# zihuixue/DynMM

Measured on AMD Instinct MI355X. Metric: images/sec fwd+bwd, 480x640 RGB-D, batch 32/GPU, higher is better.
Workload: dtype f32; 1 GPU; configs[2]: zero-grad + fwd + weighted 4-scale CE + FLOP loss + bwd + fused SGD-Nesterov update, --dynamic --global-gate soft DiffSoftmax gates tau=1; per_gpu_batch=32, global_batch=32, height=480, width=640, parallelism=dp1, launch=eager, streams=4, optimizer_in_step=fused SGD-Nesterov

## Files before the change

dynmm_amd/csrc/conv_igemm.hip:

```cpp
#include <stdlib.h>

#include "common.h"
#include "conv_igemm.h"
#include "conv_small.h"
#include "vec.h"

namespace dynmm {


__device__ __forceinline__ float ldg_f32(const float* sbase, unsigned voff_bytes) {
    return *reinterpret_cast<const float*>(reinterpret_cast<const char*>(sbase) + voff_bytes);
}
__device__ __forceinline__ float4 ldg_f32x4(const float* sbase, unsigned voff_bytes) {
    return *reinterpret_cast<const float4*>(reinterpret_cast<const char*>(sbase) + voff_bytes);
}


template <int TCO, int TPIX, int WCO, int WPIX, bool DGRAD, int MODE>
__global__ void __launch_bounds__(256, (TCO * TPIX > 8192 ? 2 : (TPIX > 128 ? 4 : 6))) conv_igemm_kernel(const IgemmArgs a) {
    constexpr bool GENERIC = MODE == 2;
    constexpr bool padded = MODE == 1;
    constexpr int BK = 16;
    constexpr int MCO = WCO / 32, MPIX = WPIX / 32;
    constexpr int WAVES_PIX = TPIX / WPIX;
    static_assert((TCO / WCO) * WAVES_PIX == 4, "4 waves per workgroup");
    constexpr int AQ = TCO / 4, A_ROWSTEP = 256 / AQ;
    constexpr int A_PER = (BK * AQ + 255) / 256;
    constexpr int B_PER = BK * TPIX / 256, B_ROWSTEP = 256 / TPIX;

    __shared__ __attribute__((aligned(16))) float As[2][BK][TCO];
    __shared__ __attribute__((aligned(16))) float Bs[2][BK][TPIX];

    const int t = threadIdx.x;
    const int lane = t & 63, wave = t >> 6;
    const int wave_co = wave / WAVES_PIX, wave_pix = wave % WAVES_PIX;
    DYNMM_TRACE_MARK(0);
#ifdef DYNMM_TRACE
    if (g_trace && threadIdx.x == 0) g_trace[(size_t)blockIdx.x * 6 + 4] = clock64();
#endif

    const int nblk = a.n_co_tiles * a.n_pix_tiles;
    const int lin = xcd_remap(blockIdx.x, nblk);
    const int co0 = (lin % a.n_co_tiles) * TCO;
    const int pix0 = (lin / a.n_co_tiles) * TPIX;

    const int HW = a.H * a.W;
    const int HoWo = a.Ho * a.Wo;

    const int a_q = t % AQ, a_row0 = t / AQ;
    const bool a_active = a_row0 < BK;
    int q_glob = co0 / 4 + a_q;
    if (q_glob > a.CoP / 4 - 1) q_glob = a.CoP / 4 - 1;
    const unsigned a_voff = (unsigned)((a_active ? a_row0 : 0) * a.CoP + q_glob * 4) * 4u;

    auto pix_decode = [&](int m, int& n, int& oh, int& ow, int& cls) {
        n = m / HoWo;
        const int q = m - n * HoWo;
        if (DGRAD && a.subpix) {
            const int Wc = a.Wo / a.SW;
            const int csz = HoWo / (a.SH * a.SW);
            cls = q / csz;
            const int q2 = q - cls * csz;
            const int ohc = q2 / Wc;
            const int ph = cls / a.SW;
            oh = ohc * a.SH + ph;
            ow = (q2 - ohc * Wc) * a.SW + (cls - ph * a.SW);
        } else {
            cls = 0;
            oh = q / a.Wo;
            ow = q - oh * a.Wo;
        }
    };
    const int b_col = t % TPIX, b_row0 = t / TPIX;
    const int m_b = pix0 + b_col;
    const bool m_ok = m_b < a.M;
    int n_b = 0, oh_b = 0, ow_b = 0, cls_b = 0;
    if (m_ok) pix_decode(m_b, n_b, oh_b, ow_b, cls_b);
    (void)cls_b;
    const int c2 = a.Ci - a.c_in_split;

    auto in_coord = [&](int r, int s, int& ih, int& iw) -> bool {
        if (!DGRAD) {
            ih = oh_b * a.SH - a.PH + r;
            iw = ow_b * a.SW - a.PW + s;
            return m_ok && ih >= 0 && ih < a.H && iw >= 0 && iw < a.W;
        } else {
            const int th = oh_b + a.PH - r, tw = ow_b + a.PW - s;
            if (!m_ok || th < 0 || tw < 0) return false;
            ih = th / a.SH;
            iw = tw / a.SW;
            return (ih * a.SH == th) && (iw * a.SW == tw) && ih < a.H && iw < a.W;
        }
    };

    float4 ra[A_PER];
    float rb[B_PER];
    f32x16 acc[MCO][MPIX];
#pragma unroll
    for (int mi = 0; mi < MCO; ++mi)
#pragma unroll
        for (int ni = 0; ni < MPIX; ++ni)
#pragma unroll
            for (int j = 0; j < 16; ++j) acc[mi][ni][j] = 0.f;

    const int khalf = lane >> 5, l31 = lane & 31;

    auto mfma_tile = [&](int buf) {
        float af[BK / 2][MCO], bf[BK / 2][MPIX];
#pragma unroll
        for (int kk = 0; kk < BK / 2; ++kk) {
#pragma unroll
            for (int mi = 0; mi < MCO; ++mi)
                af[kk][mi] = As[buf][2 * kk + khalf][wave_co * WCO + mi * 32 + l31];
#pragma unroll
            for (int ni = 0; ni < MPIX; ++ni)
                bf[kk][ni] = Bs[buf][2 * kk + khalf][wave_pix * WPIX + ni * 32 + l31];
        }
#pragma unroll
        for (int kk = 0; kk < BK / 2; ++kk)
#pragma unroll
            for (int mi = 0; mi < MCO; ++mi)
#pragma unroll
                for (int ni = 0; ni < MPIX; ++ni)
                    acc[mi][ni] = __builtin_amdgcn_mfma_f32_32x32x2f32(af[kk][mi], bf[kk][ni], acc[mi][ni], 0, 0, 0);
    };

    if constexpr (!GENERIC) {
        const int cpt = a.CiR / BK;
        int live_ph = -1, live_pw = -1;
        if (DGRAD && a.subpix) {
            int n0, oh0, ow0, c0, n1, oh1, ow1, c1;
            pix_decode(pix0, n0, oh0, ow0, c0);
            pix_decode(min(pix0 + TPIX, a.M) - 1, n1, oh1, ow1, c1);
            if (n0 == n1 && c0 == c1) { live_ph = c0 / a.SW; live_pw = c0 - live_ph * a.SW; }
        }
        auto tap_live = [&](int r, int s_) -> bool {
            if (!(DGRAD && a.subpix) || live_ph < 0) return true;
            return ((live_ph + a.PH - r) % a.SH == 0) && ((live_pw + a.PW - s_) % a.SW == 0);
        };
        int n_live = 0;
        for (int r = 0; r < a.KH; ++r)
            for (int s_ = 0; s_ < a.KW; ++s_) n_live += tap_live(r, s_) ? 1 : 0;
        const int nk = n_live * cpt;
        int ci0 = 0, tr = 0, ts = 0, kbase = 0;
        bool tap_ok;
        unsigned voff1, voff2;
        auto set_tap = [&]() {
            int ih = 0, iw = 0;
            tap_ok = in_coord(tr, ts, ih, iw);
            const unsigned pix = tap_ok ? (unsigned)(ih * a.W + iw) : 0u;
            voff1 = ((unsigned)(n_b * a.c_in_split + b_row0) * (unsigned)HW + pix) * 4u;
            voff2 = ((unsigned)(n_b * c2 + b_row0) * (unsigned)HW + pix) * 4u;
        };
        auto next_tap = [&]() {
            do {
                if (++ts == a.KW) { ts = 0; ++tr; }
                if (tr >= a.KH) return;
// ... 1143 lines not shown

extern "C" int dynmm_conv2d_stem_fwd_stats(const float* x, const float* wp_fwd, const float* bias, float* y, double* stats,
                                           const dynmm_conv_geom* g, void* stream) {
    (void)hipGetLastError();
    if (!x || !wp_fwd || !y || !stats || !geom_ok(g)) return DYNMM_EINVAL;
    if (!dynmm_conv2d_stem_fwd_stats_supported(g)) return DYNMM_EUNSUPPORTED;
    SmallConvArgs s{x, nullptr, wp_fwd, nullptr, bias, y, g->N, g->Ci, g->H, g->W, g->Co, g->Ho, g->Wo, g->KH, g->KW,
                    g->SH, g->SW, g->PH, g->PW, g->c_split, round_k(g->Ci), (g->Co + 3) & ~3, DYNMM_ACT_NONE};
    s.stats = stats;
    return launch_stem_conv_fwd(s, (hipStream_t)stream);
}

extern "C" int dynmm_conv2d_dgrad(const float* dy, const float* wp_dgrad, const float* mask,
                                  const float* accum, float* dx, float* dx2,
                                  const dynmm_conv_geom* g, void* stream) {
    (void)hipGetLastError();
    if (!dy || !wp_dgrad || !dx || !geom_ok(g)) return DYNMM_EINVAL;
    if ((g->c_split < g->Ci) != (dx2 != nullptr)) return DYNMM_EINVAL;
    if ((mask || accum) && dx2) return DYNMM_EUNSUPPORTED;
    IgemmArgs a{};
    a.x = dy; a.x2 = nullptr; a.wp = wp_dgrad; a.mask = mask; a.residual = accum; a.y = dx; a.y2 = dx2;
    a.N = g->N; a.Ci = g->Co; a.H = g->Ho; a.W = g->Wo;
    a.Co = g->Ci; a.Ho = g->H; a.Wo = g->W;
    a.KH = g->KH; a.KW = g->KW; a.SH = g->SH; a.SW = g->SW; a.PH = g->PH; a.PW = g->PW;
    a.c_in_split = g->Co; a.c_out_split = g->c_split; a.act = DYNMM_ACT_NONE;
    return launch_igemm<true>(a, (hipStream_t)stream);
}

static bool wgrad_fast_rows_ok(const dynmm_conv_geom* g) {
    return (g->Ci % 64 == 0) || (g->KH == 1 && g->KW == 1);
}

static void launch_wgrad_generic(const WgradArgs& a, const WgradGroup& grp, const WgradPlan& p, dim3 grid, bool dual,
                                 bool fast, hipStream_t st) {
#define DYNMM_WGRAD_LAUNCH(TCO, TK, WCO, WK)                                                          \
    do {                                                                                              \
        if (dual)                                                                                     \
            hipLaunchKernelGGL((conv_wgrad_kernel<TCO, TK, WCO, WK, true, false>), grid, dim3(256), 0, st, a, grp);  \
        else if (fast)                                                                                \
            hipLaunchKernelGGL((conv_wgrad_kernel<TCO, TK, WCO, WK, false, true>), grid, dim3(256), 0, st, a, grp);  \
        else                                                                                          \
            hipLaunchKernelGGL((conv_wgrad_kernel<TCO, TK, WCO, WK, false, false>), grid, dim3(256), 0, st, a, grp); \
    } while (0)
    if (p.tco == 128)
        DYNMM_WGRAD_LAUNCH(128, 128, 64, 64);
    else if (p.tco == 64 && p.tk == 192)
        DYNMM_WGRAD_LAUNCH(64, 192, 32, 96);
    else if (p.tco == 64 && p.tk == 64)
        DYNMM_WGRAD_LAUNCH(64, 64, 32, 32);
    else if (p.tco == 64)
        DYNMM_WGRAD_LAUNCH(64, 128, 64, 32);
    else
        DYNMM_WGRAD_LAUNCH(32, 128, 32, 32);
#undef DYNMM_WGRAD_LAUNCH
}

static size_t generic_wgrad_workspace_bytes(const dynmm_conv_geom* g);

extern "C" size_t dynmm_conv2d_wgrad_workspace_bytes(const dynmm_conv_geom* g) {
    if (!geom_ok(g)) return 0;
    const size_t stem = stem_conv_wgrad_eligible(g->Ci, g->Co, g->KH, g->KW, g->SH, g->SW, g->PH, g->PW, g->c_split < g->Ci, false)
                            ? stem_conv_wgrad_workspace_bytes(g->N, g->Ci, g->Ho, g->Wo) : 0;
    const size_t gen = generic_wgrad_workspace_bytes(g);
    const size_t co8 = co8_wgrad_eligible(g->Ci, g->Co, g->H, g->W, g->Ho, g->Wo, g->KH, g->KW, g->SH, g->SW, g->PH, g->PW, g->c_split)
                           ? co8_wgrad_workspace_bytes(g->N, g->Ci, g->Co) : 0;
    const size_t m = stem > gen ? stem : gen;
    return co8 > m ? co8 : m;
}

static size_t plan_workspace_bytes(const dynmm_conv_geom* g, const WgradPlan& p) {
    if (p.splits <= 1) return 0;
    const size_t wslab = ((size_t)p.splits * g->Co * g->Ci * g->KH * g->KW + 3) & ~(size_t)3;
    return (wslab + (size_t)p.splits * g->Co) * sizeof(float);
}

static size_t generic_wgrad_workspace_bytes(const dynmm_conv_geom* g) {
    const size_t a = plan_workspace_bytes(g, plan_wgrad(g)), b = plan_workspace_bytes(g, plan_wgrad(g, false));
    return a > b ? a : b;
}

extern "C" int dynmm_conv2d_wgrad(const float* x, const float* x2, const float* dy, float* dw, float* dbias,
                                  void* workspace, size_t workspace_bytes,
                                  const dynmm_conv_geom* g, void* stream) {
    (void)hipGetLastError();
    if (!x || !dy || !dw || !geom_ok(g)) return DYNMM_EINVAL;
    if ((g->c_split < g->Ci) != (x2 != nullptr)) return DYNMM_EINVAL;
    if (stem_conv_wgrad_eligible(g->Ci, g->Co, g->KH, g->KW, g->SH, g->SW, g->PH, g->PW, x2 != nullptr, dbias != nullptr) &&
        ((reinterpret_cast<uintptr_t>(dy) & 15u) == 0)) {
        const size_t need_s = stem_conv_wgrad_workspace_bytes(g->N, g->Ci, g->Ho, g->Wo);
        if (!workspace || workspace_bytes < need_s) return DYNMM_EWORKSPACE;
        return launch_stem_conv_wgrad(x, dy, dw, (float*)workspace, g->N, g->Ci, g->H, g->W, g->Ho, g->Wo, (hipStream_t)stream);
    }
    const bool aligned16 = ((reinterpret_cast<uintptr_t>(x) | reinterpret_cast<uintptr_t>(dy)) & 15u) == 0;
    if (co8_wgrad_eligible(g->Ci, g->Co, g->H, g->W, g->Ho, g->Wo, g->KH, g->KW, g->SH, g->SW, g->PH, g->PW, g->c_split) &&
        ((reinterpret_cast<uintptr_t>(x) | reinterpret_cast<uintptr_t>(x2)) & 15u) == 0) {
        const size_t need_c = co8_wgrad_workspace_bytes(g->N, g->Ci, g->Co);
        if (!workspace || workspace_bytes < need_c || (reinterpret_cast<uintptr_t>(workspace) & 15u)) return DYNMM_EWORKSPACE;
        return launch_co8_wgrad(x, x2, dy, dw, dbias, (float*)workspace, g->N, g->Ci, g->H, g->W, g->Co, g->Ho, g->Wo,
                                g->c_split, (hipStream_t)stream);
    }
    const WgradPlan p = plan_wgrad(g, aligned16 && !x2);
    const size_t need = generic_wgrad_workspace_bytes(g);
    if (need > 0 && (!workspace || workspace_bytes < need)) return DYNMM_EWORKSPACE;
    WgradArgs a{};
    a.x = x; a.x2 = x2; a.dy = dy;
    a.out = p.splits > 1 ? (float*)workspace : dw;
    const size_t wslab = ((size_t)p.splits * g->Co * g->Ci * g->KH * g->KW + 3) & ~(size_t)3;
    float* bias_slabs = p.splits > 1 ? (float*)workspace + wslab : dbias;
    a.out_bias = dbias ? bias_slabs : nullptr;
    a.N = g->N; a.Ci = g->Ci; a.H = g->H; a.W = g->W; a.Co = g->Co; a.Ho = g->Ho; a.Wo = g->Wo;
    a.KH = g->KH; a.KW = g->KW; a.SH = g->SH; a.SW = g->SW; a.PH = g->PH; a.PW = g->PW;
    a.c_split = g->c_split;
    a.M = g->N * g->Ho * g->Wo;
    a.K = g->KH * g->KW * g->Ci;
    a.n_co_tiles = p.n_co_tiles; a.n_k_tiles = p.n_k_tiles; a.steps_per_split = p.steps_per_split;
    hipStream_t st = (hipStream_t)stream;
    dim3 grid((unsigned)(p.n_co_tiles * p.n_k_tiles * p.splits));
    const bool dual = x2 != nullptr;
    const bool fast = !dual && wgrad_fast_rows_ok(g) && g->H >= g->KH && g->W >= g->KW;
    a.magic_wo = (g->Wo >= 2 && (unsigned long long)g->Ho * g->Wo * g->Wo < (1ull << 32)) ? (unsigned)((1ull << 32) / (unsigned)g->Wo) + 1u : 0u;
    const bool v4 = !p.v6 && !dual && p.tco == 128 && p.tk == 128 && (g->Ci % 64 == 0) && g->SW == 1 &&
                    (g->KW == 1 || g->KW == 3) && g->PW == g->KW / 2 && g->W == g->Wo && (g->W % 4 == 0) &&
                    ((g->Ho * g->Wo) % 4 == 0) && g->H >= g->KH &&
                    ((reinterpret_cast<uintptr_t>(x) & 15u) == 0) && ((reinterpret_cast<uintptr_t>(dy) & 15u) == 0);
    const bool bias_ok4 = !dbias || ((g->Co % 4 == 0) && ((reinterpret_cast<uintptr_t>(bias_slabs) & 15u) == 0) &&
                                     ((reinterpret_cast<uintptr_t>(dbias) & 15u) == 0));
    const bool perm = (v4 || p.v6) && p.splits > 1 && ((reinterpret_cast<uintptr_t>(workspace) & 15u) == 0) && bias_ok4;
    a.k_major_out = perm ? 1 : 0;
    if (p.v6 || v4) {
        if (p.v6)
            launch_wgrad_v6(a, WgradGroup{}, grid, wgrad_v6_occupancy(g), st);
        else
            hipLaunchKernelGGL((conv_wgrad_v4_kernel<128, 128, 1>), grid, dim3(512), 0, st, a, WgradGroup{});
        DYNMM_LAUNCH_CHECK();
        if (perm) {
            const int n = g->Co * a.K, nb1 = ceil_div(n / 4, 64), nb2 = dbias ? ceil_div(g->Co / 4, 64) : 0;
            hipLaunchKernelGGL(reduce_slabs_perm_kernel, dim3(nb1 + nb2), dim3(256), 0, st, (const float*)workspace, dw,
                               n, p.splits, g->Ci, g->KH * g->KW, a.K, dbias ? bias_slabs : nullptr, dbias,
                               dbias ? g->Co : 0, nb1, ReduceGroup{});
            DYNMM_LAUNCH_CHECK();
            return DYNMM_OK;
        }
    } else
        launch_wgrad_generic(a, WgradGroup{}, p, grid, dual, fast, st);
    DYNMM_LAUNCH_CHECK();
    if (p.splits > 1) {
        launch_reduce_slabs((const float*)workspace, dw, g->Co * a.K, p.splits, st, dbias ? bias_slabs : nullptr,
                            dbias, dbias ? g->Co : 0);
        DYNMM_LAUNCH_CHECK();
    }
    return DYNMM_OK;
}

static bool wgrad_v4_shape_ok(const dynmm_conv_geom* g, const WgradPlan& p) {
    if (p.v6) return (g->Co % 4 == 0);
    return g->c_split == g->Ci && p.tco == 128 && p.tk == 128 && (g->Ci % 64 == 0) && g->SW == 1 &&
           (g->KW == 1 || g->KW == 3) && g->PW == g->KW / 2 && g->W == g->Wo && (g->W % 4 == 0) &&
           ((g->Ho * g->Wo) % 4 == 0) && g->H >= g->KH && (g->Co % 4 == 0);
}

static WgradPlan plan_wgrad_group(const dynmm_conv_geom* g, int n) {
    WgradPlan p = plan_wgrad(g);
    if (!p.v6) p.target = 512;
    plan_splits(p, g, n);
    return p;
}

static size_t group_problem_floats(const dynmm_conv_geom* g, const WgradPlan& p) {
    const size_t wslab = ((size_t)p.splits * g->Co * g->Ci * g->KH * g->KW + 3) & ~(size_t)3;
    return (wslab + (size_t)p.splits * g->Co + 3) & ~(size_t)3;
}

extern "C" int dynmm_conv2d_wgrad_groupable(const dynmm_conv_geom* g) {
    if (!geom_ok(g) || g->c_split != g->Ci) return 0;
    if (stem_conv_wgrad_eligible(g->Ci, g->Co, g->KH, g->KW, g->SH, g->SW, g->PH, g->PW, false, false)) return 0;
    if (co8_wgrad_eligible(g->Ci, g->Co, g->H, g->W, g->Ho, g->Wo, g->KH, g->KW, g->SH, g->SW, g->PH, g->PW, g->c_split)) return 0;
    const WgradPlan p = plan_wgrad(g);
    if (p.splits <= 1) return 0;
    return wgrad_v4_shape_ok(g, p) ? 2 : 1;
}

extern "C" int dynmm_conv2d_wgrad_variant(const dynmm_conv_geom* g) {
    if (!geom_ok(g)) return 0;
    if (stem_conv_wgrad_eligible(g->Ci, g->Co, g->KH, g->KW, g->SH, g->SW, g->PH, g->PW, g->c_split < g->Ci, false)) return 0;
    if (co8_wgrad_eligible(g->Ci, g->Co, g->H, g->W, g->Ho, g->Wo, g->KH, g->KW, g->SH, g->SW, g->PH, g->PW, g->c_split)) return 8;
    const WgradPlan p = plan_wgrad(g);
    if (p.v6) return 6;
    return wgrad_v4_shape_ok(g, p) ? 4 : 0;
}

extern "C" size_t dynmm_conv2d_wgrad_group_workspace_bytes(const dynmm_conv_geom* g, int n) {
    if (!geom_ok(g) || n < 1 || n > kWgradGroupMax) return 0;
    if (n == 1 || !dynmm_conv2d_wgrad_groupable(g)) return dynmm_conv2d_wgrad_workspace_bytes(g);
    const WgradPlan p = plan_wgrad_group(g, n);
    return sizeof(float) * group_problem_floats(g, p) * (size_t)n;
}

extern "C" int dynmm_conv2d_wgrad_group(int n, const float* const* xs, const float* const* dys, float* const* dws,
                                        float* const* dbiases, void* workspace, size_t workspace_bytes,
                                        const dynmm_conv_geom* g, void* stream) {
    (void)hipGetLastError();
    if (n < 1 || n > kWgradGroupMax || !xs || !dys || !dws || !geom_ok(g)) return DYNMM_EINVAL;
    bool aligned = (reinterpret_cast<uintptr_t>(workspace) & 15u) == 0;
    for (int i = 0; i < n; ++i) {
        if (!xs[i] || !dys[i] || !dws[i]) return DYNMM_EINVAL;
        aligned = aligned && ((reinterpret_cast<uintptr_t>(xs[i]) | reinterpret_cast<uintptr_t>(dys[i])) & 15u) == 0 &&
                  (!dbiases || !dbiases[i] || (reinterpret_cast<uintptr_t>(dbiases[i]) & 15u) == 0);
        if (dbiases && ((dbiases[i] != nullptr) != (dbiases[0] != nullptr))) return DYNMM_EINVAL;
    }
    const int kind = dynmm_conv2d_wgrad_groupable(g);
    if (n == 1 || kind == 0 || (kind == 2 && !aligned)) {
        for (int i = 0; i < n; ++i) {
            const int rc = dynmm_conv2d_wgrad(xs[i], nullptr, dys[i], dws[i], dbiases ? dbiases[i] : nullptr, workspace,
                                              workspace_bytes, g, stream);
            if (rc != DYNMM_OK) return rc;
        }
        return DYNMM_OK;
    }
    const WgradPlan p = plan_wgrad_group(g, n);
    const size_t per_floats = group_problem_floats(g, p);
    if (!workspace || workspace_bytes < sizeof(float) * per_floats * (size_t)n) return DYNMM_EWORKSPACE;
    const bool has_bias = dbiases && dbiases[0];
    const size_t wslab = ((size_t)p.splits * g->Co * g->Ci * g->KH * g->KW + 3) & ~(size_t)3;
    WgradArgs a{};
    WgradGroup grp{};
    grp.nprob = n;
    grp.per = p.n_co_tiles * p.n_k_tiles * p.splits;
    for (int i = 0; i < n; ++i) {
        float* base = (float*)workspace + per_floats * (size_t)i;
        grp.x[i] = xs[i];
        grp.dy[i] = dys[i];
        grp.out[i] = base;
        grp.out_bias[i] = has_bias ? base + wslab : nullptr;
    }
    a.x = xs[0]; a.x2 = nullptr; a.dy = dys[0]; a.out = grp.out[0]; a.out_bias = grp.out_bias[0];
    a.N = g->N; a.Ci = g->Ci; a.H = g->H; a.W = g->W; a.Co = g->Co; a.Ho = g->Ho; a.Wo = g->Wo;
    a.KH = g->KH; a.KW = g->KW; a.SH = g->SH; a.SW = g->SW; a.PH = g->PH; a.PW = g->PW;
    a.c_split = g->c_split;
    a.M = g->N * g->Ho * g->Wo;
    a.K = g->KH * g->KW * g->Ci;
    a.n_co_tiles = p.n_co_tiles; a.n_k_tiles = p.n_k_tiles; a.steps_per_split = p.steps_per_split;
    a.magic_wo = (g->Wo >= 2 && (unsigned long long)g->Ho * g->Wo * g->Wo < (1ull << 32)) ? (unsigned)((1ull << 32) / (unsigned)g->Wo) + 1u : 0u;
    hipStream_t st = (hipStream_t)stream;
    dim3 grid((unsigned)(grp.per * n));
    if (kind == 1) {
        a.k_major_out = 0;
        const bool fast = wgrad_fast_rows_ok(g) && g->H >= g->KH && g->W >= g->KW;
        launch_wgrad_generic(a, grp, p, grid, false, fast, st);
        DYNMM_LAUNCH_CHECK();
        ReduceGroup rgp{};
        rgp.nprob = n;
        for (int i = 0; i < n; ++i) {
            rgp.slabs[i] = grp.out[i];
            rgp.out[i] = dws[i];
            rgp.slabs2[i] = has_bias ? grp.out_bias[i] : nullptr;
            rgp.out2[i] = has_bias ? dbiases[i] : nullptr;
        }
        launch_reduce_slabs_group(rgp, g->Co * a.K, p.splits, has_bias ? g->Co : 0, st);
        DYNMM_LAUNCH_CHECK();
        return DYNMM_OK;
    }
    a.k_major_out = 1;
    if (p.v6)
        launch_wgrad_v6(a, grp, grid, wgrad_v6_occupancy(g), st);
    else
        hipLaunchKernelGGL((conv_wgrad_v4_kernel<128, 128, 1>), grid, dim3(512), 0, st, a, grp);
    DYNMM_LAUNCH_CHECK();
    const int nel = g->Co * a.K, nb1 = ceil_div(nel / 4, 64), nb2 = has_bias ? ceil_div(g->Co / 4, 64) : 0;
    ReduceGroup rg{};
    rg.nprob = n;
    for (int i = 0; i < n; ++i) {
        rg.slabs[i] = grp.out[i];
        rg.out[i] = dws[i];
        rg.slabs2[i] = has_bias ? grp.out_bias[i] : nullptr;
        rg.out2[i] = has_bias ? dbiases[i] : nullptr;
    }
    hipLaunchKernelGGL(reduce_slabs_perm_kernel, dim3(nb1 + nb2, n), dim3(256), 0, st, (const float*)nullptr, (float*)nullptr,
                       nel, p.splits, g->Ci, g->KH * g->KW, a.K, (const float*)nullptr, (float*)nullptr,
                       has_bias ? g->Co : 0, nb1, rg);
    DYNMM_LAUNCH_CHECK();
    return DYNMM_OK;
}

extern "C" int dynmm_reduce_slabs(const float* slabs, float* out, int n, int nslabs, void* stream) {
    (void)hipGetLastError();
    if (!slabs || !out || n <= 0 || nslabs <= 0) return DYNMM_EINVAL;
    launch_reduce_slabs(slabs, out, n, nslabs, (hipStream_t)stream);
    DYNMM_LAUNCH_CHECK();
    return DYNMM_OK;
}

#ifdef DYNMM_TRACE
#include "conv_igemm_v5.hip"
#endif
```

dynmm_amd/csrc/conv_small.h:

```cpp
#pragma once
#include <hip/hip_runtime.h>

namespace dynmm {

struct SmallConvArgs {
    const float* x;
    const float* x2;
    const float* wp;
    const float* scale;
    const float* shift;
    float* y;
    int N, Ci, H, W, Co, Ho, Wo, KH, KW, SH, SW, PH, PW, c_split, CiR, CoP, act;
    double* stats = nullptr;
};

struct StemWgradArgs {
    const float* x;
    const float* dy;
    float* slabs;
    int N, H, W, Ho, Wo;
};

bool stem_conv_wgrad_eligible(int Ci, int Co, int KH, int KW, int SH, int SW, int PH, int PW, bool has_x2, bool has_bias);
size_t stem_conv_wgrad_workspace_bytes(int N, int Ci, int Ho, int Wo);
int launch_stem_conv_wgrad(const float* x, const float* dy, float* dw, float* workspace, int N, int Ci, int H, int W,
                           int Ho, int Wo, hipStream_t st);

bool co8_wgrad_eligible(int Ci, int Co, int H, int W, int Ho, int Wo, int KH, int KW, int SH, int SW, int PH, int PW, int c_split);
size_t co8_wgrad_workspace_bytes(int N, int Ci, int Co);
int launch_co8_wgrad(const float* x, const float* x2, const float* dy, float* dw, float* dbias, float* workspace, int N, int Ci,
                     int H, int W, int Co, int Ho, int Wo, int c_split, hipStream_t st);

bool small_conv_fwd_eligible(const SmallConvArgs& a, const float* residual);
int launch_small_conv_fwd(const SmallConvArgs& a, hipStream_t st);
bool stem_conv_fwd_eligible(const SmallConvArgs& a, const float* residual);
int launch_stem_conv_fwd(const SmallConvArgs& a, hipStream_t st);

}
```

dynmm_amd/csrc/conv_small.hip:

```cpp
#include "common.h"
#include "conv_small.h"
#include "conv_igemm.h"

namespace dynmm {

constexpr int kSP = 5;
constexpr int kSRows = 4;
constexpr int kSColGroups = 16;
constexpr int kSCols = kSColGroups * kSP;

__device__ __forceinline__ float small_act(float v, int act) {
    if (act == DYNMM_ACT_RELU) return v > 0.f ? v : 0.f;
    if (act == DYNMM_ACT_TANH) return tanhf(v);
    if (act == DYNMM_ACT_SWISH) return swish_fwd(v);
    if (act == DYNMM_ACT_HSWISH) return hswish_fwd(v);
    return v;
}

template <int KS, int S>
__global__ void __launch_bounds__(256) conv_co8_fwd_kernel(const SmallConvArgs a) {
    constexpr int IR = (kSRows - 1) * S + KS;
    constexpr int IC = (kSCols - 1) * S + KS;
    constexpr int TILE = IR * IC;
    constexpr int NLD = (TILE + 63) / 64;
    constexpr int XW = (kSP - 1) * S + KS;
    constexpr int RED = 4 * 8 * kSRows * kSCols;
    constexpr int LDSF = (4 * 2 * TILE > RED) ? 4 * 2 * TILE : RED;
    __shared__ float lds[LDSF];

    const int lane = threadIdx.x & 63;
    const int wave = __builtin_amdgcn_readfirstlane(threadIdx.x >> 6);
    const int tw = (a.Wo + kSCols - 1) / kSCols, th = (a.Ho + kSRows - 1) / kSRows;
    int b = blockIdx.x;
    const int n = b / (th * tw);
    b -= n * th * tw;
    const int oh0 = (b / tw) * kSRows, ow0 = (b - (b / tw) * tw) * kSCols;
    const int ih0 = oh0 * S, iw0 = ow0 * S;
    const int r = lane >> 4, cg = lane & 15;

    int goff[NLD];
    unsigned okmask = 0u;
#pragma unroll
    for (int k = 0; k < NLD; ++k) {
        const int e = k * 64 + lane;
        const int rr = e / IC, cc = e - rr * IC;
        const bool ok = e < TILE && ih0 + rr < a.H && iw0 + cc < a.W;
        goff[k] = ok ? (ih0 + rr) * a.W + iw0 + cc : 0;
        okmask |= ok ? (1u << k) : 0u;
    }
    const int cpw = a.Ci / 4;
    const int c_begin = wave * cpw;
    const int HW = a.H * a.W;
    float* const tile0 = lds + wave * 2 * TILE;

    auto plane = [&](int ci) -> const float* {
        return ci < a.c_split ? a.x + ((size_t)n * a.c_split + ci) * HW
                              : a.x2 + ((size_t)n * (a.Ci - a.c_split) + (ci - a.c_split)) * HW;
    };
    float st[NLD];
    auto stage_load = [&](int ci) {
        const float* p = plane(ci);
#pragma unroll
        for (int k = 0; k < NLD; ++k) st[k] = p[goff[k]];
    };
    auto stage_store = [&](float* t) {
#pragma unroll
        for (int k = 0; k < NLD; ++k)
            if (k * 64 + lane < TILE) t[k * 64 + lane] = ((okmask >> k) & 1u) ? st[k] : 0.f;
    };

    float acc[8][kSP];
#pragma unroll
    for (int co = 0; co < 8; ++co)
#pragma unroll
        for (int p = 0; p < kSP; ++p) acc[co][p] = 0.f;

    auto wave_sync = [] {
        __builtin_amdgcn_fence(__ATOMIC_ACQ_REL, "wavefront");
        __builtin_amdgcn_wave_barrier();
    };
    stage_load(c_begin);
    stage_store(tile0);
    wave_sync();
    for (int i = 0; i < cpw; ++i) {
        const int ci = c_begin + i;
        const float* t = tile0 + (i & 1) * TILE;
        if (i + 1 < cpw) stage_load(ci + 1);
        const float* wci = a.wp + (size_t)ci * 8;
#pragma unroll
        for (int kh = 0; kh < KS; ++kh) {
            const float* row = t + (S * r + kh) * IC + S * kSP * cg;
            float xv[XW];
#pragma unroll
            for (int j = 0; j < XW; ++j) xv[j] = row[j];
#pragma unroll
            for (int kw = 0; kw < KS; ++kw) {
                const float* wt = wci + (size_t)(kh * KS + kw) * a.CiR * 8;
#pragma unroll
                for (int co = 0; co < 8; ++co) {
                    const float wv = wt[co];
#pragma unroll
                    for (int p = 0; p < kSP; ++p) acc[co][p] = fmaf(wv, xv[S * p + kw], acc[co][p]);
                }
            }
        }
        if (i + 1 < cpw) stage_store(tile0 + ((i + 1) & 1) * TILE);
        wave_sync();
    }
    __syncthreads();
#pragma unroll
    for (int co = 0; co < 8; ++co)
#pragma unroll
        for (int p = 0; p < kSP; ++p)
            lds[((wave * 8 + co) * kSRows + r) * kSCols + cg * kSP + p] = acc[co][p];
    __syncthreads();
    constexpr int PER = 8 * kSRows * kSCols;
    for (int e = threadIdx.x; e < PER; e += 256) {
        const int co = e / (kSRows * kSCols), rem = e - co * (kSRows * kSCols);
        const int rr = rem / kSCols, cc = rem - rr * kSCols;
        const int oh = oh0 + rr, ow = ow0 + cc;
        if (co < a.Co && oh < a.Ho && ow < a.Wo) {
            float v = ((lds[e] + lds[PER + e]) + lds[2 * PER + e]) + lds[3 * PER + e];
            v = v * (a.scale ? a.scale[co] : 1.f) + (a.shift ? a.shift[co] : 0.f);
            a.y[(((size_t)n * a.Co + co) * a.Ho + oh) * a.Wo + ow] = small_act(v, a.act);
        }
    }
}

struct Co8WgradArgs {
    const float* x;
    const float* x2;
    const float* dy;
    float* slabs;
    float* bias_slabs;
    int N, Ci, H, W, Co, Ho, Wo, c_split, NI, G;
};

__device__ __forceinline__ float row16_sum(float v) {
    v += __int_as_float(__builtin_amdgcn_mov_dpp(__float_as_int(v), 0xB1, 0xF, 0xF, true));
    v += __int_as_float(__builtin_amdgcn_mov_dpp(__float_as_int(v), 0x4E, 0xF, 0xF, true));
    v += __int_as_float(__builtin_amdgcn_mov_dpp(__float_as_int(v), 0x141, 0xF, 0xF, true));
    v += __int_as_float(__builtin_amdgcn_mov_dpp(__float_as_int(v), 0x140, 0xF, 0xF, true));
    return v;
}

template <int KS, int S>
__global__ void __launch_bounds__(256, 1) conv_co8_wgrad_kernel(const Co8WgradArgs a) {
    constexpr int PR = 16;
    constexpr int IR = (PR - 1) * S + KS;
    constexpr int XW = (kSP - 1) * S + KS;
    constexpr int NACC = KS * KS * 8;
    extern __shared__ __attribute__((aligned(16))) float dyn_lds[];
    const int tile_floats = IR * a.W + 16;
    float* const tiles = dyn_lds;
    float* const red = dyn_lds + 2 * tile_floats;
// ... 184 lines not shown
    const int tw = (a.Wo + TCW - 1) / TCW, th = (a.Ho + TRW - 1) / TRW;
    const int HW = a.H * a.W;
    const int tiles = a.N * th * tw;

    float areg[NSTEP];
#pragma unroll
    for (int st = 0; st < NSTEP; ++st) {
        const int ci = st / (KS * KW8 / 2), rem = st - ci * (KS * KW8 / 2);
        const int kh = rem / (KW8 / 2), kp = rem - kh * (KW8 / 2);
        const int kw = 2 * kp + khalf;
        areg[st] = kw < KS ? a.wp[((size_t)(kh * KS + kw) * a.CiR + ci) * a.CoP + mi * 32 + l31] : 0.f;
    }
    const int pb_off = (S * 2 * rp) * ICP + S * l31 + khalf;
    const bool vec_out = (a.Wo & 3) == 0;

    auto fetch_patch = [&](int tile, float* dst) __attribute__((always_inline)) {
        int b = tile;
        const int n = b / (th * tw);
        b -= n * th * tw;
        const int ih0 = (b / tw) * TRW * S - PAD, iw0 = (b - (b / tw) * tw) * TCW * S - PAD;
        const float* xn = a.x + (size_t)n * CI * HW;
#pragma unroll 1
        for (int it = 0; it < NIT; ++it) {
            const int e = it * 256 + threadIdx.x;
            const int ci = min(e / (IR * ICP), CI - 1), rem = e - ci * (IR * ICP);
            const int rr = rem / ICP, cc = rem - rr * ICP;
            const int ih = ih0 + rr, iw = iw0 + cc;
            const bool inside = e < NPATCH;
            const bool ok = inside && ih >= 0 && ih < a.H && iw >= 0 && iw < a.W;
            float* slot = dst + it * 256 + (threadIdx.x & ~63);
            if (ok)
                __builtin_amdgcn_global_load_lds((const __attribute__((address_space(1))) void*)(xn + (size_t)ci * HW + (size_t)ih * a.W + iw),
                                                 (__attribute__((address_space(3))) void*)slot, 4, 0, 0);
            else if (inside)
                dst[e] = 0.f;
        }
    };

    float st1[2][4], st2[2][4];
#pragma unroll
    for (int q = 0; q < 2; ++q)
#pragma unroll
        for (int ps = 0; ps < 4; ++ps) st1[q][ps] = st2[q][ps] = 0.f;

    int buf = 0;
    if ((int)blockIdx.x < tiles) fetch_patch(blockIdx.x, patch2[0]);
    __builtin_amdgcn_s_waitcnt(0);
    __syncthreads();
    for (int tile = blockIdx.x; tile < tiles; tile += gridDim.x, buf ^= 1) {
        int b = tile;
        const int n = b / (th * tw);
        b -= n * th * tw;
        const int oh0 = (b / tw) * TRW, ow0 = (b - (b / tw) * tw) * TCW;
        const float* patch = patch2[buf];
        const float* pb = patch + pb_off;
        float* const ostage = patch2[buf] + wave * OCH;
        const int next = tile + (int)gridDim.x;
        if (next < tiles) fetch_patch(next, patch2[buf ^ 1]);

        f32x16 acc[2][2];
#pragma unroll
        for (int i = 0; i < 2; ++i)
#pragma unroll
            for (int j = 0; j < 2; ++j)
#pragma unroll
                for (int e = 0; e < 16; ++e) acc[i][j][e] = 0.f;
#pragma unroll
        for (int ci = 0; ci < CI; ++ci)
#pragma unroll
            for (int kh = 0; kh < KS; ++kh)
#pragma unroll
                for (int kp = 0; kp < KW8 / 2; ++kp) {
                    const int boff = (ci * IR + kh) * ICP + 2 * kp;
                    const float av = areg[(ci * KS + kh) * (KW8 / 2) + kp];
                    const float b00 = pb[boff], b01 = pb[boff + S * 32];
                    const float b10 = pb[boff + S * ICP], b11 = pb[boff + S * ICP + S * 32];
                    acc[0][0] = __builtin_amdgcn_mfma_f32_32x32x2f32(av, b00, acc[0][0], 0, 0, 0);
                    acc[0][1] = __builtin_amdgcn_mfma_f32_32x32x2f32(av, b01, acc[0][1], 0, 0, 0);
                    acc[1][0] = __builtin_amdgcn_mfma_f32_32x32x2f32(av, b10, acc[1][0], 0, 0, 0);
                    acc[1][1] = __builtin_amdgcn_mfma_f32_32x32x2f32(av, b11, acc[1][1], 0, 0, 0);
                }
        __syncthreads();

#pragma unroll
        for (int rr = 0; rr < 2; ++rr)
#pragma unroll
            for (int q = 0; q < 2; ++q) {
#pragma unroll
                for (int jj = 0; jj < 8; ++jj) {
                    const int j = 8 * q + jj;
                    const int cl = (jj & 3) + 8 * (jj >> 2) + 4 * khalf;
                    const int c = mi * 32 + 16 * q + cl;
                    const float sc = a.scale ? a.scale[c] : 1.f, sh = a.shift ? a.shift[c] : 0.f;
                    const int act = STATS ? DYNMM_ACT_NONE : a.act;
                    ostage[cl * OP + l31] = small_act(fmaf(acc[rr][0][j], sc, sh), act);
                    ostage[cl * OP + 32 + l31] = small_act(fmaf(acc[rr][1][j], sc, sh), act);
                }
                __builtin_amdgcn_fence(__ATOMIC_ACQ_REL, "wavefront");
                __builtin_amdgcn_wave_barrier();
                const int oh = oh0 + 2 * rp + rr;
                if (oh < a.Ho) {
#pragma unroll
                    for (int ps = 0; ps < 4; ++ps) {
                        const int cl = ps * 4 + (lane >> 4), col = (lane & 15) * 4;
                        const int c = mi * 32 + 16 * q + cl;
                        const float4 v = *reinterpret_cast<const float4*>(ostage + cl * OP + col);
                        float* yr = a.y + (((size_t)n * a.Co + c) * a.Ho + oh) * a.Wo + ow0 + col;
                        if (vec_out && ow0 + col + 3 < a.Wo) {
                            *reinterpret_cast<float4*>(yr) = v;
                            if constexpr (STATS) {
                                st1[q][ps] += (v.x + v.y) + (v.z + v.w);
                                st2[q][ps] += fmaf(v.x, v.x, v.y * v.y) + fmaf(v.z, v.z, v.w * v.w);
                            }
                        } else {
                            const float e[4] = {v.x, v.y, v.z, v.w};
#pragma unroll
                            for (int k = 0; k < 4; ++k)
                                if (ow0 + col + k < a.Wo) {
                                    yr[k] = e[k];
                                    if constexpr (STATS) {
                                        st1[q][ps] += e[k];
                                        st2[q][ps] = fmaf(e[k], e[k], st2[q][ps]);
                                    }
                                }
                        }
                    }
                }
                __builtin_amdgcn_fence(__ATOMIC_ACQ_REL, "wavefront");
                __builtin_amdgcn_wave_barrier();
            }
        __builtin_amdgcn_s_waitcnt(0);
        __syncthreads();
    }
    if constexpr (STATS) {
#pragma unroll
        for (int q = 0; q < 2; ++q)
#pragma unroll
            for (int ps = 0; ps < 4; ++ps) {
                float s1 = st1[q][ps], s2 = st2[q][ps];
#pragma unroll
                for (int o = 1; o < 16; o <<= 1) {
                    s1 += __shfl_xor(s1, o, 64);
                    s2 += __shfl_xor(s2, o, 64);
                }
                if ((lane & 15) == 0) {
                    const int c = mi * 32 + 16 * q + 4 * ps + (lane >> 4);
                    atomicAdd(a.stats + c, (double)s1);
                    atomicAdd(a.stats + a.Co + c, (double)s2);
                }
            }
    }
}

template <int CI>
__global__ void __launch_bounds__(256, CI == 1 ? 4 : 2) conv_stem_wgrad_kernel(const StemWgradArgs a) {
    constexpr int KS = 7, S = 2, PAD = 3, KW8 = 8;
    constexpr int TRW = 2, TCW = 64, NPX = TRW * TCW;
    constexpr int IR = (TRW - 1) * S + KS;
    constexpr int ICP = (TCW - 1) * S + KW8 + 1;
    constexpr int KT = CI * KS * KW8;
    constexpr int NKT = (KT + 31) / 32;
    constexpr int KPW = NKT / 2;
    constexpr int PP = NPX + 1;
    __shared__ float patch[CI * IR * ICP];
    __shared__ float dyt[64 * PP];

    const int lane = threadIdx.x & 63, l31 = lane & 31, khalf = lane >> 5;
    const int wave = threadIdx.x >> 6;
    const int cot = wave & 1, kt0 = (wave >> 1) * KPW;
    const int tw = (a.Wo + TCW - 1) / TCW, th = (a.Ho + TRW - 1) / TRW;
    const int HW = a.H * a.W, HoWo = a.Ho * a.Wo;
    const int tiles = a.N * th * tw;

    int boff[KPW];
#pragma unroll
    for (int j = 0; j < KPW; ++j) {
        int k = (kt0 + j) * 32 + l31;
        if (k >= KT) k = 0;
        const int ci = k / (KS * KW8), rem = k - ci * (KS * KW8);
        boff[j] = (ci * IR + (rem >> 3)) * ICP + (rem & 7) + S * khalf;
    }
    const float* ab = dyt + (cot * 32 + l31) * PP + khalf;
    f32x16 acc[KPW];
#pragma unroll
    for (int j = 0; j < KPW; ++j)
#pragma unroll
        for (int e = 0; e < 16; ++e) acc[j][e] = 0.f;

    for (int tile = blockIdx.x; tile < tiles; tile += gridDim.x) {
        int b = tile;
        const int n = b / (th * tw);
        b -= n * th * tw;
        const int oh0 = (b / tw) * TRW, ow0 = (b - (b / tw) * tw) * TCW;
        const int ih0 = oh0 * S - PAD, iw0 = ow0 * S - PAD;
        __syncthreads();
        {
            constexpr int NIT = (CI * IR * ICP + 255) / 256;
            float sv[NIT];
            const float* xn = a.x + (size_t)n * CI * HW;
#pragma unroll
            for (int it = 0; it < NIT; ++it) {
                const int e = it * 256 + threadIdx.x;
                const int ci = min(e / (IR * ICP), CI - 1), rem = e - ci * (IR * ICP);
                const int rr = rem / ICP, cc = rem - rr * ICP;
                const int ih = ih0 + rr, iw = iw0 + cc;
                const bool ok = ih >= 0 && ih < a.H && iw >= 0 && iw < a.W;
                const float v = xn[(size_t)ci * HW + (size_t)min(max(ih, 0), a.H - 1) * a.W + min(max(iw, 0), a.W - 1)];
                sv[it] = ok ? v : 0.f;
            }
            float4 dv[8];
            const float* dn = a.dy + (size_t)n * 64 * HoWo;
            const bool vec = (a.Wo & 3) == 0;
#pragma unroll
            for (int it = 0; it < 8; ++it) {
                const int i4 = it * 256 + threadIdx.x;
                const int co = i4 >> 5, q = i4 & 31, r = q >> 4, c4 = (q & 15) * 4;
                const int oh = oh0 + r, ow = ow0 + c4;
                const float* src = dn + (size_t)co * HoWo + (size_t)min(oh, a.Ho - 1) * a.Wo;
                float4 v = make_float4(0.f, 0.f, 0.f, 0.f);
                if (oh < a.Ho) {
                    if (vec && ow + 3 < a.Wo) v = *reinterpret_cast<const float4*>(src + ow);
                    else {
                        if (ow < a.Wo) v.x = src[ow];
                        if (ow + 1 < a.Wo) v.y = src[ow + 1];
                        if (ow + 2 < a.Wo) v.z = src[ow + 2];
                        if (ow + 3 < a.Wo) v.w = src[ow + 3];
                    }
                }
                dv[it] = v;
            }
#pragma unroll
            for (int it = 0; it < NIT; ++it) {
                const int e = it * 256 + threadIdx.x;
                if (e < CI * IR * ICP) patch[e] = sv[it];
            }
#pragma unroll
            for (int it = 0; it < 8; ++it) {
                const int i4 = it * 256 + threadIdx.x;
                const int co = i4 >> 5, q = i4 & 31;
                float* dst = dyt + co * PP + q * 4;
                dst[0] = dv[it].x; dst[1] = dv[it].y; dst[2] = dv[it].z; dst[3] = dv[it].w;
            }
        }
        __syncthreads();
#pragma unroll
        for (int ps = 0; ps < NPX / 2; ++ps) {
            const int row = (2 * ps) / TCW, col = (2 * ps) % TCW;
            const int poff = S * row * ICP + S * col;
            const float av = ab[2 * ps];
#pragma unroll
            for (int j = 0; j < KPW; ++j) {
                const float bv = patch[boff[j] + poff];
                acc[j] = __builtin_amdgcn_mfma_f32_32x32x2f32(av, bv, acc[j], 0, 0, 0);
            }
        }
    }
    float* slab = a.slabs + (size_t)blockIdx.x * 64 * (NKT * 32);
#pragma unroll
    for (int j = 0; j < KPW; ++j)
#pragma unroll
        for (int e = 0; e < 16; ++e) {
            const int co = cot * 32 + (e & 3) + 8 * (e >> 2) + 4 * khalf;
            slab[(size_t)co * (NKT * 32) + (kt0 + j) * 32 + l31] = acc[j][e];
        }
}

__global__ void __launch_bounds__(256) stem_wgrad_finish_kernel(const float* __restrict__ slabs, int nslabs, int kpad,
                                                                int CI, float* __restrict__ dw) {
    const int i = blockIdx.x * 256 + threadIdx.x;
    const int per_co = CI * 49;
    if (i >= 64 * per_co) return;
    const int co = i / per_co, rem = i - co * per_co;
    const int ci = rem / 49, t = rem - ci * 49;
    const int k = (ci * 7 + t / 7) * 8 + t % 7;
    float s0 = 0.f, s1 = 0.f, s2 = 0.f, s3 = 0.f;
    const size_t stride = (size_t)64 * kpad;
    const float* p = slabs + (size_t)co * kpad + k;
    int sl = 0;
    for (; sl + 3 < nslabs; sl += 4) {
        s0 += p[(size_t)sl * stride];
        s1 += p[(size_t)(sl + 1) * stride];
        s2 += p[(size_t)(sl + 2) * stride];
        s3 += p[(size_t)(sl + 3) * stride];
    }
    for (; sl < nslabs; ++sl) s0 += p[(size_t)sl * stride];
    dw[i] = (s0 + s1) + (s2 + s3);
}

static int stem_wgrad_grid(long tiles, int Ci) {
    static int cus = 0;
    if (!cus) {
        int dev = 0;
        hipDeviceProp_t prop;
        if (hipGetDevice(&dev) == hipSuccess && hipGetDeviceProperties(&prop, dev) == hipSuccess) cus = prop.multiProcessorCount;
        if (cus <= 0) cus = 256;
    }
    const long cap = (long)cus * (Ci == 1 ? 4 : 2);
    return (int)(tiles < cap ? tiles : cap);
}

bool stem_conv_wgrad_eligible(int Ci, int Co, int KH, int KW, int SH, int SW, int PH, int PW, bool has_x2, bool has_bias) {
    if (has_x2 || has_bias) return false;
    if (KH != 7 || KW != 7 || SH != 2 || SW != 2 || PH != 3 || PW != 3) return false;
    return (Ci == 1 || Ci == 3) && Co == 64;
}

size_t stem_conv_wgrad_workspace_bytes(int N, int Ci, int Ho, int Wo) {
    const long tiles = (long)N * ceil_div(Ho, 2) * ceil_div(Wo, 64);
    const int kpad = ((Ci * 56 + 31) / 32) * 32;
    return sizeof(float) * (size_t)stem_wgrad_grid(tiles, Ci) * 64 * kpad;
}

int launch_stem_conv_wgrad(const float* x, const float* dy, float* dw, float* workspace, int N, int Ci, int H, int W,
                           int Ho, int Wo, hipStream_t st) {
    const long tiles = (long)N * ceil_div(Ho, 2) * ceil_div(Wo, 64);
    if (tiles > 0x7fffffffL) return DYNMM_EUNSUPPORTED;
    const int grid = stem_wgrad_grid(tiles, Ci);
    const int kpad = ((Ci * 56 + 31) / 32) * 32;
    StemWgradArgs a{x, dy, workspace, N, H, W, Ho, Wo};
    if (Ci == 3)
        hipLaunchKernelGGL((conv_stem_wgrad_kernel<3>), dim3(grid), dim3(256), 0, st, a);
    else
        hipLaunchKernelGGL((conv_stem_wgrad_kernel<1>), dim3(grid), dim3(256), 0, st, a);
    DYNMM_LAUNCH_CHECK();
    hipLaunchKernelGGL(stem_wgrad_finish_kernel, dim3(ceil_div(64 * Ci * 49, 256)), dim3(256), 0, st, workspace, grid, kpad,
                       Ci, dw);
    DYNMM_LAUNCH_CHECK();
    return DYNMM_OK;
}

bool stem_conv_fwd_eligible(const SmallConvArgs& a, const float* residual) {
    if (residual || a.x2) return false;
    if (a.KH != 7 || a.KW != 7 || a.SH != 2 || a.SW != 2 || a.PH != 3 || a.PW != 3) return false;
    return (a.Ci == 1 || a.Ci == 3) && a.Co == 64;
}

int launch_stem_conv_fwd(const SmallConvArgs& a_in, hipStream_t st) {
    const long tiles = (long)a_in.N * ceil_div(a_in.Ho, 4) * ceil_div(a_in.Wo, 64);
    if (tiles > 0x7fffffffL) return DYNMM_EUNSUPPORTED;
    const SmallConvArgs& a = a_in;
    static int cus = 0;
    if (!cus) {
        int dev = 0;
        hipDeviceProp_t prop;
        if (hipGetDevice(&dev) == hipSuccess && hipGetDeviceProperties(&prop, dev) == hipSuccess) cus = prop.multiProcessorCount;
        if (cus <= 0) cus = 256;
    }
    const int resident = a.Ci == 1 ? 3 : 2;
    const long cap = (long)cus * resident;
    const unsigned grid = (unsigned)(tiles < cap ? tiles : cap);
    if (a.stats) {
        if (a.act != DYNMM_ACT_NONE) return DYNMM_EUNSUPPORTED;
        if (a.Ci == 3)
            hipLaunchKernelGGL((conv_stem_fwd_kernel<3, true>), dim3(grid), dim3(256), 0, st, a);
        else
            hipLaunchKernelGGL((conv_stem_fwd_kernel<1, true>), dim3(grid), dim3(256), 0, st, a);
    } else if (a.Ci == 3)
        hipLaunchKernelGGL((conv_stem_fwd_kernel<3>), dim3(grid), dim3(256), 0, st, a);
    else
        hipLaunchKernelGGL((conv_stem_fwd_kernel<1>), dim3(grid), dim3(256), 0, st, a);
    DYNMM_LAUNCH_CHECK();
    return DYNMM_OK;
}

bool small_conv_fwd_eligible(const SmallConvArgs& a, const float* residual) {
    if (residual) return false;
    if (a.Co < 5 || a.Co > 8) return false;
    if (a.KH != 5 || a.KW != 5 || a.SH != 2 || a.SW != 2 || a.PH != 0 || a.PW != 0) return false;
    if (a.Ci % 4 != 0 || a.Ci < 16) return false;
    if (a.c_split < a.Ci && a.c_split % (a.Ci / 4) != 0) return false;
    return true;
}

int launch_small_conv_fwd(const SmallConvArgs& a, hipStream_t st) {
    const long tiles = (long)a.N * ceil_div(a.Ho, kSRows) * ceil_div(a.Wo, kSCols);
    if (tiles > 0x7fffffffL) return DYNMM_EUNSUPPORTED;
    hipLaunchKernelGGL((conv_co8_fwd_kernel<5, 2>), dim3((unsigned)tiles), dim3(256), 0, st, a);
    DYNMM_LAUNCH_CHECK();
    return DYNMM_OK;
}

}
```

dynmm_amd/csrc/pointwise.hip:

```cpp
#include "common.h"
#include <initializer_list>
#include "vec.h"
#include "pool.h"

namespace dynmm {

__device__ __forceinline__ float keep_if(float v, bool keep) { return __int_as_float(__float_as_int(v) & -(int)keep); }



__global__ void __launch_bounds__(256) maxpool_fwd_kernel(const float* __restrict__ x,
                                                          float* __restrict__ y,
                                                          signed char* __restrict__ idx, int H,
                                                          int W, int Ho, int Wo) {
    const size_t plane = blockIdx.x;
    const float* xp = x + plane * H * W;
    const int HoWo = Ho * Wo;
    const int beg = blockIdx.y * kChunk, end = min(HoWo, beg + kChunk);
    for (int i = beg + threadIdx.x; i < end; i += 256) {
        const int oh = i / Wo, ow = i - oh * Wo;
        float best = -INFINITY;
        int bi = -1;
#pragma unroll
        for (int r = 0; r < 3; ++r) {
// ... 872 lines not shown
    return DYNMM_OK;
}

extern "C" int dynmm_nearest_into_bwd(const float* g_out, float* dy, int N, int C, int h, int w,
                                      int Ctot, int c_off, int H, int W, void* stream) {
    (void)hipGetLastError();
    if (!g_out || !dy || N <= 0 || C <= 0 || h <= 0 || w <= 0 || H <= 0 || W <= 0) return DYNMM_EINVAL;
    if (c_off < 0 || c_off + C > Ctot) return DYNMM_EINVAL;
    const int area = ceil_div(H, h) * ceil_div(W, w);
    const int nout = N * C * h * w;
#define DYNMM_NIB(L) hipLaunchKernelGGL(nearest_into_bwd_kernel<L>, dim3(ceil_div_sz((size_t)nout * L, 256)), dim3(256), 0, ST, \
                                        g_out, dy, N, C, h, w, Ctot, c_off, H, W)
    if ((h == H && w == W) || area < 8) DYNMM_NIB(1);
    else if (area < 32) DYNMM_NIB(4);
    else if (area < 128) DYNMM_NIB(16);
    else DYNMM_NIB(64);
#undef DYNMM_NIB
    DYNMM_LAUNCH_CHECK();
    return DYNMM_OK;
}

extern "C" int dynmm_upsample2x_dw3x3_fwd(const float* x, const float* w, const float* b,
                                          const float* skip, float* y, int N, int C, int H, int W,
                                          void* stream) {
    (void)hipGetLastError();
    if (!x || !w || !y || N <= 0 || C <= 0 || H <= 0 || W <= 0) return DYNMM_EINVAL;
    if (!aligned16(y) || (skip && !aligned16(skip))) return DYNMM_EUNSUPPORTED;
    dim3 grid(N * C, plane_chunks(H * ((W + 1) / 2), kChunk / 8));
    hipLaunchKernelGGL(upsample_fwd_kernel, grid, dim3(256), 0, ST, x, w, b, skip, y, C, H, W);
    DYNMM_LAUNCH_CHECK();
    return DYNMM_OK;
}

static int upsample_w_splits(int N, int C) {
    int S = 2048 / C;
    if (S < 1) S = 1;
    if (S > N) S = N;
    return S;
}

extern "C" size_t dynmm_upsample2x_dw3x3_bwd_workspace_bytes(int N, int C) {
    if (N <= 0 || C <= 0) return 0;
    const int S = upsample_w_splits(N, C);
    return S > 1 ? sizeof(float) * (size_t)S * C * 10 : 0;
}

extern "C" int dynmm_upsample2x_dw3x3_bwd(const float* g, const float* x, const float* w, float* dx,
                                          float* dw, float* db, float* workspace, int N, int C, int H, int W,
                                          void* stream) {
    (void)hipGetLastError();
    if (!g || !w || N <= 0 || C <= 0 || H <= 0 || W <= 0) return DYNMM_EINVAL;
    if (dx) {
        dim3 grid(N * C, plane_chunks(H * W, kChunk));
        const int pairs = (W % 2 == 0) && aligned16(g) && ((reinterpret_cast<uintptr_t>(dx) & 7u) == 0);
        hipLaunchKernelGGL(upsample_bwd_dx_kernel, grid, dim3(256), 0, ST, g, w, dx, C, H, W, pairs);
        DYNMM_LAUNCH_CHECK();
    }
    if (dw) {
        if (!x) return DYNMM_EINVAL;
        const int S = upsample_w_splits(N, C);
        if (S == 1) {
            hipLaunchKernelGGL(upsample_bwd_w_kernel, dim3(C, 1), dim3(256), 0, ST, g, x, dw, db, N, C, H, W);
            DYNMM_LAUNCH_CHECK();
        } else {
            if (!workspace) return DYNMM_EWORKSPACE;
            float* pw = workspace, *pb = workspace + (size_t)S * C * 9;
            hipLaunchKernelGGL(upsample_bwd_w_kernel, dim3(C, S), dim3(256), 0, ST, g, x, pw, db ? pb : nullptr, N, C, H, W);
            DYNMM_LAUNCH_CHECK();
            launch_reduce_slabs(pw, dw, C * 9, S, ST, db ? pb : nullptr, db, db ? C : 0);
            DYNMM_LAUNCH_CHECK();
        }
    }
    return DYNMM_OK;
}

static int gap2_launch(const float* xr, const float* xd, float* sr, float* sd, int NC, int HW, const float* tr, int C,
                       void* stream);

extern "C" int dynmm_gap2_fwd(const float* xr, const float* xd, float* sr, float* sd, int NC, int HW,
                              void* stream) {
    return gap2_launch(xr, xd, sr, sd, NC, HW, nullptr, 1, stream);
}

extern "C" int dynmm_gap2_bnrelu_fwd(const float* xr, const float* xd, const float* bn_tr, int C, float* sr, float* sd,
                                     int NC, int HW, void* stream) {
    if (!bn_tr || C <= 0 || NC % C != 0) return DYNMM_EINVAL;
    return gap2_launch(xr, xd, sr, sd, NC, HW, bn_tr, C, stream);
}

static int gap2_launch(const float* xr, const float* xd, float* sr, float* sd, int NC, int HW, const float* tr, int C,
                       void* stream) {
    (void)hipGetLastError();
    if (!xr || !sr || NC <= 0 || HW <= 0) return DYNMM_EINVAL;
    if (xd && !sd) return DYNMM_EINVAL;
#define DYNMM_GAP2(V, DUAL, TR) hipLaunchKernelGGL((gap2_kernel<V, DUAL, TR>), dim3(NC), dim3(256), 0, ST, xr, xd, sr, sd, HW, tr, C)
#define DYNMM_GAP2_V(V)                                    \
    do {                                                   \
        if (xd && tr) DYNMM_GAP2(V, true, true);           \
        else if (xd) DYNMM_GAP2(V, true, false);           \
        else if (tr) DYNMM_GAP2(V, false, true);           \
        else DYNMM_GAP2(V, false, false);                  \
    } while (0)
    if (can_vec4(HW, {xr, xd}))
        DYNMM_GAP2_V(4);
    else
        DYNMM_GAP2_V(1);
#undef DYNMM_GAP2_V
#undef DYNMM_GAP2
    DYNMM_LAUNCH_CHECK();
    return DYNMM_OK;
}

extern "C" int dynmm_axpby_fwd(const float* xr, const float* xd, const float* a, const float* b,
                               float* out, int NC, int HW, void* stream) {
    (void)hipGetLastError();
    if (!xr || !xd || !a || !b || !out || NC <= 0 || HW <= 0) return DYNMM_EINVAL;
    dim3 grid(NC, plane_chunks(HW, kChunk));
    if (can_vec4(HW, {xr, xd, out}))
        hipLaunchKernelGGL(axpby_fwd_kernel<4>, grid, dim3(256), 0, ST, xr, xd, a, b, out, HW);
    else
        hipLaunchKernelGGL(axpby_fwd_kernel<1>, grid, dim3(256), 0, ST, xr, xd, a, b, out, HW);
    DYNMM_LAUNCH_CHECK();
    return DYNMM_OK;
}

extern "C" int dynmm_axpby_bwd_reduce(const float* g, const float* xr, const float* xd, float* da,
                                      float* db, int NC, int HW, void* stream) {
    (void)hipGetLastError();
    if (!g || !xr || !xd || !da || !db || NC <= 0 || HW <= 0) return DYNMM_EINVAL;
    if (can_vec4(HW, {g, xr, xd}))
        hipLaunchKernelGGL(axpby_bwd_reduce_kernel<4>, dim3(NC), dim3(256), 0, ST, g, xr, xd, da, db, HW);
    else
        hipLaunchKernelGGL(axpby_bwd_reduce_kernel<1>, dim3(NC), dim3(256), 0, ST, g, xr, xd, da, db, HW);
    DYNMM_LAUNCH_CHECK();
    return DYNMM_OK;
}

extern "C" int dynmm_axpby_bwd_apply(const float* g, const float* a, const float* b, const float* ca,
                                     const float* cb, float cscale, float* dxr, float* dxd, int NC,
                                     int HW, void* stream) {
    (void)hipGetLastError();
    if (!g || !a || !b || !dxr || !dxd || NC <= 0 || HW <= 0) return DYNMM_EINVAL;
    dim3 grid(NC, plane_chunks(HW, kChunk));
    if (can_vec4(HW, {g, dxr, dxd}))
        hipLaunchKernelGGL(axpby_bwd_apply_kernel<4>, grid, dim3(256), 0, ST, g, a, b, ca, cb, cscale, dxr, dxd, HW);
    else
        hipLaunchKernelGGL(axpby_bwd_apply_kernel<1>, grid, dim3(256), 0, ST, g, a, b, ca, cb, cscale, dxr, dxd, HW);
    DYNMM_LAUNCH_CHECK();
    return DYNMM_OK;
}

namespace dynmm {

struct StemBnArgs {
    const float* go; const signed char* io;
    const float* gd; const signed char* id;
    const float* coef; const float* off; float cscale;
    const float* x; const float* mean; const float* invstd; const float* gamma; const float* beta;
    int N, C, H, W, Ho, Wo;
};

__device__ __forceinline__ void stem_gy_block(const StemBnArgs& a, size_t plane, int ar, int t, float fc, float fo,
                                              float (&top)[8], float (&bot)[8]) {
    const size_t po = plane * (size_t)a.Ho * a.Wo;
    pool_bwd_block(a.go + po, a.io + po, ar, t, a.Ho, a.Wo, top, bot);
#pragma unroll
    for (int k = 0; k < 8; ++k) { top[k] = fmaf(fc, top[k], fo); bot[k] = fmaf(fc, bot[k], fo); }
    if (a.gd) {
        float dt[8], db[8];
        pool_bwd_block(a.gd + po, a.id + po, ar, t, a.Ho, a.Wo, dt, db);
#pragma unroll
        for (int k = 0; k < 8; ++k) { top[k] += dt[k]; bot[k] += db[k]; }
    }
}

__global__ void __launch_bounds__(256) stem_bn_bwd_reduce_kernel(const StemBnArgs a, double* __restrict__ sums) {
    __shared__ float red[4];
    const int c = blockIdx.x, S = gridDim.y;
    const float mu = a.mean[c], is = a.invstd[c];
    const float sc = a.gamma[c] * is;
    const float sh = fmaf(-mu, sc, a.beta[c]);
    const int Wq = a.Wo / 4, nq = a.Ho * Wq;
    float s1 = 0.f, s2 = 0.f;
    for (int n = blockIdx.y; n < a.N; n += S) {
        const size_t plane = (size_t)n * a.C + c;
        const float fc = a.coef[plane], fo = a.off ? a.off[plane] * a.cscale : 0.f;
        const float* xp = a.x + plane * (size_t)a.H * a.W;
        float a1 = 0.f, a2 = 0.f;
        for (int q = threadIdx.x; q < nq; q += 256) {
            const int ar = q / Wq, t = q - ar * Wq;
            float top[8], bot[8];
            stem_gy_block(a, plane, ar, t, fc, fo, top, bot);
            const size_t o = (size_t)(2 * ar) * a.W + 8 * t;
#pragma unroll
            for (int h = 0; h < 2; ++h) {
                const float4 x0 = *reinterpret_cast<const float4*>(xp + o + 4 * h);
                const float4 x1 = *reinterpret_cast<const float4*>(xp + o + a.W + 4 * h);
                const float xv[8] = {x0.x, x0.y, x0.z, x0.w, x1.x, x1.y, x1.z, x1.w};
#pragma unroll
                for (int k = 0; k < 8; ++k) {
                    const float gy = k < 4 ? top[4 * h + k] : bot[4 * h + k - 4];
                    const float ge = fmaf(xv[k], sc, sh) > 0.f ? gy : 0.f;
                    a1 += ge;
                    a2 += ge * (xv[k] - mu) * is;
                }
            }
        }
        s1 += a1; s2 += a2;
    }
    const float t1 = block_reduce_sum_256<float>(s1, red);
    const float t2 = block_reduce_sum_256<float>(s2, red);
    if (threadIdx.x == 0) {
        atomicAdd(&sums[c], (double)t1);
        atomicAdd(&sums[a.C + c], (double)t2);
    }
}

__global__ void __launch_bounds__(256) stem_bn_bwd_apply_kernel(const StemBnArgs a, const double* __restrict__ sums,
                                                                float* __restrict__ dx, float* __restrict__ dgamma,
                                                                float* __restrict__ dbeta) {
    const size_t plane = blockIdx.x;
    const int c = (int)(plane % a.C);
    const float mu = a.mean[c], is = a.invstd[c];
    const float sc = a.gamma[c] * is;
    const float sh = fmaf(-mu, sc, a.beta[c]);
    const float sg = (float)sums[c], sgx = (float)sums[a.C + c];
    if (plane < (size_t)a.C && blockIdx.y == 0 && threadIdx.x == 0) {
        if (dgamma) dgamma[c] = sgx;
        if (dbeta) dbeta[c] = sg;
    }
    const float invM = 1.f / ((float)a.N * (float)(a.H * a.W));
    const float k0 = sc, m1 = sg * invM, m2 = sgx * invM;
    const float fc = a.coef[plane], fo = a.off ? a.off[plane] * a.cscale : 0.f;
    const float* xp = a.x + plane * (size_t)a.H * a.W;
    float* dp = dx + plane * (size_t)a.H * a.W;
    const int Wq = a.Wo / 4, nq = a.Ho * Wq;
    const int beg = blockIdx.y * (kChunk / 4), end = min(nq, beg + kChunk / 4);
    for (int q = beg + threadIdx.x; q < end; q += 256) {
        const int ar = q / Wq, t = q - ar * Wq;
        float top[8], bot[8];
        stem_gy_block(a, plane, ar, t, fc, fo, top, bot);
        const size_t o = (size_t)(2 * ar) * a.W + 8 * t;
#pragma unroll
        for (int h = 0; h < 2; ++h) {
            const float4 x0 = *reinterpret_cast<const float4*>(xp + o + 4 * h);
            const float4 x1 = *reinterpret_cast<const float4*>(xp + o + a.W + 4 * h);
            const float xv[8] = {x0.x, x0.y, x0.z, x0.w, x1.x, x1.y, x1.z, x1.w};
            float ov[8];
#pragma unroll
            for (int k = 0; k < 8; ++k) {
                const float gy = k < 4 ? top[4 * h + k] : bot[4 * h + k - 4];
                const float ge = fmaf(xv[k], sc, sh) > 0.f ? gy : 0.f;
                ov[k] = k0 * (ge - m1 - (xv[k] - mu) * is * m2);
            }
            *reinterpret_cast<float4*>(dp + o + 4 * h) = make_float4(ov[0], ov[1], ov[2], ov[3]);
            *reinterpret_cast<float4*>(dp + o + a.W + 4 * h) = make_float4(ov[4], ov[5], ov[6], ov[7]);
        }
    }
}

}

extern "C" int dynmm_axpby_pool_supported(int H, int W) { return (H > 0 && W > 0 && H % 2 == 0 && W % 8 == 0) ? 1 : 0; }

extern "C" int dynmm_axpby_pool_fwd(const float* xr, const float* xd, const float* a, const float* b, float* y_out,
                                    signed char* idx_out, float* y_depth, signed char* idx_depth, const float* bn_tr,
                                    int C, int NC, int H, int W, void* stream) {
    (void)hipGetLastError();
    if (!xr || !xd || !a || !b || !y_out || !idx_out || !y_depth || !idx_depth || NC <= 0) return DYNMM_EINVAL;
    if (bn_tr && (C <= 0 || NC % C != 0)) return DYNMM_EINVAL;
    const int Ho = H / 2, Wo = W / 2;
    if (!pool_fusable(H, W, Ho, Wo, {xr, xd, y_out, y_depth}, {idx_out, idx_depth})) return DYNMM_EUNSUPPORTED;
    hipLaunchKernelGGL(axpby_pool_fwd_kernel, dim3(NC, plane_chunks(Ho * Wo, kChunk)), dim3(256), 0, ST, xr, xd, a, b,
                       y_out, idx_out, y_depth, idx_depth, H, W, Ho, Wo, bn_tr, C);
    DYNMM_LAUNCH_CHECK();
    return DYNMM_OK;
}

extern "C" int dynmm_axpby_pool_bwd_reduce(const float* g_out, const signed char* idx_out, const float* xr,
                                           const float* xd, float* da, float* db, const float* bn_tr, int C, int NC,
                                           int H, int W, void* stream) {
    (void)hipGetLastError();
    if (!g_out || !idx_out || !xr || !xd || !da || !db || NC <= 0) return DYNMM_EINVAL;
    if (bn_tr && (C <= 0 || NC % C != 0)) return DYNMM_EINVAL;
    const int Ho = H / 2, Wo = W / 2;
    if (!pool_fusable(H, W, Ho, Wo, {g_out, xr, xd}, {idx_out})) return DYNMM_EUNSUPPORTED;
    hipLaunchKernelGGL(axpby_pool_bwd_reduce_kernel, dim3(NC), dim3(256), 0, ST, g_out, idx_out, xr, xd, da, db, H, W,
                       Ho, Wo, bn_tr, C);
    DYNMM_LAUNCH_CHECK();
    return DYNMM_OK;
}

extern "C" int dynmm_axpby_pool_bwd_apply(const float* g_out, const signed char* idx_out, const float* g_depth,
                                          const signed char* idx_depth, const float* a, const float* b, const float* ca,
                                          const float* cb, float cscale, float* dxr, float* dxd, int NC, int H, int W,
                                          void* stream) {
    (void)hipGetLastError();
    if (!g_out || !idx_out || !g_depth || !idx_depth || !a || !b || !dxr || !dxd || NC <= 0) return DYNMM_EINVAL;
    const int Ho = H / 2, Wo = W / 2;
    if (!pool_fusable(H, W, Ho, Wo, {g_out, g_depth, dxr, dxd}, {idx_out, idx_depth})) return DYNMM_EUNSUPPORTED;
    hipLaunchKernelGGL(axpby_pool_bwd_apply_kernel, dim3(NC, plane_chunks(Ho * Wo, kChunk)), dim3(256), 0, ST, g_out,
                       idx_out, g_depth, idx_depth, a, b, ca, cb, cscale, dxr, dxd, H, W, Ho, Wo);
    DYNMM_LAUNCH_CHECK();
    return DYNMM_OK;
}

static int stem_bn_args(StemBnArgs& a, const float* g_out, const signed char* idx_out, const float* g_depth,
                        const signed char* idx_depth, const float* coef, const float* off, float cscale, const float* x,
                        const float* mean, const float* invstd, const float* gamma, const float* beta, int N, int C, int H,
                        int W) {
    if (!g_out || !idx_out || !coef || !x || !mean || !invstd || !gamma || !beta || N <= 0 || C <= 0) return DYNMM_EINVAL;
    if ((g_depth != nullptr) != (idx_depth != nullptr)) return DYNMM_EINVAL;
    const int Ho = H / 2, Wo = W / 2;
    if (!pool_fusable(H, W, Ho, Wo, {g_out, g_depth, x}, {idx_out, idx_depth})) return DYNMM_EUNSUPPORTED;
    a = StemBnArgs{g_out, idx_out, g_depth, idx_depth, coef, off, cscale, x, mean, invstd, gamma, beta, N, C, H, W, Ho, Wo};
    return DYNMM_OK;
}

extern "C" int dynmm_stem_bn_bwd_reduce(const float* g_out, const signed char* idx_out, const float* g_depth,
                                        const signed char* idx_depth, const float* coef, const float* off, float cscale,
                                        const float* x, const float* mean, const float* invstd, const float* gamma,
                                        const float* beta, double* sums, int N, int C, int H, int W, int sums_are_zero,
                                        void* stream) {
    (void)hipGetLastError();
    StemBnArgs a;
    const int rc = stem_bn_args(a, g_out, idx_out, g_depth, idx_depth, coef, off, cscale, x, mean, invstd, gamma, beta, N, C,
                                H, W);
    if (rc != DYNMM_OK || !sums) return rc != DYNMM_OK ? rc : DYNMM_EINVAL;
    if (!sums_are_zero) DYNMM_HIP_TRY(hipMemsetAsync(sums, 0, sizeof(double) * 2 * C, ST));
    int S = 2048 / C;
    S = S < 1 ? 1 : (S > N ? N : S);
    hipLaunchKernelGGL(stem_bn_bwd_reduce_kernel, dim3(C, S), dim3(256), 0, ST, a, sums);
    DYNMM_LAUNCH_CHECK();
    return DYNMM_OK;
}

extern "C" int dynmm_stem_bn_bwd_apply(const float* g_out, const signed char* idx_out, const float* g_depth,
                                       const signed char* idx_depth, const float* coef, const float* off, float cscale,
                                       const float* x, const float* mean, const float* invstd, const float* gamma,
                                       const float* beta, const double* sums, float* dx, float* dgamma, float* dbeta,
                                       int N, int C, int H, int W, void* stream) {
    (void)hipGetLastError();
    StemBnArgs a;
    const int rc = stem_bn_args(a, g_out, idx_out, g_depth, idx_depth, coef, off, cscale, x, mean, invstd, gamma, beta, N, C,
                                H, W);
    if (rc != DYNMM_OK || !sums || !dx) return rc != DYNMM_OK ? rc : DYNMM_EINVAL;
    if (reinterpret_cast<uintptr_t>(dx) & 15u) return DYNMM_EUNSUPPORTED;
    hipLaunchKernelGGL(stem_bn_bwd_apply_kernel, dim3(N * C, plane_chunks(a.Ho * a.Wo, kChunk)), dim3(256), 0, ST, a, sums,
                       dx, dgamma, dbeta);
    DYNMM_LAUNCH_CHECK();
    return DYNMM_OK;
}
```

dynmm_amd/csrc/pool.h:

```cpp
#pragma once
#include <initializer_list>
#include "common.h"

namespace dynmm {

static inline int plane_chunks(int HW, int chunk) { return (HW + chunk - 1) / chunk; }
constexpr int kChunk = 8192;

__device__ __forceinline__ void pool_update(float& best, int& bi, float val, int code) {
    if (bi < 0 || val > best || val != val) { best = val; bi = code; }
}

__device__ __forceinline__ void pool_bwd_block(const float* __restrict__ gp, const signed char* __restrict__ ip, int a,
                                               int t, int Ho, int Wo, float (&top)[8], float (&bot)[8]) {
    float gv[2][5];
    int cd[2][5];
#pragma unroll
    for (int rr = 0; rr < 2; ++rr) {
        const bool rok = a + rr < Ho;
        const size_t o = (size_t)(rok ? a + rr : a) * Wo + 4 * t;
        const float4 g4 = *reinterpret_cast<const float4*>(gp + o);
        const unsigned c4 = *reinterpret_cast<const unsigned*>(ip + o);
        const bool cok = 4 * t + 4 < Wo;
        const float g5 = cok ? gp[o + 4] : 0.f;
        const int c5 = cok ? (int)ip[o + 4] : -1;
        gv[rr][0] = g4.x; gv[rr][1] = g4.y; gv[rr][2] = g4.z; gv[rr][3] = g4.w; gv[rr][4] = g5;
#pragma unroll
        for (int j = 0; j < 4; ++j) cd[rr][j] = rok ? (int)(signed char)((c4 >> (8 * j)) & 0xffu) : -1;
        cd[rr][4] = rok ? c5 : -1;
    }
#pragma unroll
    for (int m = 0; m < 4; ++m) {
        const float g00 = gv[0][m], g01 = gv[0][m + 1], g10 = gv[1][m], g11 = gv[1][m + 1];
        const int c00 = cd[0][m], c01 = cd[0][m + 1], c10 = cd[1][m], c11 = cd[1][m + 1];
        top[2 * m] = c00 == 4 ? g00 : 0.f;
        top[2 * m + 1] = (c00 == 5 ? g00 : 0.f) + (c01 == 3 ? g01 : 0.f);
        bot[2 * m] = (c00 == 7 ? g00 : 0.f) + (c10 == 1 ? g10 : 0.f);
        bot[2 * m + 1] = ((c00 == 8 ? g00 : 0.f) + (c01 == 6 ? g01 : 0.f)) + ((c10 == 2 ? g10 : 0.f) + (c11 == 0 ? g11 : 0.f));
    }
}

static inline bool pool_fusable(int H, int W, int Ho, int Wo, std::initializer_list<const void*> p16,
                                std::initializer_list<const void*> p4) {
    if (H % 2 != 0 || W % 8 != 0 || Ho != H / 2 || Wo != W / 2) return false;
    for (const void* p : p16) if (reinterpret_cast<uintptr_t>(p) & 15u) return false;
    for (const void* p : p4) if (reinterpret_cast<uintptr_t>(p) & 3u) return false;
    return true;
}

}
```

dynmm_amd/lib.py:

```python
import ctypes as C
import os
import subprocess

_HERE = os.path.dirname(os.path.abspath(__file__))
LIB_PATH = os.path.join(_HERE, 'libdynmm_hip.so')
CSRC = os.path.join(_HERE, 'csrc')

ACT_NONE, ACT_RELU, ACT_TANH, ACT_SWISH, ACT_HSWISH = 0, 1, 2, 3, 4
SMOOTH_ACTS = (ACT_SWISH, ACT_HSWISH)
DYNMM_OK, DYNMM_EINVAL, DYNMM_EUNSUPPORTED, DYNMM_EWORKSPACE = 0, -1, -2, -3
ACT = {None: 0, 'none': 0, 'relu': 1, 'tanh': 2, 'swish': 3, 'silu': 3, 'hswish': 4}
LOSS_BCE_LOGITS, LOSS_L1 = 0, 1

c_f = C.c_void_p
c_i = C.c_int
c_fl = C.c_float
c_sz = C.c_size_t
c_ll = C.c_longlong


class ConvGeom(C.Structure):
    _fields_ = [(n, C.c_int) for n in ('N', 'Ci', 'H', 'W', 'Co', 'Ho', 'Wo',
                                       'KH', 'KW', 'SH', 'SW', 'PH', 'PW', 'c_split')]


class Dropout(C.Structure):
    _fields_ = [('mask', C.c_void_p), ('step', C.c_void_p), ('seed', C.c_ulonglong), ('offset', C.c_ulonglong),
                ('p', C.c_float)]


_GP = C.POINTER(ConvGeom)
_DP = C.POINTER(Dropout)
_PP = C.POINTER(C.c_void_p)
_IP = C.POINTER(C.c_int)

SIGNATURES = {
    'dynmm_abi_version': (c_i, []),
    'dynmm_build_info': (C.c_char_p, []),
    'dynmm_debug_set_igemm_v5': (c_i, [c_i]),
    'dynmm_conv2d_uses_operand_ring': (c_i, [_GP, c_i]),
    'dynmm_packed_weight_floats': (c_sz, [c_i, c_i, c_i, c_i, c_i]),
    'dynmm_pack_weight': (c_i, [c_f, c_f, c_f, c_i, c_i, c_i, c_i, c_f]),
    'dynmm_pack_weight_multi': (c_i, [c_f, c_f, c_f, c_i, c_i, c_f]),
    'dynmm_pack_weight_multi_blocks': (c_i, [c_i] * 5),
    'dynmm_conv2d_fwd': (c_i, [c_f, c_f, c_f, c_f, c_f, c_f, c_f, _GP, c_i, c_f]),
    'dynmm_conv2d_stem_fwd_stats_supported': (c_i, [_GP]),
    'dynmm_conv2d_stem_fwd_stats': (c_i, [c_f, c_f, c_f, c_f, c_f, _GP, c_f]),
    'dynmm_conv2d_dgrad': (c_i, [c_f, c_f, c_f, c_f, c_f, c_f, _GP, c_f]),
    'dynmm_conv2d_wino_supported': (c_i, [_GP, c_i]),
    'dynmm_wino_packed_floats': (c_sz, [c_i, c_i, c_i, c_i]),
    'dynmm_wino_pack': (c_i, [c_f, c_f, c_f, c_i, c_i, c_i, c_i, c_i, c_f]),
    'dynmm_wino_pack_multi_blocks': (c_i, [c_i] * 4),
    'dynmm_wino_pack_multi': (c_i, [c_f, c_f, c_f, c_i, c_i, c_f]),
    'dynmm_conv2d_wino_fwd': (c_i, [c_f, c_f, c_f, c_f, c_f, _GP, c_i, c_f]),
    'dynmm_conv2d_wino_dgrad_bnred_supported': (c_i, [_GP]),
    'dynmm_conv2d_wino_dgrad_bnred_slots': (c_i, [_GP]),
    'dynmm_conv2d_wino_dgrad_bnred': (c_i, [c_f] * 9 + [_GP, c_f]),
    'dynmm_conv2d_wino_dgrad_bnred2': (c_i, [c_f] * 9 + [_GP, c_f]),
    'dynmm_conv2d_wino_fwd_stats_supported': (c_i, [_GP]),
    'dynmm_conv2d_wino_fwd_stats_slots': (c_i, [_GP]),
    'dynmm_conv2d_wino_fwd_stats': (c_i, [c_f, c_f, c_f, c_f, c_f, c_i, _GP, c_f]),
    'dynmm_conv2d_wino_dgrad': (c_i, [c_f, c_f, c_f, c_f, c_f, _GP, c_f]),
    'dynmm_conv2d_wino2d_supported': (c_i, [_GP, c_i]),
    'dynmm_wino2d_packed_floats': (c_sz, [c_i, c_i]),
    'dynmm_wino2d_pack': (c_i, [c_f, c_f, c_f, c_i, c_i, c_i, c_f]),
    'dynmm_wino2d_pack_multi_blocks': (c_i, [c_i, c_i, c_i]),
    'dynmm_wino2d_pack_multi': (c_i, [c_f, c_f, c_f, c_i, c_i, c_f]),
    'dynmm_conv2d_wino2d_stats_slots': (c_i, [_GP]),
    'dynmm_conv2d_wino2d_fwd': (c_i, [c_f, c_f, c_f, c_f, c_f, c_f, c_i, _GP, c_i, c_f]),
    'dynmm_conv2d_wino2d_dgrad': (c_i, [c_f, c_f, c_f, c_f, c_f, _GP, c_f]),
    'dynmm_conv2d_wino43_supported': (c_i, [_GP]),
    'dynmm_wino43_packed_floats': (c_sz, [c_i, c_i, c_i, c_i]),
    'dynmm_wino43_pack': (c_i, [c_f, c_f, c_i, c_i, c_i, c_i, c_f]),
    'dynmm_wino43_pack_multi_blocks': (c_i, [c_i] * 4),
    'dynmm_wino43_pack_multi': (c_i, [c_f, c_f, c_f, c_i, c_i, c_f]),
    'dynmm_conv2d_wino43_dgrad': (c_i, [c_f, c_f, c_f, c_f, c_f, _GP, c_f]),
    'dynmm_conv2d_wgrad_workspace_bytes': (c_sz, [_GP]),
    'dynmm_conv2d_wgrad': (c_i, [c_f, c_f, c_f, c_f, c_f, c_f, c_sz, _GP, c_f]),
    'dynmm_conv2d_wgrad_groupable': (c_i, [_GP]),
    'dynmm_conv2d_wgrad_variant': (c_i, [_GP]),
    'dynmm_conv2d_wgrad_group_workspace_bytes': (c_sz, [_GP, c_i]),
    'dynmm_conv2d_wgrad_group': (c_i, [c_i, c_f, c_f, c_f, c_f, c_f, c_sz, _GP, c_f]),
    'dynmm_act_bwd_bias_workspace_bytes': (c_sz, [c_i, c_i]),
    'dynmm_act_bwd_bias': (c_i, [c_f, c_f, c_f, c_f, c_f, c_i, c_i, c_i, c_i, c_f]),
    'dynmm_act_pre_fwd': (c_i, [c_f, c_f, c_i, c_i, c_i, c_i, c_f]),
    'dynmm_act_pre_bwd': (c_i, [c_f, c_f, c_f, c_f, c_f, c_i, c_i, c_i, c_i, c_f]),
    'dynmm_bn_stats': (c_i, [c_f, c_f, c_i, c_i, c_i, c_i, c_f]),
    'dynmm_bn_stats_f64': (c_i, [c_f, c_f, c_i, c_i, c_i, c_i, c_f]),
    'dynmm_bn_relu_bits_words': (c_sz, [c_i, c_i, c_i]),
    'dynmm_bn_apply': (c_i, [c_f] * 11 + [c_i, c_i, c_i, c_fl, c_fl, c_i, c_i, c_f, c_f]),
    'dynmm_bn_bwd_reduce': (c_i, [c_f] * 8 + [c_i, c_i, c_i, c_i, c_i, c_f, c_f]),
    'dynmm_bn_bwd_apply': (c_i, [c_f] * 12 + [c_i, c_i, c_i, c_i, c_i, c_f, c_f]),
    'dynmm_bn_bwd_reduce_pre': (c_i, [c_f] * 8 + [c_i, c_i, c_i, c_i, c_i, c_f]),
    'dynmm_bn_bwd_apply_pre': (c_i, [c_f] * 12 + [c_i, c_i, c_i, c_i, c_i, c_f]),
    'dynmm_bn_fold': (c_i, [c_f] * 7 + [c_i, c_fl, c_f]),
    'dynmm_maxpool3x3s2_fwd': (c_i, [c_f, c_f, c_f] + [c_i] * 6 + [c_f]),
    'dynmm_maxpool3x3s2_bwd': (c_i, [c_f, c_f, c_f] + [c_i] * 6 + [c_f]),
    'dynmm_adaptive_avgpool_fwd': (c_i, [c_f, c_f] + [c_i] * 5 + [c_f]),
    'dynmm_adaptive_avgpool_bwd': (c_i, [c_f, c_f] + [c_i] * 5 + [c_f]),
    'dynmm_nearest_into_fwd': (c_i, [c_f, c_f] + [c_i] * 8 + [c_f]),
    'dynmm_nearest_into_bwd': (c_i, [c_f, c_f] + [c_i] * 8 + [c_f]),
    'dynmm_upsample2x_dw3x3_fwd': (c_i, [c_f] * 5 + [c_i] * 4 + [c_f]),
    'dynmm_upsample2x_dw3x3_bwd_workspace_bytes': (c_sz, [c_i, c_i]),
    'dynmm_upsample2x_dw3x3_bwd': (c_i, [c_f] * 7 + [c_i] * 4 + [c_f]),
    'dynmm_upsample2x_fwd': (c_i, [c_f] * 3 + [c_i] * 5 + [c_f]),
    'dynmm_upsample2x_bwd': (c_i, [c_f] * 2 + [c_i] * 5 + [c_f]),
    'dynmm_upsample2x_dw3x3_rep_fwd': (c_i, [c_f] * 5 + [c_i] * 4 + [c_f]),
    'dynmm_upsample2x_dw3x3_rep_bwd': (c_i, [c_f] * 7 + [c_i] * 4 + [c_f]),
    'dynmm_bilinear_into_fwd': (c_i, [c_f, c_f] + [c_i] * 8 + [c_f]),
    'dynmm_bilinear_into_bwd': (c_i, [c_f, c_f] + [c_i] * 8 + [c_f]),
    'dynmm_gap2_fwd': (c_i, [c_f] * 4 + [c_i, c_i, c_f]),
    'dynmm_se_coeff_fwd_act': (c_i, [c_f, c_f, _PP, c_f, c_i] + [c_f] * 6 + [c_i, c_i, c_i, c_i, c_f]),
    'dynmm_se_coeff_bwd_act': (c_i, [c_f] * 4 + [_PP, c_f, c_i] + [c_f] * 4 + [_PP, c_f, c_f, c_f, c_i, c_f, c_i, c_i, c_i, c_i, c_f]),
    'dynmm_se_coeff_bwd_workspace_bytes': (c_sz, [c_i, c_i]),
    'dynmm_axpby_fwd': (c_i, [c_f] * 5 + [c_i, c_i, c_f]),
    'dynmm_axpby_bwd_reduce': (c_i, [c_f] * 5 + [c_i, c_i, c_f]),
    'dynmm_axpby_bwd_apply': (c_i, [c_f] * 5 + [c_fl, c_f, c_f, c_i, c_i, c_f]),
    'dynmm_axpby_pool_supported': (c_i, [c_i, c_i]),
    'dynmm_axpby_pool_fwd': (c_i, [c_f] * 9 + [c_i] * 4 + [c_f]),
    'dynmm_axpby_pool_bwd_reduce': (c_i, [c_f] * 7 + [c_i] * 4 + [c_f]),
    'dynmm_stem_bn_bwd_reduce': (c_i, [c_f] * 6 + [c_fl] + [c_f] * 6 + [c_i] * 5 + [c_f]),
    'dynmm_stem_bn_bwd_apply': (c_i, [c_f] * 6 + [c_fl] + [c_f] * 9 + [c_i] * 4 + [c_f]),
    'dynmm_gap2_bnrelu_fwd': (c_i, [c_f] * 3 + [c_i] + [c_f] * 2 + [c_i] * 2 + [c_f]),
    'dynmm_bn_finalize': (c_i, [c_f] * 10 + [c_i] * 3 + [c_fl, c_fl, c_f]),
    'dynmm_axpby_pool_bwd_apply': (c_i, [c_f] * 8 + [C.c_float] + [c_f] * 2 + [c_i] * 3 + [c_f]),
    'dynmm_se1_coeff_fwd': (c_i, [c_f, _PP, c_f, c_f, c_i, c_i, c_i, c_f]),
    'dynmm_se1_coeff_bwd_workspace_bytes': (c_sz, [c_i, c_i]),
    'dynmm_se1_coeff_bwd': (c_i, [c_f, c_f, _PP, c_f, c_f, _PP, c_f, c_f, c_i, c_i, c_i, c_f]),
    'dynmm_se1_scale_fwd': (c_i, [c_f] * 3 + [c_i, c_i, c_f]),
    'dynmm_se1_scale_bwd_reduce': (c_i, [c_f] * 3 + [c_i, c_i, c_f]),
    'dynmm_se1_scale_bwd_apply': (c_i, [c_f] * 3 + [c_fl, c_f, c_i, c_i, c_f]),
    'dynmm_se1_scale_pool_supported': (c_i, [c_i, c_i]),
    'dynmm_se1_scale_pool_fwd': (c_i, [c_f] * 4 + [c_i] * 3 + [c_f]),
    'dynmm_se1_scale_pool_bwd_reduce': (c_i, [c_f] * 4 + [c_i] * 3 + [c_f]),
    'dynmm_se1_scale_pool_bwd_apply': (c_i, [c_f] * 4 + [c_fl, c_f] + [c_i] * 3 + [c_f]),
    'dynmm_reweigh_fwd_act': (c_i, [c_f, c_f, _PP, c_f, c_i, c_f, c_i, c_f, C.c_ulonglong, C.c_ulonglong, c_fl, c_i]
                              + [c_f] * 6 + [c_i, c_i, c_i, c_f]),
    'dynmm_reweigh_bwd_act': (c_i, [c_f] * 5 + [_PP, c_f, c_i, c_f, c_f, c_f, _PP, c_f, c_f, c_f, c_f, c_f, c_fl, c_i, c_i, c_i,
                                    c_f]),
    'dynmm_reweigh_bwd_workspace_bytes': (c_sz, [c_i, c_i]),
    'dynmm_gate_head_fwd': (c_i, [c_f] * 8 + [c_i, c_i, c_fl, c_i, c_i, c_f]),
    'dynmm_gate_decide': (c_i, [c_f] * 5 + [c_i, c_f]),
    'dynmm_gate_head_bwd': (c_i, [c_f] * 9 + [c_i, c_i, c_fl, c_f]),
    'dynmm_ce2d_fwd': (c_i, [c_f] * 4 + [c_i, c_i, c_i, c_i, c_f]),
    'dynmm_up2ce_fwd': (c_i, [c_f] * 7 + [c_i] * 5 + [c_f]),
    'dynmm_up2ce_bwd_workspace_bytes': (c_sz, [c_i] * 4),
    'dynmm_up2ce_bwd': (c_i, [c_f] * 11 + [c_i] * 4 + [c_f]),
    'dynmm_loss_head': (c_i, [c_f, c_i, c_f, c_fl, c_fl, c_f, c_f, c_f, c_f, c_f]),
    'dynmm_ce2d_valid': (c_i, [c_f] * 4 + [c_i, c_i, c_i, c_f]),
    'dynmm_ce2d_bwd': (c_i, [c_f] * 5 + [c_i, c_i, c_i, c_f]),
    'dynmm_eval_confusion': (c_i, [c_f, c_f, c_f] + [c_i] * 6 + [c_f]),
    'dynmm_batch_gather': (c_i, [c_f, c_f, c_f, c_i, c_sz, c_f]),
    'dynmm_batch_merge': (c_i, [c_f, c_f, c_f, c_f, c_i, c_sz, c_f]),
    'dynmm_add_n': (c_i, [_PP, c_i, c_f, c_sz, c_f]),
    'dynmm_reduce_slabs': (c_i, [c_f, c_f, c_i, c_i, c_f]),
    'dynmm_opt_tick': (c_i, [c_f, c_f]),
    'dynmm_sgd_nesterov': (c_i, [c_f, c_f, c_f, c_sz, c_sz, c_f, c_fl, c_fl, c_f, c_f, c_f, c_f]),
    'dynmm_adam': (c_i, [c_f, c_f, c_f, c_f, c_sz, c_sz, c_f, c_f, c_fl, c_fl, c_f, c_f, c_i, c_f, c_f]),
    'dynmm_layernorm_fwd': (c_i, [c_f] * 7 + [c_i, c_i, c_i, c_fl, c_f]),
    'dynmm_layernorm_bwd': (c_i, [c_f] * 9 + [c_i, c_i, c_i, c_f]),
    'dynmm_moe_blend_bwd': (c_i, [c_f, c_f, c_f, _PP, c_i, c_f, c_fl, _PP, c_f, c_i, c_f]),
    'dynmm_mha_fwd': (c_i, [c_f, c_f, c_f, c_i, c_i, c_i, c_i, c_f]),
    'dynmm_mha_bwd': (c_i, [c_f, c_f, c_f, c_f, c_i, c_i, c_i, c_i, c_f]),
    'dynmm_dropout_apply': (c_i, [c_f, c_f, c_sz, _DP, c_f]),
    'dynmm_layernorm_drop_fwd': (c_i, [c_f] * 7 + [c_i, c_i, c_i, c_fl, _DP, c_f]),
    'dynmm_layernorm_drop_bwd': (c_i, [c_f] * 10 + [c_i, c_i, c_i, _DP, c_f]),
    'dynmm_layernorm_bwd_workspace_bytes': (c_sz, [c_i, c_i, c_i]),
    'dynmm_layernorm_drop_bwd_ws': (c_i, [c_f] * 10 + [c_i, c_i, c_i, _DP, c_f, c_sz, c_f]),
    'dynmm_layernorm_parts_fwd': (c_i, [c_f, c_i] + [c_f] * 8 + [c_i, c_i, c_i, c_fl, _DP, c_f]),
    'dynmm_ffn_supported': (c_i, [c_i] * 4),
    'dynmm_ffn_nsplit': (c_i, [c_i] * 4),
    'dynmm_ffn_fwd': (c_i, [c_f] * 6 + [c_i] * 5 + [_DP, c_f]),
    'dynmm_ffn_bwd_data': (c_i, [c_f] * 6 + [c_i] * 5 + [c_fl, c_f]),
    'dynmm_mha_drop_fwd': (c_i, [c_f, c_f, c_f, c_i, c_i, c_i, c_i, _DP, c_f]),
    'dynmm_mha_drop_bwd': (c_i, [c_f, c_f, c_f, c_f, c_i, c_i, c_i, c_i, _DP, c_f]),
    'dynmm_moe_head': (c_i, [c_f, _PP, c_i, c_f, c_fl, c_i, c_fl, c_f, c_f, c_f, _PP, c_f, c_i, c_f]),
    'dynmm_clip_grad_norm_workspace_bytes': (c_sz, []),
    'dynmm_clip_grad_norm': (c_i, [c_f, c_sz, c_fl, c_f, c_f, c_f]),
    'dynmm_maxout_bn_fwd': (c_i, [c_f] * 9 + [c_i, c_i, c_i, c_fl, c_fl, c_i, _DP, c_f]),
    'dynmm_maxout_bn_bwd': (c_i, [c_f] * 8 + [c_i, c_i, c_i, c_i, _DP, c_f]),
    'dynmm_ml_head': (c_i, [c_f, _PP, c_i, c_i, c_f, c_fl, c_i, c_fl, c_f, c_f, c_f, _PP, c_f, c_i, c_f]),
    'dynmm_ml_blend_bwd': (c_i, [c_f, c_f, c_f, _PP, c_i, c_i, c_f, c_fl, _PP, c_f, c_i, c_f]),
    'dynmm_ml_counts': (c_i, [c_f, c_f, c_i, c_i, c_f, c_f, c_f]),
    'dynmm_ml_partition': (c_i, [c_f, c_i, c_i, c_f, c_f, c_f, c_f]),
    'dynmm_posneg_counts': (c_i, [c_f, c_i, c_f, c_i, c_f, C.c_double, c_i, c_f, c_f, c_f]),
    'dynmm_head_loss': (c_i, [c_f, c_f, c_i, c_i, c_i, c_f, c_f, c_f, c_f]),
    'dynmm_gru_packed_floats': (c_sz, [c_i]),
    'dynmm_gru_pack': (c_i, [c_f, c_f, c_i, c_f]),
    'dynmm_gru_arm': (c_i, [c_i, c_i, c_i]),
    'dynmm_gru_bwd_workspace_bytes': (c_sz, [c_i, c_i]),
    'dynmm_gru_seq_fwd': (c_i, [c_f] * 7 + [c_i] * 4 + [c_f]),
    'dynmm_gru_seq_bwd': (c_i, [c_f] * 9 + [c_sz] + [c_i] * 4 + [c_f]),
    'dynmm_lrtf_fwd_workspace_bytes': (c_sz, [c_i, c_i, c_i]),
    'dynmm_lrtf_fwd': (c_i, [_PP, _PP, _IP, c_i, c_f, c_f, c_f, c_f, c_sz, c_i, c_i, c_i, c_f]),
    'dynmm_lrtf_bwd_workspace_bytes': (c_sz, [c_i, _IP, c_i, c_i, c_i]),
    'dynmm_lrtf_bwd': (c_i, [c_f, _PP, _PP, _IP, c_i, c_f, _PP, _PP, c_f, c_f, c_f, c_sz, c_i, c_i, c_i, c_f]),
    'dynmm_mim_fwd_workspace_bytes': (c_sz, [c_i] * 4),
    'dynmm_mim_fwd': (c_i, [c_f] * 8 + [c_sz] + [c_i] * 4 + [c_f]),
    'dynmm_mim_bwd_workspace_bytes': (c_sz, [c_i] * 4),
    'dynmm_mim_bwd': (c_i, [c_f] * 13 + [c_sz] + [c_i] * 4 + [c_f]),
    'dynmm_attn_supported': (c_i, [c_i, c_i, c_i]),
    'dynmm_attn_fwd': (c_i, [c_f, c_f, c_f, c_i, c_i, c_i, c_i, _DP, c_f]),
    'dynmm_attn_bwd': (c_i, [c_f, c_f, c_f, c_f, c_i, c_i, c_i, c_i, _DP, c_f]),
    'dynmm_xattn_supported': (c_i, [c_i] * 4),
    'dynmm_xattn_fwd': (c_i, [c_f] * 3 + [c_ll] * 3 + [c_f, c_f] + [c_i] * 6 + [_DP, c_f]),
    'dynmm_xattn_bwd': (c_i, [c_f] * 4 + [c_ll] * 3 + [c_f] * 4 + [c_ll] * 3 + [c_i] * 6 + [_DP, c_f]),
    'dynmm_posembed_fwd': (c_i, [c_f] * 4 + [c_i] * 3 + [c_fl, _DP, _DP, c_f]),
    'dynmm_posembed_bwd': (c_i, [c_f] * 3 + [c_i] * 3 + [c_fl, _DP, _DP, c_f]),
    'dynmm_prenorm_fwd': (c_i, [c_f] * 8 + [c_i] * 3 + [c_fl, _DP, c_f]),
    'dynmm_prenorm_bwd_workspace_bytes': (c_sz, [c_i, c_i, c_i]),
    'dynmm_prenorm_bwd': (c_i, [c_f] * 10 + [c_i] * 3 + [_DP, c_i, c_f, c_sz, c_f]),
    'dynmm_rgbd_aug': (c_i, [c_f, c_f, c_f] + [c_i] * 3 + [c_f, c_f] + [c_i] * 3 + [c_fl, c_fl, c_i] + [c_f] * 7),
}

ABI_VERSION = 5
_lib = None


class DynmmHipError(RuntimeError):
    pass


def build(force=False):
    if force and os.path.exists(LIB_PATH):
        os.remove(LIB_PATH)
    subprocess.run(['make', '-C', CSRC, '-j8'], check=True)
    if not os.path.exists(LIB_PATH):
        raise DynmmHipError(f'build did not produce {LIB_PATH}')
    return LIB_PATH


def load():
    global _lib
    if _lib is not None:
        return _lib
    if not os.path.exists(LIB_PATH):
        raise DynmmHipError(
            f'{LIB_PATH} not found: the HIP extension is required (no CPU/PyTorch fallback). '
            'Build it with `python -c "import __graft_entry__ as g; g.build()"` or `make -C dynmm_amd/csrc`.')
    import torch
    lib = C.CDLL(LIB_PATH)
    runtimes = _mapped_hip_runtimes()
    if len(runtimes) > 1:
        raise DynmmHipError(f'two HIP runtimes are mapped in this process: {sorted(runtimes)}; '
                            'import torch before anything that links libamdhip64')
    for name, (res, args) in SIGNATURES.items():
        fn = getattr(lib, name)
        fn.restype = res
        fn.argtypes = args
    if lib.dynmm_abi_version() != ABI_VERSION:
        raise DynmmHipError('libdynmm_hip.so ABI version mismatch')
    _lib = lib
    return lib


def _mapped_hip_runtimes():
    try:
        with open('/proc/self/maps') as f:
            return {ln.split()[-1] for ln in f if 'libamdhip64' in ln}
    except OSError:
        return set()


def check(status, what):
    if status != 0:
        if status <= -1000:
            raise DynmmHipError(f'{what}: HIP error {-(status + 1000)}')
        raise DynmmHipError(f'{what}: status {status} '
                            f'({ {-1: "EINVAL", -2: "EUNSUPPORTED", -3: "EWORKSPACE"}.get(status, "?") })')
```

dynmm_amd/ops.py:

```python
import collections
import contextlib
import ctypes as C

import torch
from torch.autograd import Function

from . import lib as L

ACT = L.ACT


def _lib():
    return L.load()


def _stream():
    if not torch.cuda.is_available():
        raise L.DynmmHipError('no HIP device is available: the DynMM hot path runs only on its HIP kernels '
                              '(there is no CPU / eager-PyTorch fallback)')
    h = torch.cuda.current_stream().cuda_stream
    _CENSUS.add(h)
    return h


def _p(t):
    return None if t is None else t.data_ptr()


def _chk(t, name='tensor'):
    if t is None:
        return None
    if not t.is_cuda:
        raise L.DynmmHipError(f'{name} is on {t.device}: the DynMM HIP path needs a HIP (cuda) device; '
                              'there is no CPU fallback')
    if t.dtype != torch.float32:
        raise L.DynmmHipError(f'{name} must be float32, got {t.dtype}')
    return t if t.is_contiguous() else t.contiguous()


def _operand(op, t, name, shape=None):
    if not torch.is_tensor(t):
        raise L.DynmmHipError(f'{op}: {name} must be a tensor, got {type(t).__name__}')
    _chk(t, name)
    if not t.is_contiguous():
        raise L.DynmmHipError(f'{op}: {name} must be contiguous, got strides {tuple(t.stride())} for {tuple(t.shape)}')
    if shape is not None and tuple(t.shape) != tuple(shape):
        raise L.DynmmHipError(f'{op}: {name} must be {tuple(shape)}, got {tuple(t.shape)}')
    return t


WINO = 'all'
WINO_DGRAD = '43h'
CONV_BN_STATS = True
_WINO_OK = {}
_WINO43_OK = {}


def _wino43(g):
    if WINO_DGRAD == '23' or g.KW != 3:
        return False
    key = (g.N, g.Ci, g.H, g.W, g.Co, g.KH, g.KW, g.SH, g.SW, g.PH, g.PW, g.c_split)
    ok = _WINO43_OK.get(key)
    if ok is None:
        ok = _WINO43_OK[key] = bool(_lib().dynmm_conv2d_wino43_supported(C.byref(g)))
    return ok


_WINO2D_OK = {}


def _wino2d(g, dgrad, x2=None, infer=False):
    if WINO == '0' or x2 is not None or g.KH != 3 or g.KW != 3:
        return False
    if not infer and ((WINO == 'dgrad' and not dgrad) or (WINO == 'fwd' and dgrad)):
        return False
    key = (g.N, g.Ci, g.H, g.W, g.Co, g.SH, g.SW, g.PH, g.PW, g.c_split, bool(dgrad))
    ok = _WINO2D_OK.get(key)
    if ok is None:
        ok = _WINO2D_OK[key] = bool(_lib().dynmm_conv2d_wino2d_supported(C.byref(g), int(bool(dgrad))))
    return ok


def _wino(g, dgrad, x2=None, infer=False):
    if WINO == '0' or x2 is not None:
        return False
    if not infer and ((WINO == 'dgrad' and not dgrad) or (WINO == 'fwd' and dgrad)):
        return False
    key = (g.N, g.Ci, g.H, g.W, g.Co, g.KH, g.KW, g.SH, g.SW, g.PH, g.PW, g.c_split, bool(dgrad))
    ok = _WINO_OK.get(key)
    if ok is None:
        ok = _WINO_OK[key] = int(_lib().dynmm_conv2d_wino_supported(C.byref(g), int(bool(dgrad))))
    return ok


_FWD_KIND = {'direct': 'fwd', 'wino': 'wino_fwd', 'wino2d': 'wino2d_fwd'}
_DGRAD_KIND = {'direct': 'dgrad', 'wino': 'wino_dgrad', 'wino_s2': 'wino_dgrad_s2', 'wino43': 'wino43_dgrad',
               'wino2d': 'wino2d_dgrad'}
_WINO_F23 = ('wino', 'wino_s2')


def _fwd_route(g, x2, aligned, infer=False):
    if not aligned:
        return 'direct'
    if _wino2d(g, False, x2, infer):
        return 'wino2d'
    return 'wino' if _wino(g, False, x2, infer) else 'direct'


def _dgrad_route(g, x2):
    if _wino2d(g, True, x2):
        return 'wino2d'
    w = _wino(g, True, x2)
    if not w:
        return 'direct'
    if _wino43(g):
        return 'wino43'
    return 'wino_s2' if w == 2 else 'wino'


_WINO_PACK_ARG = {'wino_fwd': 0, 'wino_dgrad': 1, 'wino_dgrad_s2': 2}
_WINO2D_PACK_ARG = {'wino2d_fwd': 0, 'wino2d_dgrad': 1}


def _pack_operands(weight, g, kinds, scale=None):
    lib, st, dims = _lib(), _stream(), (g.Co, g.Ci, g.KH, g.KW)
    out = {}

    def new(kind, n):
        out[kind] = torch.empty(n, device=weight.device, dtype=torch.float32)
        return out[kind].data_ptr()
    if 'fwd' in kinds or 'dgrad' in kinds:
        wp = new('fwd', lib.dynmm_packed_weight_floats(*dims, 0)) if 'fwd' in kinds else None
        wpd = new('dgrad', lib.dynmm_packed_weight_floats(*dims, 1)) if 'dgrad' in kinds else None
        L.check(lib.dynmm_pack_weight(_p(weight), wp, wpd, *dims, st), 'pack_weight')
    for kind in kinds:
        if kind in _WINO_PACK_ARG:
            L.check(lib.dynmm_wino_pack(_p(weight), new(kind, lib.dynmm_wino_packed_floats(*dims)), _p(scale), *dims,
                                        _WINO_PACK_ARG[kind], st), 'wino_pack')
        elif kind == 'wino43_dgrad':
            L.check(lib.dynmm_wino43_pack(_p(weight), new(kind, lib.dynmm_wino43_packed_floats(*dims)), *dims, st), 'wino43_pack')
        elif kind in _WINO2D_PACK_ARG:
            L.check(lib.dynmm_wino2d_pack(_p(weight), new(kind, lib.dynmm_wino2d_packed_floats(g.Co, g.Ci)), _p(scale), g.Co, g.Ci,
                                          _WINO2D_PACK_ARG[kind], st), 'wino2d_pack')
    return out


WGRAD_STREAMS = 2
_WGRAD_RR = [0]


MAX_BUSY_STREAMS = 4
VERIFY_STREAM_PLAN = True
_PLANS = {}
_HIP_RT = []
_CENSUS = set()


def _hip_runtime():
    if not _HIP_RT:
        mapped = sorted(L._mapped_hip_runtimes())
        hip = C.CDLL(mapped[0]) if len(mapped) == 1 else None
        if hip is not None:
            hip.hipDeviceGetStreamPriorityRange.argtypes = [C.POINTER(C.c_int), C.POINTER(C.c_int)]
            hip.hipDeviceGetStreamPriorityRange.restype = C.c_int
            hip.hipStreamCreateWithPriority.argtypes = [C.POINTER(C.c_void_p), C.c_uint, C.c_int]
            hip.hipStreamCreateWithPriority.restype = C.c_int
            hip.hipStreamGetPriority.argtypes = [C.c_void_p, C.POINTER(C.c_int)]
            hip.hipStreamGetPriority.restype = C.c_int
        _HIP_RT.append(hip)
    return _HIP_RT[0]


def _runtime_stream(device, least_priority):
    hip = _hip_runtime()
    with torch.cuda.device(device):
        torch.cuda.current_stream()
        if hip is None:
            return torch.cuda.Stream(device=device), None
        prio = 0
        if least_priority:
            least, greatest = C.c_int(0), C.c_int(0)
            if hip.hipDeviceGetStreamPriorityRange(C.byref(least), C.byref(greatest)) != 0 or least.value <= 0:
                return torch.cuda.Stream(device=device), None
            prio = least.value
        h = C.c_void_p()
        if hip.hipStreamCreateWithPriority(C.byref(h), 1, prio) != 0 or not h.value:
            return torch.cuda.Stream(device=device), None
        return torch.cuda.ExternalStream(h.value, device=device), h


class _StreamPlan:
    def __init__(self, device):
        if torch.cuda.is_current_stream_capturing():
            raise L.DynmmHipError('the stream plan must exist before a stream capture starts (hipStreamCreate is not '
                                  'capturable): build engine.TrainStep / call ops.stream_plan() first')
        self.device = device
        self.handles = []
        self.side = self._make(False)
        self.wgrad = [self._make(True) for _ in range(max(1, WGRAD_STREAMS))]
        self.report = {'checked': False}
        if VERIFY_STREAM_PLAN:
            self.verify()

    def _make(self, least_priority):
        s, h = _runtime_stream(self.device, least_priority)
        if h is not None:
# ... 463 lines not shown
                rows.append([src, dstf, dstd, Co | (Ci << 32), (KH * KW) | (blk << 32)])
                span['fwd'] = (dstf, nf)
                if nd:
                    span['dgrad'] = (dstd, ndg)
                blk += lib.dynmm_pack_weight_multi_blocks(Co, Ci, KH, KW, int(nd))
            for kind, dgrad in _WINO_PACK_ARG.items():
                if kind in kinds:
                    nu = lib.dynmm_wino_packed_floats(Co, Ci, KH, KW)
                    wrows.append([src, off, Co | (Ci << 32), KH | (KW << 8) | (dgrad << 16) | (wblk << 32)])
                    span[kind] = (off, nu)
                    off += nu
                    wblk += lib.dynmm_wino_pack_multi_blocks(Co, Ci, KH, KW)
            if 'wino43_dgrad' in kinds:
                nu43 = lib.dynmm_wino43_packed_floats(Co, Ci, KH, KW)
                w43rows.append([src, off, Co | (Ci << 32), KH | (KW << 8) | (w43blk << 32)])
                span['wino43_dgrad'] = (off, nu43)
                off += _up4(nu43)
                w43blk += lib.dynmm_wino43_pack_multi_blocks(Co, Ci, KH, KW)
            for kind, dgrad in _WINO2D_PACK_ARG.items():
                if kind in kinds:
                    nu2 = lib.dynmm_wino2d_packed_floats(Co, Ci)
                    w2rows.append([src, off, Co | (Ci << 32), (dgrad << 16) | (w2blk << 32)])
                    span[kind] = (off, nu2)
                    off += nu2
                    w2blk += lib.dynmm_wino2d_pack_multi_blocks(Co, Ci, dgrad)
        self.arena = torch.empty(off, device=dev, dtype=torch.float32)
        self.base = base
        self.launches = [(name, torch.tensor(r, dtype=torch.int64).to(dev), len(r), b) for name, r, b in
                         (('pack_weight_multi', rows, blk), ('wino_pack_multi', wrows, wblk), ('wino43_pack_multi', w43rows, w43blk),
                          ('wino2d_pack_multi', w2rows, w2blk)) if r]
        self.slots = {k: {kind: self.arena[o:o + n] for kind, (o, n) in span.items()} for k, span in spans.items()}
        self.dirty = False

    def pack(self):
        self.valid = False
        if not self.reg:
            return
        if self.dirty or self.arena is None:
            if torch.cuda.is_current_stream_capturing():
                return
            self._layout()
        for name, desc, n, blocks in self.launches:
            L.check(getattr(_lib(), 'dynmm_' + name)(C.c_void_p(self.base), _p(self.arena), desc.data_ptr(), n, blocks, _stream()), name)
        self.valid = True

    def invalidate(self):
        self.valid = False


def _planes(t):
    if t.dim() >= 2:
        return t.shape[0], t.shape[1], max(t.numel() // max(t.shape[0] * t.shape[1], 1), 1)
    return 1, max(t.numel(), 1), 1


class _Activation(Function):

    @staticmethod
    def forward(ctx, z, act):
        z = _chk(z, 'z')
        a = torch.empty_like(z)
        if z.numel():
            N, Cc, HW = _planes(z)
            L.check(_lib().dynmm_act_pre_fwd(_p(z), _p(a), N, Cc, HW, act, _stream()), 'act_pre_fwd')
        ctx.act = act
        ctx.save_for_backward(z)
        return a

    @staticmethod
    def backward(ctx, g):
        z, = ctx.saved_tensors
        g = _chk(g, 'grad')
        dz = torch.empty_like(z)
        if z.numel():
            N, Cc, HW = _planes(z)
            L.check(_lib().dynmm_act_pre_bwd(_p(g), _p(z), _p(dz), None, None, N, Cc, HW, ctx.act, _stream()), 'act_pre_bwd')
        return dz, None


def is_smooth(act):
    return ACT[act] in L.SMOOTH_ACTS


def activation(x, act):
    code = ACT[act]
    if code == L.ACT_NONE:
        return x
    if not (torch.is_grad_enabled() and x.requires_grad):
        x = _chk(x, 'x')
        a = torch.empty_like(x)
        if x.numel():
            N, Cc, HW = _planes(x)
            L.check(_lib().dynmm_act_pre_fwd(_p(x), _p(a), N, Cc, HW, code, _stream()), 'act_pre_fwd')
        return a
    return _Activation.apply(x, code)


class _Conv2d(Function):
    @staticmethod
    def forward(ctx, x, x2, weight, bias, stride, padding, act, mask_input, defer_mask, link, w_owner=None, stats=None,
                bn_link=None):
        lib = _lib()
        st = _stream()
        x, x2, weight, bias = _chk(x, 'x'), _chk(x2, 'x2'), _chk(weight, 'weight'), _chk(bias, 'bias')
        g = _geom(x, x2, weight, stride, padding)
        need_dx = ctx.needs_input_grad[0] or (x2 is not None and ctx.needs_input_grad[1])
        y = torch.empty((g.N, g.Co, g.Ho, g.Wo), device=x.device, dtype=torch.float32)
        fwd = _fwd_route(g, x2, x.data_ptr() % 16 == 0)
        dgrad = _dgrad_route(g, x2) if need_dx else None
        kinds = (_FWD_KIND[fwd], _DGRAD_KIND[dgrad]) if need_dx else (_FWD_KIND[fwd],)
        wkey = w_owner if w_owner is not None else weight
        prepack = _STEP.prepack if _STEP is not None else None
        packed = prepack.lookup(wkey, kinds) if prepack is not None else None
        if packed is None:
            packed = _pack_operands(weight, g, kinds)
            if prepack is not None:
                prepack.register(wkey, g, kinds)
        wf = packed[kinds[0]]
        if fwd == 'wino2d':
            sums, ns = None, 0
            if stats is not None and act == L.ACT_NONE and g.Co % 64 == 0:
                ns = lib.dynmm_conv2d_wino2d_stats_slots(C.byref(g))
                stats['sums'] = sums = _zeroed_sums(2 * g.Co * ns, x.device)
            L.check(_timed('fwd', g, lambda: lib.dynmm_conv2d_wino2d_fwd(_p(x), _p(wf), _p(bias), None, _p(y), _p(sums), ns,
                                                                         C.byref(g), act, st), route=fwd), 'conv2d_wino2d_fwd')
        elif (fwd == 'wino' and stats is not None and act == L.ACT_NONE and g.KW == 3 and
                lib.dynmm_conv2d_wino_fwd_stats_supported(C.byref(g))):
            ns = lib.dynmm_conv2d_wino_fwd_stats_slots(C.byref(g))
            sums = _zeroed_sums(2 * g.Co * ns, x.device)
            L.check(_timed('fwd', g, lambda: lib.dynmm_conv2d_wino_fwd_stats(_p(x), _p(wf), _p(bias), _p(y), _p(sums), ns,
                                                                             C.byref(g), st), route=fwd), 'conv2d_wino_fwd_stats')
            stats['sums'] = sums
        elif fwd == 'wino':
            L.check(_timed('fwd', g, lambda: lib.dynmm_conv2d_wino_fwd(_p(x), _p(wf), _p(bias), None, _p(y), C.byref(g), act, st),
                           route=fwd), 'conv2d_wino_fwd')
        elif (stats is not None and act == L.ACT_NONE and x2 is None and
                lib.dynmm_conv2d_stem_fwd_stats_supported(C.byref(g))):
            sums = _zeroed_sums(2 * g.Co, x.device)
            L.check(_timed('fwd', g, lambda: lib.dynmm_conv2d_stem_fwd_stats(_p(x), _p(wf), _p(bias), _p(y), _p(sums),
                                                                             C.byref(g), st)), 'conv2d_stem_fwd_stats')
            stats['sums'] = sums
        else:
            L.check(_timed('fwd', g, lambda: lib.dynmm_conv2d_fwd(_p(x), _p(x2), _p(wf), None, _p(bias), None, _p(y),
                                                                  C.byref(g), act, st)), 'conv2d_fwd')
        ctx.geom = g
        ctx.act = act
        ctx.has_bias = bias is not None
        ctx.has_x2 = x2 is not None
        ctx.dgrad_route = dgrad
        ctx.mask_input = mask_input
        ctx.defer_mask = defer_mask
        ctx.link = link
        ctx.bn_link = bn_link
        ctx.save_for_backward(x, x2, packed[kinds[1]] if need_dx else None, y if (act != L.ACT_NONE and not defer_mask) else None)
        ctx.wshape = tuple(weight.shape)
        ctx.w_param, ctx.b_param = (w_owner if w_owner is not None else weight), bias
        return y

    @staticmethod
    def backward(ctx, gy):
        lib = _lib()
        st = _stream()
        x, x2, wpd, y = ctx.saved_tensors
        g = ctx.geom
        gy = _chk(gy, 'grad')
        dbias = None
        act = L.ACT_NONE if ctx.defer_mask else ctx.act
        dbias_ret = None
        bias_in_wgrad = ctx.has_bias and ctx.needs_input_grad[2]
        defer = (ctx.needs_input_grad[2] and x2 is None and
                 _wgrad_grouped(g, ctx.w_param, *([ctx.b_param] if ctx.has_bias else [])))
        if ctx.has_bias and not (defer and bias_in_wgrad):
            dbias, dbias_ret = _grad_dst(ctx.b_param)
        if act != L.ACT_NONE or (ctx.has_bias and not bias_in_wgrad):
            ge = torch.empty_like(gy) if act != L.ACT_NONE else None
            wsb = None
            if not bias_in_wgrad and dbias is not None:
                nb = lib.dynmm_act_bwd_bias_workspace_bytes(g.N, g.Co)
                wsb = torch.empty(max(nb // 4, 1), device=gy.device, dtype=torch.float32)
            L.check(lib.dynmm_act_bwd_bias(_p(gy), _p(y), _p(ge), None if bias_in_wgrad else _p(dbias), _p(wsb),
                                           g.N, g.Co, g.Ho * g.Wo, act, st), 'act_bwd_bias')
            if ge is not None:
                gy = ge
        dx = dx2 = None
        if wpd is not None:
            dx = torch.empty_like(x)
            dx2 = torch.empty_like(x2) if x2 is not None else None
            mask = x if ctx.mask_input else None
            accum = None
            if ctx.link is not None and ctx.link.dres is not None:
                accum, ctx.link.dres = ctx.link.dres, None
            extra = (mask is not None) + (accum is not None)
            route = ctx.dgrad_route
            if route != 'direct':
                gyw = gy if gy.data_ptr() % 16 == 0 else gy.clone()
                mask, accum = (t if (t is None or t.data_ptr() % 16 == 0) else t.clone() for t in (mask, accum))
                bl = ctx.bn_link
                if (bl is not None and bl.x is not None and bl.bits is not None and route in _WINO_F23 and mask is None and
                        (ctx.link is None) == (accum is None) and
                        bl.x.data_ptr() % 8 == 0 and (g.H * g.W) % 4 == 0 and
                        lib.dynmm_conv2d_wino_dgrad_bnred_supported(C.byref(g))):
                    sums = _zeroed_sums(2 * g.Ci * lib.dynmm_conv2d_wino_dgrad_bnred_slots(C.byref(g)), dx.device)
                    L.check(_timed('dgrad', g, lambda: lib.dynmm_conv2d_wino_dgrad_bnred2(
                        _p(gyw), _p(wpd), _p(accum), _p(bl.x), _p(bl.bits), _p(bl.mean), _p(bl.invstd), _p(sums), _p(dx),
                        C.byref(g), st), extra=2, route=route), 'conv2d_wino_dgrad_bnred2')
                    bl.sums, bl.premasked = sums, True
                elif (bl is not None and bl.x is not None and bl.bits is None and route in _WINO_F23 and mask is None and
                        accum is None and
                        bl.x.data_ptr() % 8 == 0 and lib.dynmm_conv2d_wino_dgrad_bnred_supported(C.byref(g))):
                    sums = _zeroed_sums(2 * g.Ci * lib.dynmm_conv2d_wino_dgrad_bnred_slots(C.byref(g)), dx.device)
                    L.check(_timed('dgrad', g, lambda: lib.dynmm_conv2d_wino_dgrad_bnred(
                        _p(gyw), _p(wpd), _p(bl.x), _p(bl.mean), _p(bl.invstd), _p(bl.gamma), _p(bl.beta), _p(sums), _p(dx),
                        C.byref(g), st), extra=1, route=route), 'conv2d_wino_dgrad_bnred')
                    bl.sums = sums
                else:
                    fn = {'wino2d': lib.dynmm_conv2d_wino2d_dgrad, 'wino43': lib.dynmm_conv2d_wino43_dgrad}.get(route, lib.dynmm_conv2d_wino_dgrad)
                    L.check(_timed('dgrad', g, lambda: fn(_p(gyw), _p(wpd), _p(mask), _p(accum), _p(dx), C.byref(g), st),
                                   extra=extra, route=route), 'conv2d_wino_dgrad')
            else:
                L.check(_timed('dgrad', g, lambda: lib.dynmm_conv2d_dgrad(_p(gy), _p(wpd), _p(mask), _p(accum), _p(dx),
                                                                          _p(dx2), C.byref(g), st), extra=extra), 'conv2d_dgrad')
        dw_ret = None
        ws_stream = None
        _age_wgrad_queues()
        if defer:
            _queue_wgrad(g, x, gy, ctx.w_param, ctx.b_param if bias_in_wgrad else None)
        elif ctx.needs_input_grad[2]:
            dw, dw_ret = _grad_dst(ctx.w_param)
            nbytes = lib.dynmm_conv2d_wgrad_workspace_bytes(C.byref(g))
            if dw_ret is None and _STEP.async_wgrad and PROFILE is None:
                ws_stream = _wgrad_stream()
                _CENSUS.add(ws_stream.cuda_stream)
                ws_stream.wait_stream(torch.cuda.current_stream())
                with torch.cuda.stream(ws_stream):
                    ws = torch.empty(max(nbytes // 4, 1), device=gy.device, dtype=torch.float32)
                    L.check(lib.dynmm_conv2d_wgrad(_p(x), _p(x2), _p(gy), _p(dw), _p(dbias) if bias_in_wgrad else None,
                                                   _p(ws), nbytes, C.byref(g), ws_stream.cuda_stream), 'conv2d_wgrad')
                _STEP.inflight.append((x, x2, gy))
            else:
                ws = torch.empty(max(nbytes // 4, 1), device=gy.device, dtype=torch.float32)
                L.check(_timed('wgrad', g, lambda: lib.dynmm_conv2d_wgrad(_p(x), _p(x2), _p(gy), _p(dw),
                                                                          _p(dbias) if bias_in_wgrad else None, _p(ws), nbytes,
                                                                          C.byref(g), st)), 'conv2d_wgrad')
        _grads_enqueued(torch.cuda.current_stream(), ws_stream)
        if dw_ret is not None and tuple(dw_ret.shape) != ctx.wshape:
            dw_ret = dw_ret.reshape(ctx.wshape)
        return dx, dx2, dw_ret, dbias_ret, None, None, None, None, None, None, None, None, None


def conv2d(x, weight, bias=None, stride=1, padding=0, act=None, x2=None, mask_input=False, defer_mask=False,
           link=None, w_owner=None, bn_stats=False, bn_link=None):
    if is_smooth(act) and (torch.is_grad_enabled() or not isinstance(weight, torch.nn.Parameter) or w_owner is not None):
        z = conv2d(x, weight, bias, stride, padding, None, x2, link=link, w_owner=w_owner)
        return activation(z, act)
    if not torch.is_grad_enabled() and isinstance(weight, torch.nn.Parameter) and w_owner is None:
        return conv2d_fused_eval(x, weight, bias, None, act, None, stride, padding, x2)
    holder = {} if (bn_stats and CONV_BN_STATS and x2 is None) else None
    y = _Conv2d.apply(x, x2, weight, bias, _pair(stride), _pair(padding), ACT[act], bool(mask_input),
                      bool(defer_mask), link, w_owner, holder, bn_link if BN_BWD_FUSE else None)
    if holder:
        y._bn_sums = holder['sums']
    if ACT_TRACE is not None and ACT[act] == L.ACT_RELU:
        ACT_TRACE.append(y.detach())
    return y


class _FanOut(Function):

    @staticmethod
    def forward(ctx, x, n):
        return tuple(x.view_as(x) for _ in range(n))

    @staticmethod
    def backward(ctx, *gs):
        gs = [_chk(g, 'grad') for g in gs if g is not None]
        if not gs:
            return None, None
        if len(gs) == 1:
            return gs[0], None
        out = torch.empty_like(gs[0])
        while len(gs) > 1:
            take, gs = gs[:4], gs[4:]
            dst = out if not gs else torch.empty_like(out)
            L.check(_lib().dynmm_add_n(_ptr_array(take), len(take), _p(dst), C.c_size_t(dst.numel()), _stream()), 'add_n')
            gs = [dst] + gs
        return out, None


_NO_FANOUT = False


def fan_out(x, n):
    if n <= 1 or _NO_FANOUT or not (torch.is_grad_enabled() and x.requires_grad):
        return (x,) * n
    return _FanOut.apply(x, n)


_MUTATION_GEN = [0]


def note_mutation():
    _MUTATION_GEN[0] += 1


CAPTURE_EVAL_CACHE = False
_EVAL_CACHE = {'direct': '_dynmm_eval_cache', 'wino': '_dynmm_eval_cache_wino', 'wino2d': '_dynmm_eval_cache_wino2d'}


def conv2d_fused_eval(x, weight, conv_bias, bn, act=None, residual=None, stride=1, padding=0, x2=None):
    lib = _lib()
    st = _stream()
    x, x2, weight = _chk(x, 'x'), _chk(x2, 'x2'), _chk(weight, 'weight')
    residual = _chk(residual, 'residual')
    g = _geom(x, x2, weight, _pair(stride), _pair(padding))
    dev = x.device
    srcs = [weight, conv_bias] + ([bn.weight, bn.bias, bn.running_mean, bn.running_var] if bn is not None else [])
    route = _fwd_route(g, x2, x.data_ptr() % 16 == 0 and (residual is None or residual.data_ptr() % 8 == 0), infer=True)
    slot = _EVAL_CACHE[route]
    stamp = (_MUTATION_GEN[0],) + tuple((t.data_ptr(), t._version) for t in srcs if t is not None) + \
        ((float(bn.eps),) if bn is not None else ())
    hit = getattr(weight, slot, None)
    if hit is not None and hit[0] == stamp and (CAPTURE_EVAL_CACHE or not torch.cuda.is_current_stream_capturing()):
        wp, scale, shift = hit[1]
    else:
        scale = shift = None
        if bn is not None:
            scale = torch.empty(g.Co, device=dev, dtype=torch.float32)
            shift = torch.empty(g.Co, device=dev, dtype=torch.float32)
            L.check(lib.dynmm_bn_fold(_p(bn.weight), _p(bn.bias), _p(bn.running_mean), _p(bn.running_var),
                                      _p(conv_bias), _p(scale), _p(shift), g.Co, bn.eps, st), 'bn_fold')
        else:
            shift = _chk(conv_bias, 'bias')
        kind = _FWD_KIND[route]
        wp = _pack_operands(weight, g, (kind,), scale)[kind]
        if route != 'direct':
            scale = None
        if not torch.cuda.is_current_stream_capturing():
            setattr(weight, slot, (stamp, (wp, scale, shift)))
    y = torch.empty((g.N, g.Co, g.Ho, g.Wo), device=dev, dtype=torch.float32)
    if route == 'wino2d':
        L.check(_timed('fwd', g, lambda: lib.dynmm_conv2d_wino2d_fwd(_p(x), _p(wp), _p(shift), _p(residual), _p(y), None, 0, C.byref(g),
                                                                     ACT[act], st), extra=int(residual is not None), route=route),
                'conv2d_wino2d_fwd')
    elif route == 'wino':
        L.check(_timed('fwd', g, lambda: lib.dynmm_conv2d_wino_fwd(_p(x), _p(wp), _p(shift), _p(residual), _p(y), C.byref(g),
                                                                   ACT[act], st), extra=int(residual is not None), route=route),
                'conv2d_wino_fwd')
    else:
        L.check(_timed('fwd', g, lambda: lib.dynmm_conv2d_fwd(_p(x), _p(x2), _p(wp), _p(scale), _p(shift), _p(residual),
                                                              _p(y), C.byref(g), ACT[act], st),
                       extra=int(residual is not None)), 'conv2d_fwd')
    return y


_ARENA = {'buf': None, 'off': 0, 'elems': 1 << 19}


def begin_step():
    a = _ARENA
    if a['buf'] is not None and a['off'] > 0:
        a['buf'][:a['off']].zero_()
    a['off'] = 0


def _zero_sums(n, device):
    a = _ARENA
    if a['buf'] is None or a['buf'].device != device:
        if torch.cuda.is_current_stream_capturing():
            return torch.empty(n, device=device, dtype=torch.float64), 0
        a['buf'] = torch.zeros(a['elems'], device=device, dtype=torch.float64)
        a['off'] = 0
    if a['off'] + n > a['elems']:
        return torch.empty(n, device=device, dtype=torch.float64), 0
    t = a['buf'][a['off']:a['off'] + n]
    a['off'] += n
    return t, 1


def _zeroed_sums(n, device):
    sums, zeroed = _zero_sums(n, device)
    if not zeroed:
        sums.zero_()
    return sums


class _BatchNormAct(Function):
    @staticmethod
    def forward(ctx, x, gamma, beta, running_mean, running_var, residual, training, momentum, eps, act, link, nbt, pre_sums=None,
                bwd_link=None):
        lib = _lib()
        st = _stream()
        x, residual = _chk(x, 'x'), _chk(residual, 'residual')
        _same_shape(x, residual, 'batch_norm residual')
        N, Cc, H, W = x.shape
        HW = H * W
        dev = x.device
# ... 383 lines not shown
            raise L.DynmmHipError(f'rgb/depth fusion: shape mismatch {tuple(rgb.shape)} vs {tuple(depth.shape)}')
        HW = H * W
        wc_ptr, wc_stride = None, 0
        if wcum is not None:
            wcum = _chk(wcum, 'wcum')
            wc_stride = wcum.shape[1]
            wc_ptr = wcum.data_ptr() + 4 * col
        params, a, b, saved = _se2_excite(
            lib, st, lambda sr, sd: L.check(lib.dynmm_gap2_fwd(_p(rgb), _p(depth), _p(sr), _p(sd), n_act * Cc, HW, st), 'gap2'),
            params, use_se, se_act, n_act, Cc, rgb.device, wc_ptr, wc_stride)
        if inplace and n_act < N:
            out = rgb
            ctx.mark_dirty(rgb)
        else:
            out = torch.empty_like(rgb)
            _copy_rows(rgb, out, n_act, N - n_act)
        L.check(lib.dynmm_axpby_fwd(_p(rgb), _p(depth), _p(a), _p(b), _p(out), n_act * Cc, HW, st), 'axpby_fwd')
        ctx.use_se = use_se
        ctx.se_act = se_act
        ctx.col = col
        ctx.param_objs = params
        ctx.save_for_backward(rgb, depth, wcum, a, b, *saved, *params)
        return out

    @staticmethod
    def backward(ctx, g):
        lib = _lib()
        st = _stream()
        rgb, depth, wcum, a, b = ctx.saved_tensors[:5]
        saved, params = ctx.saved_tensors[5:11], list(ctx.saved_tensors[11:])
        g = _chk(g, 'grad')
        N, Cc, H, W = rgb.shape
        n_act = depth.shape[0]
        HW = H * W
        f32 = dict(device=g.device, dtype=torch.float32)
        da, db = torch.empty((n_act, Cc), **f32), torch.empty((n_act, Cc), **f32)
        L.check(lib.dynmm_axpby_bwd_reduce(_p(g), _p(rgb), _p(depth), _p(da), _p(db), n_act * Cc, HW, st), 'axpby_bwd_reduce')
        dwcum = None
        wc_ptr, wc_stride, dwc_ptr = None, 0, None
        if wcum is not None:
            wc_stride = wcum.shape[1]
            wc_ptr = wcum.data_ptr() + 4 * ctx.col
            if ctx.needs_input_grad[2]:
                dwcum = torch.zeros_like(wcum)
                dwc_ptr = dwcum.data_ptr() + 4 * ctx.col
        dsr, dsd, dparams_ret = _se2_excite_bwd(lib, st, ctx, da, db, saved, params, wc_ptr, wc_stride, dwc_ptr)
        drgb, ddepth = torch.empty_like(rgb), torch.empty_like(depth)
        L.check(lib.dynmm_axpby_bwd_apply(_p(g), _p(a), _p(b), _p(dsr), _p(dsd), 1.0 / HW,
                                          _p(drgb), _p(ddepth), n_act * Cc, HW, st), 'axpby_bwd_apply')
        _copy_rows(g, drgb, n_act, N - n_act)
        _grads_enqueued()
        return (drgb, ddepth, dwcum, None, None, None, None, *dparams_ret)


class _SEFusePool(Function):

    @staticmethod
    def forward(ctx, rgb, depth, use_se, se_act, *params):
        lib = _lib()
        st = _stream()
        rgb, depth = _chk(rgb, 'rgb'), _chk(depth, 'depth')
        _same_shape(rgb, depth, 'stem fusion')
        N, Cc, H, W = rgb.shape
        params, a, b, saved = _se2_excite(
            lib, st, lambda sr, sd: L.check(lib.dynmm_gap2_fwd(_p(rgb), _p(depth), _p(sr), _p(sd), N * Cc, H * W, st), 'gap2'),
            params, use_se, se_act, N, Cc, rgb.device)
        yo, yd, io, idd = _fuse_pool_fwd(lib, st, rgb, depth, a, b, None)
        ctx.use_se = use_se
        ctx.se_act = se_act
        ctx.param_objs = params
        ctx.save_for_backward(rgb, depth, a, b, *saved, io, idd, *params)
        return yo, yd

    @staticmethod
    def backward(ctx, g_o, g_d):
        lib = _lib()
        st = _stream()
        rgb, depth, a, b = ctx.saved_tensors[:4]
        saved, (io, idd), params = ctx.saved_tensors[4:10], ctx.saved_tensors[10:12], list(ctx.saved_tensors[12:])
        N, Cc, H, W = rgb.shape
        HW = H * W
        f32 = dict(device=rgb.device, dtype=torch.float32)
        g_o = torch.zeros_like(io, dtype=torch.float32) if g_o is None else _chk(g_o, 'grad')
        g_d = torch.zeros_like(io, dtype=torch.float32) if g_d is None else _chk(g_d, 'grad')
        da, db = torch.empty((N, Cc), **f32), torch.empty((N, Cc), **f32)
        L.check(lib.dynmm_axpby_pool_bwd_reduce(_p(g_o), io.data_ptr(), _p(rgb), _p(depth), _p(da), _p(db), None, Cc,
                                                N * Cc, H, W, st), 'axpby_pool_bwd_reduce')
        dsr, dsd, dparams_ret = _se2_excite_bwd(lib, st, ctx, da, db, saved, params)
        drgb, ddepth = torch.empty_like(rgb), torch.empty_like(depth)
        L.check(lib.dynmm_axpby_pool_bwd_apply(_p(g_o), io.data_ptr(), _p(g_d), idd.data_ptr(), _p(a), _p(b), _p(dsr), _p(dsd),
                                               1.0 / HW, _p(drgb), _p(ddepth), N * Cc, H, W, st), 'axpby_pool_bwd_apply')
        _grads_enqueued()
        return (drgb, ddepth, None, None, *dparams_ret)


class _StemBNFusePool(Function):

    @staticmethod
    def forward(ctx, xr, xd, gam_r, bet_r, rm_r, rv_r, nbt_r, gam_d, bet_d, rm_d, rv_d, nbt_d, mom_r, eps_r, mom_d,
                eps_d, use_se, pre_r, pre_d, slots, *params):
        lib = _lib()
        st = _stream()
        xr, xd = _chk(xr, 'x_rgb'), _chk(xd, 'x_depth')
        _same_shape(xr, xd, 'stem fusion')
        N, Cc, H, W = xr.shape
        HW = H * W
        dev = xr.device
        f32 = dict(device=dev, dtype=torch.float32)
        if N * HW <= 1:
            raise ValueError(f'Expected more than 1 value per channel when training, got input size {tuple(xr.shape)}')
        note_mutation()
        tr = torch.empty((4, Cc), **f32)
        stats = torch.empty((4, Cc), **f32)
        for k, (x, gam, bet, rm, rv, nbt, mom, eps, pre) in enumerate(((xr, gam_r, bet_r, rm_r, rv_r, nbt_r, mom_r, eps_r, pre_r),
                                                                       (xd, gam_d, bet_d, rm_d, rv_d, nbt_d, mom_d, eps_d, pre_d))):
            if pre is not None:
                sums = pre
            else:
                sums, zeroed = _zero_sums(2 * Cc, dev)
                L.check(lib.dynmm_bn_stats(_p(x), _p(sums), N, Cc, HW, zeroed, st), 'bn_stats')
            L.check(lib.dynmm_bn_finalize(_p(sums), _p(gam), _p(bet), _p(rm), _p(rv), _p(stats[2 * k]), _p(stats[2 * k + 1]),
                                          _p(nbt), _p(tr[2 * k]), _p(tr[2 * k + 1]), N, Cc, HW, eps, mom, st), 'bn_finalize')
        ctx.se_act = ACT['relu']
        params, a, b, saved = _se2_excite(
            lib, st, lambda sr, sd: L.check(lib.dynmm_gap2_bnrelu_fwd(_p(xr), _p(xd), _p(tr), Cc, _p(sr), _p(sd), N * Cc, HW, st),
                                            'gap2_bnrelu'),
            params, use_se, ctx.se_act, N, Cc, dev)
        yo, yd, io, idd = _fuse_pool_fwd(lib, st, xr, xd, a, b, tr)
        ctx.use_se = use_se
        ctx.param_objs = params
        ctx.bn_params = (gam_r, bet_r, gam_d, bet_d)
        ctx.slots = slots
        ctx.save_for_backward(xr, xd, tr, stats, a, b, *saved, io, idd, gam_r, bet_r, gam_d, bet_d, *params)
        return yo, yd

    @staticmethod
    def backward(ctx, g_o, g_d):
        lib = _lib()
        st = _stream()
        xr, xd, tr, stats, a, b = ctx.saved_tensors[:6]
        saved, (io, idd, gam_r, bet_r, gam_d, bet_d) = ctx.saved_tensors[6:12], ctx.saved_tensors[12:18]
        params = list(ctx.saved_tensors[18:])
        N, Cc, H, W = xr.shape
        HW = H * W
        dev = xr.device
        f32 = dict(device=dev, dtype=torch.float32)
        g_o = torch.zeros_like(io, dtype=torch.float32) if g_o is None else _chk(g_o, 'grad')
        g_d = torch.zeros_like(io, dtype=torch.float32) if g_d is None else _chk(g_d, 'grad')
        da, db = torch.empty((N, Cc), **f32), torch.empty((N, Cc), **f32)
        L.check(lib.dynmm_axpby_pool_bwd_reduce(_p(g_o), io.data_ptr(), _p(xr), _p(xd), _p(da), _p(db), _p(tr), Cc,
                                                N * Cc, H, W, st), 'axpby_pool_bwd_reduce')
        dsr, dsd, dparams_ret = _se2_excite_bwd(lib, st, ctx, da, db, saved, params)
        _grads_enqueued()
        def bn_chain(k):
            x, coef, off, gdp, idp, gam, bet, gp, bp = (
                (xr, a, dsr, None, None, gam_r, bet_r, ctx.bn_params[0], ctx.bn_params[1]),
                (xd, b, dsd, g_d, idd, gam_d, bet_d, ctx.bn_params[2], ctx.bn_params[3]))[k]
            stq = _stream()
            mean, invstd = stats[2 * k], stats[2 * k + 1]
            sums, zeroed = _zero_sums(2 * Cc, dev)
            head = (_p(g_o), io.data_ptr(), _p(gdp), None if idp is None else idp.data_ptr(), _p(coef), _p(off), 1.0 / HW,
                    _p(x), _p(mean), _p(invstd), _p(gam), _p(bet))
            L.check(lib.dynmm_stem_bn_bwd_reduce(*head, _p(sums), N, Cc, H, W, zeroed, stq), 'stem_bn_bwd_reduce')
            dgamma, dgamma_ret = _grad_dst(gp)
            dbeta, dbeta_ret = _grad_dst(bp)
            dx = torch.empty_like(x)
            L.check(lib.dynmm_stem_bn_bwd_apply(*head, _p(sums), _p(dx), _p(dgamma), _p(dbeta), N, Cc, H, W, stq),
                    'stem_bn_bwd_apply')
            _grads_enqueued()
            return dx, dgamma_ret, dbeta_ret
        if ctx.slots is not None:
            for k in (0, 1):
                ctx.slots[k]['bwd'] = (lambda k=k: bn_chain(k))
            ph = torch.empty(1, **f32)
            return (ph.expand(xr.shape), ph.expand(xd.shape), *([None] * 18), *dparams_ret)
        (dxr, dgr, dbr), (dxd, dgd, dbd) = bn_chain(0), bn_chain(1)
        return (dxr, dxd, dgr, dbr, None, None, None, dgd, dbd, None, None, None, None, None, None, None, None, None, None, None,
                *dparams_ret)


class _StemBNDeferred(Function):

    @staticmethod
    def forward(ctx, x, gam, bet, slot):
        ctx.slot = slot
        return x.view_as(x)

    @staticmethod
    def backward(ctx, g):
        fn = ctx.slot.pop('bwd', None)
        if fn is None:
            return g, None, None, None
        dx, dgam, dbet = fn()
        return dx, dgam, dbet, None


def stem_bn_defer(x, bn):
    if not (torch.is_grad_enabled() and (x.requires_grad or bn.weight.requires_grad)):
        return x
    slot = {}
    y = _StemBNDeferred.apply(x, bn.weight, bn.bias, slot)
    y._stem_slot = slot
    for attr in ('_bn_sums',):
        if hasattr(x, attr):
            setattr(y, attr, getattr(x, attr))
    return y


def stem_bn_fuse_pool(x_rgb, bn_rgb, x_depth, bn_depth, se_params=None):
    use_se = se_params is not None
    for bn in (bn_rgb, bn_depth):
        nbt = bn.num_batches_tracked
        if nbt.dtype != torch.int64 or not nbt.is_cuda:
            raise L.DynmmHipError('BatchNorm num_batches_tracked must be an int64 tensor on the HIP device')
    pre = []
    for x in (x_rgb, x_depth):
        p = getattr(x, '_bn_sums', None)
        pre.append(p if (p is not None and p.numel() == 2 * x.shape[1]) else None)
    slots = (getattr(x_rgb, '_stem_slot', None), getattr(x_depth, '_stem_slot', None))
    slots = slots if (slots[0] is not None and slots[1] is not None) else None
    return _StemBNFusePool.apply(x_rgb, x_depth, bn_rgb.weight, bn_rgb.bias, bn_rgb.running_mean, bn_rgb.running_var,
                                 bn_rgb.num_batches_tracked, bn_depth.weight, bn_depth.bias, bn_depth.running_mean,
                                 bn_depth.running_var, bn_depth.num_batches_tracked, float(bn_rgb.momentum),
                                 float(bn_rgb.eps), float(bn_depth.momentum), float(bn_depth.eps), use_se, pre[0], pre[1], slots,
                                 *(tuple(se_params) if use_se else ()))


def stem_bn_fuse_supported(h, w, bn_a, bn_b, act='relu'):
    return ACT[act] == L.ACT_RELU and bool(_lib().dynmm_axpby_pool_supported(int(h), int(w))) and \
        bn_a.training and bn_b.training and torch.is_grad_enabled() and bn_a.momentum is not None and \
        bn_b.momentum is not None


def se_fuse_pool_supported(x):
    return x.dim() == 4 and bool(_lib().dynmm_axpby_pool_supported(int(x.shape[2]), int(x.shape[3])))


def se_fuse_pool(rgb, depth, se_params=None, se_act='relu'):
    use_se = se_params is not None
    return _SEFusePool.apply(rgb, depth, use_se, ACT[se_act], *(tuple(se_params) if use_se else ()))


def se_fuse_blend(rgb, depth, se_params=None, wcum=None, col=0, inplace=False, se_act='relu'):
    use_se = se_params is not None
    params = tuple(se_params) if use_se else ()
    return _SEFuseBlend.apply(rgb, depth, wcum, col, use_se, bool(inplace) and not torch.is_grad_enabled(), ACT[se_act], *params)


def _se1_excite(lib, st, x, params, se_act):
    N, Cc, H, W = x.shape
    f32 = dict(device=x.device, dtype=torch.float32)
    s, h, g = torch.empty((N, Cc), **f32), torch.empty((N, Cc // 16), **f32), torch.empty((N, Cc), **f32)
    L.check(lib.dynmm_gap2_fwd(_p(x), None, _p(s), None, N * Cc, H * W, st), 'gap')
    L.check(lib.dynmm_se1_coeff_fwd(_p(s), _ptr_array(params), _p(h), _p(g), N, Cc, se_act, st), 'se1_coeff_fwd')
    return s, h, g


def _se1_excite_bwd(lib, st, ctx, dg, s, h, g, params):
    N, Cc = s.shape
    dparams, dparams_ret = _grad_dsts(ctx.param_objs)
    ds = torch.empty_like(s)
    ws = torch.empty(lib.dynmm_se1_coeff_bwd_workspace_bytes(N, Cc) // 4, device=s.device, dtype=torch.float32)
    L.check(lib.dynmm_se1_coeff_bwd(_p(dg), _p(s), _ptr_array(params), _p(h), _p(g), _ptr_array(dparams), _p(ds), _p(ws),
                                    N, Cc, ctx.se_act, st), 'se1_coeff_bwd')
    return ds, dparams_ret


class _SEScale(Function):

    @staticmethod
    def forward(ctx, x, inplace, se_act, *params):
        lib = _lib()
        st = _stream()
        x = _chk(x, 'x')
        params = [_chk(p, 'se param') for p in params]
        N, Cc, H, W = x.shape
        s, h, g = _se1_excite(lib, st, x, params, se_act)
        if inplace:
            out = x
            ctx.mark_dirty(x)
        else:
            out = torch.empty_like(x)
        L.check(lib.dynmm_se1_scale_fwd(_p(x), _p(g), _p(out), N * Cc, H * W, st), 'se1_scale_fwd')
        ctx.se_act = se_act
        ctx.param_objs = list(params)
        ctx.save_for_backward(x, s, h, g, *params)
        return out

    @staticmethod
    def backward(ctx, gout):
        lib = _lib()
        st = _stream()
        x, s, h, g = ctx.saved_tensors[:4]
        params = list(ctx.saved_tensors[4:])
        gout = _chk(gout, 'grad')
        N, Cc, H, W = x.shape
        HW = H * W
        dg = torch.empty_like(g)
        L.check(lib.dynmm_se1_scale_bwd_reduce(_p(gout), _p(x), _p(dg), N * Cc, HW, st), 'se1_scale_bwd_reduce')
        ds, dparams_ret = _se1_excite_bwd(lib, st, ctx, dg, s, h, g, params)
        dx = torch.empty_like(x)
        L.check(lib.dynmm_se1_scale_bwd_apply(_p(gout), _p(g), _p(ds), 1.0 / HW, _p(dx), N * Cc, HW, st), 'se1_scale_bwd_apply')
        _grads_enqueued()
        return (dx, None, None, *dparams_ret)


class _SEScalePool(Function):

    @staticmethod
    def forward(ctx, x, se_act, *params):
        lib = _lib()
        st = _stream()
        x = _chk(x, 'x')
        params = [_chk(p, 'se param') for p in params]
        N, Cc, H, W = x.shape
        s, h, g = _se1_excite(lib, st, x, params, se_act)
        y = torch.empty((N, Cc, H // 2, W // 2), device=x.device, dtype=torch.float32)
        idx = torch.empty((N, Cc, H // 2, W // 2), device=x.device, dtype=torch.int8)
        L.check(lib.dynmm_se1_scale_pool_fwd(_p(x), _p(g), _p(y), idx.data_ptr(), N * Cc, H, W, st), 'se1_scale_pool_fwd')
        ctx.se_act = se_act
        ctx.param_objs = list(params)
        ctx.save_for_backward(x, s, h, g, idx, *params)
        return y

    @staticmethod
    def backward(ctx, gy):
        lib = _lib()
        st = _stream()
        x, s, h, g, idx = ctx.saved_tensors[:5]
        params = list(ctx.saved_tensors[5:])
        gy = _chk(gy, 'grad')
        if gy.data_ptr() % 16 != 0:
            gy = gy.clone()
        N, Cc, H, W = x.shape
        dg = torch.empty_like(g)
        L.check(lib.dynmm_se1_scale_pool_bwd_reduce(_p(gy), idx.data_ptr(), _p(x), _p(dg), N * Cc, H, W, st),
                'se1_scale_pool_bwd_reduce')
        ds, dparams_ret = _se1_excite_bwd(lib, st, ctx, dg, s, h, g, params)
        dx = torch.empty_like(x)
        L.check(lib.dynmm_se1_scale_pool_bwd_apply(_p(gy), idx.data_ptr(), _p(g), _p(ds), 1.0 / (H * W), _p(dx), N * Cc, H, W, st),
                'se1_scale_pool_bwd_apply')
        _grads_enqueued()
        return (dx, None, *dparams_ret)


def _se1_params(x, se_params):
    params = tuple(se_params)
    if len(params) != 4:
        raise L.DynmmHipError(f'se_scale: se_params must be the 4 tensors (W1, b1, W2, b2), got {len(params)}')
    if x.dim() != 4 or x.shape[1] % 16 != 0:
        raise L.DynmmHipError(f'se_scale: x must be [N, C, H, W] with C a multiple of 16, got {tuple(x.shape)}')
    return params

# ... 415 lines not shown
```

include/dynmm_hip.h:

```cpp
#ifndef DYNMM_HIP_H
#define DYNMM_HIP_H

#include <stddef.h>

#ifdef __cplusplus
extern "C" {
#endif

#define DYNMM_OK 0
#define DYNMM_EINVAL (-1)
#define DYNMM_EUNSUPPORTED (-2)
#define DYNMM_EWORKSPACE (-3)

#define DYNMM_ACT_NONE 0
#define DYNMM_ACT_RELU 1
#define DYNMM_ACT_TANH 2
#define DYNMM_ACT_SWISH 3
#define DYNMM_ACT_HSWISH 4

#define DYNMM_LOSS_BCE_LOGITS 0
#define DYNMM_LOSS_L1 1

int dynmm_abi_version(void);
const char* dynmm_build_info(void);
// ... 37 lines not shown
                          void* stream);
int dynmm_conv2d_wino_fwd(const float* x, const float* ut, const float* bias, const float* residual, float* y,
                          const dynmm_conv_geom* g, int act, void* stream);
int dynmm_conv2d_wino_dgrad_bnred_supported(const dynmm_conv_geom* g);
int dynmm_conv2d_wino_dgrad_bnred_slots(const dynmm_conv_geom* g);
int dynmm_conv2d_wino_dgrad_bnred(const float* dy, const float* ut, const float* bn_x, const float* bn_mean,
                                  const float* bn_invstd, const float* bn_gamma, const float* bn_beta, double* sums, float* dx,
                                  const dynmm_conv_geom* g, void* stream);
int dynmm_conv2d_wino_dgrad_bnred2(const float* dy, const float* ut, const float* accum, const float* bn_x,
                                   const unsigned long long* relu_bits, const float* bn_mean, const float* bn_invstd,
                                   double* sums, float* dx, const dynmm_conv_geom* g, void* stream);
int dynmm_conv2d_wino_fwd_stats_supported(const dynmm_conv_geom* g);
int dynmm_conv2d_wino_fwd_stats_slots(const dynmm_conv_geom* g);
int dynmm_conv2d_wino_fwd_stats(const float* x, const float* ut, const float* bias, float* y, double* stats, int nslots,
                                const dynmm_conv_geom* g, void* stream);
int dynmm_conv2d_wino_dgrad(const float* dy, const float* ut, const float* mask, const float* accum, float* dx,
                            const dynmm_conv_geom* g, void* stream);

int dynmm_conv2d_wino2d_supported(const dynmm_conv_geom* g, int dgrad);
size_t dynmm_wino2d_packed_floats(int Co, int Ci);
int dynmm_wino2d_pack(const float* w, float* ut, const float* scale, int Co, int Ci, int dgrad, void* stream);
int dynmm_wino2d_pack_multi_blocks(int Co, int Ci, int dgrad);
int dynmm_wino2d_pack_multi(const float* src_base, float* dst_base, const void* desc, int ndesc, int total_blocks, void* stream);
int dynmm_conv2d_wino2d_stats_slots(const dynmm_conv_geom* g);
int dynmm_conv2d_wino2d_fwd(const float* x, const float* ut, const float* bias, const float* residual, float* y, double* stats,
                            int nslots, const dynmm_conv_geom* g, int act, void* stream);
int dynmm_conv2d_wino2d_dgrad(const float* dy, const float* ut, const float* mask, const float* accum, float* dx,
                              const dynmm_conv_geom* g, void* stream);

int dynmm_conv2d_wino43_supported(const dynmm_conv_geom* g);
size_t dynmm_wino43_packed_floats(int Co, int Ci, int KH, int KW);
int dynmm_wino43_pack(const float* w, float* ut, int Co, int Ci, int KH, int KW, void* stream);
int dynmm_wino43_pack_multi_blocks(int Co, int Ci, int KH, int KW);
int dynmm_wino43_pack_multi(const float* src_base, float* dst_base, const void* desc, int ndesc, int total_blocks,
                            void* stream);
int dynmm_conv2d_wino43_dgrad(const float* dy, const float* ut, const float* mask, const float* accum, float* dx,
                              const dynmm_conv_geom* g, void* stream);

size_t dynmm_conv2d_wgrad_workspace_bytes(const dynmm_conv_geom* g);
int dynmm_conv2d_wgrad(const float* x, const float* x2, const float* dy, float* dw, float* dbias,
                       void* workspace, size_t workspace_bytes,
                       const dynmm_conv_geom* g, void* stream);

int dynmm_conv2d_wgrad_groupable(const dynmm_conv_geom* g);
int dynmm_conv2d_wgrad_variant(const dynmm_conv_geom* g);
size_t dynmm_conv2d_wgrad_group_workspace_bytes(const dynmm_conv_geom* g, int n);
int dynmm_conv2d_wgrad_group(int n, const float* const* xs, const float* const* dys, float* const* dws,
                             float* const* dbiases, void* workspace, size_t workspace_bytes,
                             const dynmm_conv_geom* g, void* stream);

size_t dynmm_act_bwd_bias_workspace_bytes(int N, int C);
int dynmm_act_bwd_bias(const float* g, const float* y, float* g_out, float* dbias, float* workspace,
                       int N, int C, int HW, int act, void* stream);

int dynmm_act_pre_fwd(const float* z, float* a, int N, int C, int HW, int act, void* stream);
int dynmm_act_pre_bwd(const float* g, const float* z, float* dz, float* dbias, float* workspace,
                      int N, int C, int HW, int act, void* stream);

int dynmm_bn_stats(const float* x, double* sums, int N, int C, int HW, int sums_are_zero, void* stream);
int dynmm_bn_stats_f64(const float* x, double* sums, int N, int C, int HW, int sums_are_zero, void* stream);
size_t dynmm_bn_relu_bits_words(int N, int C, int HW);
int dynmm_bn_apply(const float* x, const double* sums, const float* gamma, const float* beta,
                   float* running_mean, float* running_var, float* save_mean, float* save_invstd,
                   const float* residual, float* y, long long* num_batches_tracked, int N, int C, int HW,
                   float eps, float momentum, int training, int act, unsigned long long* relu_bits, void* stream);
int dynmm_bn_finalize(const double* sums, const float* gamma, const float* beta, float* running_mean,
                      float* running_var, float* save_mean, float* save_invstd, long long* num_batches_tracked,
                      float* scale, float* shift, int N, int C, int HW, float eps, float momentum, void* stream);
int dynmm_bn_bwd_reduce(const float* g, const float* y, const float* x,
                        const float* mean, const float* invstd, const float* gamma, const float* beta,
                        double* sums, int N, int C, int HW, int act, int sums_are_zero,
                        const unsigned long long* relu_bits, void* stream);
int dynmm_bn_bwd_apply(const float* g, const float* y, const float* x,
                       const float* mean, const float* invstd, const float* gamma, const float* beta,
                       const double* sums, float* dx, float* d_residual,
                       float* dgamma, float* dbeta,
                       int N, int C, int HW, int training, int act, const unsigned long long* relu_bits, void* stream);
int dynmm_bn_bwd_reduce_pre(const float* g, const float* x, const float* residual, const float* mean, const float* invstd,
                            const float* gamma, const float* beta, double* sums, int N, int C, int HW, int act,
                            int sums_are_zero, void* stream);
int dynmm_bn_bwd_apply_pre(const float* g, const float* x, const float* residual, const float* mean, const float* invstd,
                           const float* gamma, const float* beta, const double* sums, float* dx, float* d_residual,
                           float* dgamma, float* dbeta, int N, int C, int HW, int training, int act, void* stream);
int dynmm_bn_fold(const float* gamma, const float* beta, const float* running_mean,
                  const float* running_var, const float* conv_bias, float* scale, float* shift,
                  int C, float eps, void* stream);

int dynmm_maxpool3x3s2_fwd(const float* x, float* y, signed char* idx,
                           int N, int C, int H, int W, int Ho, int Wo, void* stream);
int dynmm_maxpool3x3s2_bwd(const float* g, const signed char* idx, float* dx,
                           int N, int C, int H, int W, int Ho, int Wo, void* stream);
int dynmm_adaptive_avgpool_fwd(const float* x, float* y, int NC, int H, int W, int OH, int OW, void* stream);
int dynmm_adaptive_avgpool_bwd(const float* g, float* dx, int NC, int H, int W, int OH, int OW, void* stream);
int dynmm_nearest_into_fwd(const float* y, float* out, int N, int C, int h, int w,
                           int Ctot, int c_off, int H, int W, void* stream);
int dynmm_nearest_into_bwd(const float* g_out, float* dy, int N, int C, int h, int w,
                           int Ctot, int c_off, int H, int W, void* stream);
int dynmm_upsample2x_dw3x3_fwd(const float* x, const float* w, const float* b, const float* skip,
                               float* y, int N, int C, int H, int W, void* stream);
size_t dynmm_upsample2x_dw3x3_bwd_workspace_bytes(int N, int C);
int dynmm_upsample2x_dw3x3_bwd(const float* g, const float* x, const float* w,
                               float* dx, float* dw, float* db, float* workspace,
                               int N, int C, int H, int W, void* stream);
#define DYNMM_UP_NEAREST 0
#define DYNMM_UP_BILINEAR 1
int dynmm_upsample2x_fwd(const float* x, const float* skip, float* y, int N, int C, int H, int W, int mode, void* stream);
int dynmm_upsample2x_bwd(const float* g, float* dx, int N, int C, int H, int W, int mode, void* stream);
int dynmm_upsample2x_dw3x3_rep_fwd(const float* x, const float* w, const float* b, const float* skip,
                                   float* y, int N, int C, int H, int W, void* stream);
int dynmm_upsample2x_dw3x3_rep_bwd(const float* g, const float* x, const float* w,
                                   float* dx, float* dw, float* db, float* workspace,
                                   int N, int C, int H, int W, void* stream);
int dynmm_bilinear_into_fwd(const float* y, float* out, int N, int C, int h, int w,
                            int Ctot, int c_off, int H, int W, void* stream);
int dynmm_bilinear_into_bwd(const float* g_out, float* dy, int N, int C, int h, int w,
                            int Ctot, int c_off, int H, int W, void* stream);

int dynmm_gap2_fwd(const float* xr, const float* xd, float* sr, float* sd, int NC, int HW, void* stream);
size_t dynmm_se_coeff_bwd_workspace_bytes(int N, int C);
int dynmm_se_coeff_fwd_act(const float* sr, const float* sd, const float* const* params,
                           const float* wc, int wc_stride, float* a, float* b,
                           float* hr, float* hd, float* gr, float* gd,
                           int N, int C, int use_se, int act, void* stream);
int dynmm_se_coeff_bwd_act(const float* da, const float* db, const float* sr, const float* sd,
                           const float* const* params, const float* wc, int wc_stride,
                           const float* hr, const float* hd, const float* gr, const float* gd,
                           float* const* dparams, float* dsr, float* dsd, float* dwc, int dwc_stride,
                           float* workspace, int N, int C, int use_se, int act, void* stream);
int dynmm_axpby_fwd(const float* xr, const float* xd, const float* a, const float* b, float* out,
                    int NC, int HW, void* stream);
int dynmm_axpby_bwd_reduce(const float* g, const float* xr, const float* xd, float* da, float* db,
                           int NC, int HW, void* stream);
int dynmm_axpby_bwd_apply(const float* g, const float* a, const float* b,
                          const float* ca, const float* cb, float cscale, float* dxr, float* dxd,
                          int NC, int HW, void* stream);

int dynmm_axpby_pool_supported(int H, int W);
int dynmm_axpby_pool_fwd(const float* xr, const float* xd, const float* a, const float* b, float* y_out,
                         signed char* idx_out, float* y_depth, signed char* idx_depth, const float* bn_tr, int C,
                         int NC, int H, int W, void* stream);
int dynmm_axpby_pool_bwd_reduce(const float* g_out, const signed char* idx_out, const float* xr, const float* xd,
                                float* da, float* db, const float* bn_tr, int C, int NC, int H, int W, void* stream);
int dynmm_gap2_bnrelu_fwd(const float* xr, const float* xd, const float* bn_tr, int C, float* sr, float* sd, int NC,
                          int HW, void* stream);
int dynmm_stem_bn_bwd_reduce(const float* g_out, const signed char* idx_out, const float* g_depth,
                             const signed char* idx_depth, const float* coef, const float* off, float cscale,
                             const float* x, const float* mean, const float* invstd, const float* gamma,
                             const float* beta, double* sums, int N, int C, int H, int W, int sums_are_zero, void* stream);
int dynmm_stem_bn_bwd_apply(const float* g_out, const signed char* idx_out, const float* g_depth,
                            const signed char* idx_depth, const float* coef, const float* off, float cscale,
                            const float* x, const float* mean, const float* invstd, const float* gamma,
                            const float* beta, const double* sums, float* dx, float* dgamma, float* dbeta,
                            int N, int C, int H, int W, void* stream);
int dynmm_axpby_pool_bwd_apply(const float* g_out, const signed char* idx_out, const float* g_depth,
                               const signed char* idx_depth, const float* a, const float* b, const float* ca,
                               const float* cb, float cscale, float* dxr, float* dxd, int NC, int H, int W, void* stream);

int dynmm_se1_coeff_fwd(const float* s, const float* const* params, float* h, float* g, int N, int C, int act,
                        void* stream);
size_t dynmm_se1_coeff_bwd_workspace_bytes(int N, int C);
int dynmm_se1_coeff_bwd(const float* dg, const float* s, const float* const* params, const float* h, const float* g,
                        float* const* dparams, float* ds, float* workspace, int N, int C, int act, void* stream);
int dynmm_se1_scale_fwd(const float* x, const float* g, float* out, int NC, int HW, void* stream);
int dynmm_se1_scale_bwd_reduce(const float* gout, const float* x, float* dg, int NC, int HW, void* stream);
int dynmm_se1_scale_bwd_apply(const float* gout, const float* g, const float* ds, float cscale, float* dx, int NC, int HW,
                              void* stream);
int dynmm_se1_scale_pool_supported(int H, int W);
int dynmm_se1_scale_pool_fwd(const float* x, const float* g, float* y, signed char* idx, int NC, int H, int W,
                             void* stream);
int dynmm_se1_scale_pool_bwd_reduce(const float* gy, const signed char* idx, const float* x, float* dg, int NC, int H,
                                    int W, void* stream);
int dynmm_se1_scale_pool_bwd_apply(const float* gy, const signed char* idx, const float* g, const float* ds, float cscale,
                                   float* dx, int NC, int H, int W, void* stream);

size_t dynmm_reweigh_bwd_workspace_bytes(int N, int C);
int dynmm_reweigh_fwd_act(const float* sr, const float* sd, const float* const* params,
                          const float* wblend, int blend_mode, const float* prev, int prev_stride,
                          const float* noise, unsigned long long seed, unsigned long long offset,
                          float temp, int hard, float* a, float* b, float* wnext, float* h, float* g,
                          float* aux, int N, int C, int act, void* stream);
int dynmm_reweigh_bwd_act(const float* d_wnext, const float* da, const float* db, const float* sr,
                          const float* sd, const float* const* params, const float* prev, int prev_stride,
                          const float* h, const float* g, const float* aux, float* const* dparams,
                          float* dsr, float* dsd, float* d_wblend, float* d_prev, float* workspace, float temp,
                          int N, int C, int act, void* stream);

int dynmm_gate_head_fwd(const float* pooled, const float* fc, float* weight, float* wcum,
                        float* soft, float* flop_loss, const float* flop_table, const int* force_branch,
                        int N, int J, float temp, int hard, int mode, void* stream);
int dynmm_gate_head_bwd(const float* d_weight, const float* d_wcum, const float* d_loss,
                        const float* pooled, const float* fc, const float* soft,
                        const float* flop_table, float* d_pooled, float* d_fc,
                        int N, int J, float temp, void* stream);

int dynmm_ce2d_fwd(const float* x, const unsigned char* target, const float* cw,
                   double* loss_sum_wsum , int N, int C, int HW, int acc_is_zero, void* stream);
int dynmm_ce2d_valid(const float* x, const unsigned char* target, const float* cw,
                     double* acc4, int N, int C, int HW, void* stream);
int dynmm_loss_head(const double* acc, int S, const float* flop_loss, float ratio, float budget,
                    float* losses, float* total, float* gscale, float* d_flop, void* stream);
int dynmm_ce2d_bwd(const float* x, const unsigned char* target, const float* cw,
                   const float* gscale, float* dx, int N, int C, int HW, void* stream);

int dynmm_up2ce_fwd(const float* x, const float* w, const float* b, const unsigned char* target, const float* cw,
                    float* lse, double* loss_sum_wsum, int N, int C, int H, int W, int acc_is_zero, void* stream);
size_t dynmm_up2ce_bwd_workspace_bytes(int N, int C, int H, int W);
int dynmm_up2ce_bwd(const float* x, const float* w, const float* b, const unsigned char* target, const float* cw,
                    const float* lse, const float* gscale, float* dx, float* dw, float* db, float* workspace,
                    int N, int C, int H, int W, void* stream);

int dynmm_eval_confusion(const float* logits, const unsigned char* label, long long* cm,
                         int N, int C, int H, int W, int Ho, int Wo, void* stream);

int dynmm_batch_gather(const float* src, const int* idx, float* dst, int n_out, size_t row, void* stream);
int dynmm_gate_decide(const float* weight, int* branch, int* order, int* inv, int* counts, int N, void* stream);
int dynmm_batch_merge(const float* base, const float* sub, const int* map, float* out, int N, size_t row,
                      void* stream);

int dynmm_add_n(const float* const* srcs, int n, float* out, size_t numel, void* stream);
int dynmm_reduce_slabs(const float* slabs, float* out, int n, int nslabs, void* stream);
int dynmm_opt_tick(int* step, void* stream);
int dynmm_sgd_nesterov(float* p, const float* g, float* buf, size_t lo, size_t hi, const float* hyper,
                       float weight_decay, float grad_scale, const float* loss, int* nan_flag,
                       const int* step, void* stream);
int dynmm_adam(float* p, const float* g, float* m, float* v, size_t lo, size_t hi, const float* hyper,
               const int* step, float weight_decay, float grad_scale, const float* loss, int* nan_flag,
               int decoupled , const float* grad_scale_dev ,
               void* stream);

int dynmm_layernorm_fwd(const float* x, const float* res, const float* gamma, const float* beta, float* y,
                        float* mean, float* rstd, int B, int D, int T, float eps, void* stream);
int dynmm_layernorm_bwd(const float* g, const float* x, const float* res, const float* gamma, const float* mean,
                        const float* rstd, float* dx, float* dgamma, float* dbeta, int B, int D, int T, void* stream);
int dynmm_mha_fwd(const float* qkv, float* out, float* probs, int B, int D, int T, int heads, void* stream);
int dynmm_mha_bwd(const float* g, const float* qkv, const float* probs, float* dqkv, int B, int D, int T, int heads,
                  void* stream);
typedef struct dynmm_dropout {
    const unsigned char* mask;
    const unsigned long long* step;
    unsigned long long seed, offset;
    float p;
} dynmm_dropout;
int dynmm_dropout_apply(const float* x, float* y, size_t n, const dynmm_dropout* drop, void* stream);
int dynmm_layernorm_drop_fwd(const float* x, const float* res, const float* gamma, const float* beta, float* y,
                             float* mean, float* rstd, int B, int D, int T, float eps, const dynmm_dropout* drop,
                             void* stream);
int dynmm_layernorm_drop_bwd(const float* g, const float* x, const float* res, const float* gamma, const float* mean,
                             const float* rstd, float* dx, float* dres, float* dgamma, float* dbeta, int B, int D, int T,
                             const dynmm_dropout* drop, void* stream);
size_t dynmm_layernorm_bwd_workspace_bytes(int B, int D, int T);
int dynmm_layernorm_drop_bwd_ws(const float* g, const float* x, const float* res, const float* gamma, const float* mean,
                                const float* rstd, float* dx, float* dres, float* dgamma, float* dbeta, int B, int D, int T,
                                const dynmm_dropout* drop, float* workspace, size_t workspace_bytes, void* stream);
int dynmm_layernorm_parts_fwd(const float* parts, int nparts, const float* xbias, float* xsum, const float* res,
                              const float* gamma, const float* beta, float* y, float* mean, float* rstd, int B, int D, int T,
                              float eps, const dynmm_dropout* drop, void* stream);
int dynmm_ffn_supported(int B, int D, int T, int F);
int dynmm_ffn_nsplit(int B, int D, int T, int F);
int dynmm_ffn_fwd(const float* x, const float* w1, const float* b1, const float* w2, float* hidden, float* out_parts, int B,
                  int D, int T, int F, int nsplit, const dynmm_dropout* drop, void* stream);
int dynmm_ffn_bwd_data(const float* dout, const float* hidden, const float* w1, const float* w2, float* dhidden,
                       float* dx_parts, int B, int D, int T, int F, int nsplit, float p, void* stream);
int dynmm_mha_drop_fwd(const float* qkv, float* out, float* probs, int B, int D, int T, int heads,
                       const dynmm_dropout* drop, void* stream);
int dynmm_mha_drop_bwd(const float* g, const float* qkv, const float* probs, float* dqkv, int B, int D, int T, int heads,
                       const dynmm_dropout* drop, void* stream);
int dynmm_moe_head(const float* logits, const float* const* preds, int K, const float* target, float temp, int hard,
                   float reg, float* out, float* weight, float* scalars, float* const* d_preds, float* d_logits, int B,
                   void* stream);
int dynmm_moe_blend_bwd(const float* d_out, const float* d_aux, const float* logits, const float* const* preds, int K,
                        const float* weight, float temp, float* const* d_preds, float* d_logits, int B, void* stream);
size_t dynmm_clip_grad_norm_workspace_bytes(void);
int dynmm_clip_grad_norm(const float* flat_grad, size_t n, float max_norm, double* workspace, float* norm_and_coef,
                         void* stream);

int dynmm_maxout_bn_fwd(const float* z, float* y, float* save_mean, float* save_rstd, float* running_mean, float* running_var,
                        long long* num_batches_tracked, const float* gamma, const float* beta, int B, int M, int maxout,
                        float eps, float momentum, int train, const dynmm_dropout* drop, void* stream);
int dynmm_maxout_bn_bwd(const float* dy, const float* z, const float* save_mean, const float* save_rstd, const float* gamma,
                        float* dz, float* dgamma, float* dbeta, int B, int M, int maxout, int train, const dynmm_dropout* drop,
                        void* stream);
int dynmm_ml_head(const float* logits, const float* const* preds, int K, int C, const float* target, float temp, int hard,
                  float reg, float* out, float* weight, float* scalars, float* const* d_preds, float* d_logits, int B,
                  void* stream);
int dynmm_ml_blend_bwd(const float* d_out, const float* d_aux, const float* logits, const float* const* preds, int K, int C,
                       const float* weight, float temp, float* const* d_preds, float* d_logits, int B, void* stream);
int dynmm_ml_counts(const float* logits, const float* target, int B, int C, int* counts, double* loss_sum, void* stream);
int dynmm_ml_partition(const float* weight, int K, int B, int* order, int* inv, int* counts, void* stream);

int dynmm_posneg_counts(const float* out, int out_stride, const float* y, int B, const float* aux, double lossw, int form,
                        long long* counts, double* loss_acc, void* stream);

int dynmm_head_loss(const float* out, const float* target, int B, int C, int kind, float* loss, float* d_out,
                    double* loss_acc, void* stream);

size_t dynmm_gru_packed_floats(int H);
int dynmm_gru_pack(const float* w_hh, float* packed, int H, void* stream);
int dynmm_gru_arm(int B, int H, int T);
size_t dynmm_gru_bwd_workspace_bytes(int B, int H);
int dynmm_gru_seq_fwd(const float* gi, const float* packed, const float* b_hh, const int* lengths, float* hbuf, float* gates,
                      float* hn, int T, int B, int H, int arm, void* stream);
int dynmm_gru_seq_bwd(const float* d_hn, const float* d_hseq, const float* packed, const int* lengths, const float* hbuf,
                      const float* gates, float* dgi, float* dgh, float* workspace, size_t workspace_bytes, int T, int B, int H,
                      int arm, void* stream);

size_t dynmm_lrtf_fwd_workspace_bytes(int B, int O, int R);
// ... 50 lines not shown
```

Before: 519.1 images/s.

## Fold stem BatchNorm backward apply into stem conv weight-gradient kernel

When the stem conv needs no input gradient, the BN backward apply step (pool backward, coefficient scaling, BN dx) is no longer written to a full dx tensor. The stem wgrad kernel recomputes dy on the fly from pooled gradients, indices and BN statistics while loading its tile, and also writes dgamma/dbeta. This removes one full-resolution write and read of the stem activation gradient plus a kernel launch. In exchange the wgrad kernel does more arithmetic and gathers per tile, and the autograd plumbing uses a placeholder gradient that raises an error if the conv output has another consumer.

```diff
diff --git a/dynmm_amd/csrc/conv_igemm.hip b/dynmm_amd/csrc/conv_igemm.hip
--- a/dynmm_amd/csrc/conv_igemm.hip
+++ b/dynmm_amd/csrc/conv_igemm.hip
@@ -3,6 +3,7 @@
 #include "common.h"
 #include "conv_igemm.h"
 #include "conv_small.h"
+#include "pool.h"
 #include "vec.h"
 
 namespace dynmm {
@@ -1452,6 +1453,31 @@
     return DYNMM_OK;
 }
 
+extern "C" int dynmm_conv2d_stem_wgrad_bn_supported(const dynmm_conv_geom* g) {
+    if (!geom_ok(g)) return 0;
+    return stem_conv_wgrad_bn_eligible(g->Ci, g->Co, g->KH, g->KW, g->SH, g->SW, g->PH, g->PW, g->c_split < g->Ci, g->Ho, g->Wo)
+               ? 1 : 0;
+}
+
+extern "C" int dynmm_conv2d_stem_wgrad_bn(const float* g_out, const signed char* idx_out, const float* g_depth,
+                                          const signed char* idx_depth, const float* coef, const float* off, float cscale,
+                                          const float* y, const float* mean, const float* invstd, const float* gamma,
+                                          const float* beta, const double* sums, float* dgamma, float* dbeta, const float* x,
+                                          float* dw, void* workspace, size_t workspace_bytes, const dynmm_conv_geom* g,
+                                          void* stream) {
+    (void)hipGetLastError();
+    if (!x || !dw || !sums || !geom_ok(g)) return DYNMM_EINVAL;
+    if (!dynmm_conv2d_stem_wgrad_bn_supported(g)) return DYNMM_EUNSUPPORTED;
+    StemBnArgs bn;
+    const int rc = stem_bn_args(bn, g_out, idx_out, g_depth, idx_depth, coef, off, cscale, y, mean, invstd, gamma, beta, g->N,
+                                g->Co, g->Ho, g->Wo);
+    if (rc != DYNMM_OK) return rc;
+    const size_t need = stem_conv_wgrad_workspace_bytes(g->N, g->Ci, g->Ho, g->Wo);
+    if (!workspace || workspace_bytes < need) return DYNMM_EWORKSPACE;
+    return launch_stem_conv_wgrad_bn(x, bn, sums, dgamma, dbeta, dw, (float*)workspace, g->N, g->Ci, g->H, g->W, g->Ho, g->Wo,
+                                     (hipStream_t)stream);
+}
+
 static bool wgrad_v4_shape_ok(const dynmm_conv_geom* g, const WgradPlan& p) {
     if (p.v6) return (g->Co % 4 == 0);
     return g->c_split == g->Ci && p.tco == 128 && p.tk == 128 && (g->Ci % 64 == 0) && g->SW == 1 &&
diff --git a/dynmm_amd/csrc/conv_small.h b/dynmm_amd/csrc/conv_small.h
--- a/dynmm_amd/csrc/conv_small.h
+++ b/dynmm_amd/csrc/conv_small.h
@@ -21,10 +21,15 @@
     int N, H, W, Ho, Wo;
 };
 
+struct StemBnArgs;
+
 bool stem_conv_wgrad_eligible(int Ci, int Co, int KH, int KW, int SH, int SW, int PH, int PW, bool has_x2, bool has_bias);
 size_t stem_conv_wgrad_workspace_bytes(int N, int Ci, int Ho, int Wo);
 int launch_stem_conv_wgrad(const float* x, const float* dy, float* dw, float* workspace, int N, int Ci, int H, int W,
                            int Ho, int Wo, hipStream_t st);
+bool stem_conv_wgrad_bn_eligible(int Ci, int Co, int KH, int KW, int SH, int SW, int PH, int PW, bool has_x2, int Ho, int Wo);
+int launch_stem_conv_wgrad_bn(const float* x, const StemBnArgs& bn, const double* sums, float* dgamma, float* dbeta, float* dw,
+                              float* workspace, int N, int Ci, int H, int W, int Ho, int Wo, hipStream_t st);
 
 bool co8_wgrad_eligible(int Ci, int Co, int H, int W, int Ho, int Wo, int KH, int KW, int SH, int SW, int PH, int PW, int c_split);
 size_t co8_wgrad_workspace_bytes(int N, int Ci, int Co);
diff --git a/dynmm_amd/csrc/conv_small.hip b/dynmm_amd/csrc/conv_small.hip
--- a/dynmm_amd/csrc/conv_small.hip
+++ b/dynmm_amd/csrc/conv_small.hip
@@ -1,6 +1,8 @@
+#include <type_traits>
 #include "common.h"
 #include "conv_small.h"
 #include "conv_igemm.h"
+#include "pool.h"
 
 namespace dynmm {
 
@@ -491,8 +493,16 @@
     }
 }
 
-template <int CI>
-__global__ void __launch_bounds__(256, CI == 1 ? 4 : 2) conv_stem_wgrad_kernel(const StemWgradArgs a) {
+struct StemWgradBnArgs : StemWgradArgs {
+    StemBnArgs bn;
+    const double* sums;
+    float* dgamma;
+    float* dbeta;
+};
+
+template <int CI, bool BNFOLD = false>
+__global__ void __launch_bounds__(256, CI == 1 ? 4 : 2)
+conv_stem_wgrad_kernel(const std::conditional_t<BNFOLD, StemWgradBnArgs, StemWgradArgs> a) {
     constexpr int KS = 7, S = 2, PAD = 3, KW8 = 8;
     constexpr int TRW = 2, TCW = 64, NPX = TRW * TCW;
     constexpr int IR = (TRW - 1) * S + KS;
@@ -503,6 +513,7 @@
     constexpr int PP = NPX + 1;
     __shared__ float patch[CI * IR * ICP];
     __shared__ float dyt[64 * PP];
+    __shared__ float bnc[BNFOLD ? 64 * 6 : 1];
 
     const int lane = threadIdx.x & 63, l31 = lane & 31, khalf = lane >> 5;
     const int wave = threadIdx.x >> 6;
@@ -510,6 +521,22 @@
     const int tw = (a.Wo + TCW - 1) / TCW, th = (a.Ho + TRW - 1) / TRW;
     const int HW = a.H * a.W, HoWo = a.Ho * a.Wo;
     const int tiles = a.N * th * tw;
+    if constexpr (BNFOLD) {
+        if (threadIdx.x < 64) {
+            const int c = threadIdx.x;
+            const float mu = a.bn.mean[c], is = a.bn.invstd[c];
+            const float sc = a.bn.gamma[c] * is;
+            const float sh = fmaf(-mu, sc, a.bn.beta[c]);
+            const float sg = (float)a.sums[c], sgx = (float)a.sums[64 + c];
+            const float invM = 1.f / ((float)a.bn.N * (float)(a.bn.H * a.bn.W));
+            bnc[c * 6 + 0] = sc; bnc[c * 6 + 1] = sh; bnc[c * 6 + 2] = mu; bnc[c * 6 + 3] = is;
+            bnc[c * 6 + 4] = sg * invM; bnc[c * 6 + 5] = sgx * invM;
+            if (blockIdx.x == 0) {
+                if (a.dgamma) a.dgamma[c] = sgx;
+                if (a.dbeta) a.dbeta[c] = sg;
+            }
+        }
+    }
 
     int boff[KPW];
 #pragma unroll
@@ -547,38 +574,78 @@
                 const float v = xn[(size_t)ci * HW + (size_t)min(max(ih, 0), a.H - 1) * a.W + min(max(iw, 0), a.W - 1)];
                 sv[it] = ok ? v : 0.f;
             }
-            float4 dv[8];
-            const float* dn = a.dy + (size_t)n * 64 * HoWo;
-            const bool vec = (a.Wo & 3) == 0;
-#pragma unroll
-            for (int it = 0; it < 8; ++it) {
-                const int i4 = it * 256 + threadIdx.x;
-                const int co = i4 >> 5, q = i4 & 31, r = q >> 4, c4 = (q & 15) * 4;
-                const int oh = oh0 + r, ow = ow0 + c4;
-                const float* src = dn + (size_t)co * HoWo + (size_t)min(oh, a.Ho - 1) * a.Wo;
-                float4 v = make_float4(0.f, 0.f, 0.f, 0.f);
-                if (oh < a.Ho) {
-                    if (vec && ow + 3 < a.Wo) v = *reinterpret_cast<const float4*>(src + ow);
-                    else {
-                        if (ow < a.Wo) v.x = src[ow];
-                        if (ow + 1 < a.Wo) v.y = src[ow + 1];
-                        if (ow + 2 < a.Wo) v.z = src[ow + 2];
-                        if (ow + 3 < a.Wo) v.w = src[ow + 3];
+            if constexpr (BNFOLD) {
+#pragma unroll
+                for (int it = 0; it < 2; ++it) {
+                    const int bi = it * 256 + threadIdx.x;
+                    const int co = bi >> 3, t8 = bi & 7;
+                    const int ow = ow0 + 8 * t8;
+                    float ot[8], ob[8];
+#pragma unroll
+                    for (int k = 0; k < 8; ++k) ot[k] = ob[k] = 0.f;
+                    if (oh0 + 1 < a.Ho && ow + 7 < a.Wo) {
+                        const size_t plane = (size_t)n * 64 + co;
+                        const float* cc = bnc + co * 6;
+                        const float sc = cc[0], sh = cc[1], mu = cc[2], is = cc[3], m1 = cc[4], m2 = cc[5];
+                        const float fc = a.bn.coef[plane], fo = a.bn.off ? a.bn.off[plane] * a.bn.cscale : 0.f;
+                        float top[8], bot[8];
+                        stem_gy_block(a.bn, plane, oh0 >> 1, ow >> 3, fc, fo, top, bot);
+                        const float* xp = a.bn.x + plane * (size_t)HoWo + (size_t)oh0 * a.Wo + ow;
+#pragma unroll
+                        for (int h = 0; h < 2; ++h) {
+                            const float4 x0 = *reinterpret_cast<const float4*>(xp + 4 * h);
+                            const float4 x1 = *reinterpret_cast<const float4*>(xp + a.Wo + 4 * h);
+                            const float xv[8] = {x0.x, x0.y, x0.z, x0.w, x1.x, x1.y, x1.z, x1.w};
+#pragma unroll
+                            for (int k = 0; k < 4; ++k) {
+                                ot[4 * h + k] = stem_bn_dx(xv[k], top[4 * h + k], sc, sh, mu, is, m1, m2);
+                                ob[4 * h + k] = stem_bn_dx(xv[4 + k], bot[4 * h + k], sc, sh, mu, is, m1, m2);
+                            }
+                        }
                     }
-                }
-                dv[it] = v;
-            }
-#pragma unroll
-            for (int it = 0; it < NIT; ++it) {
-                const int e = it * 256 + threadIdx.x;
-                if (e < CI * IR * ICP) patch[e] = sv[it];
-            }
-#pragma unroll
-            for (int it = 0; it < 8; ++it) {
-                const int i4 = it * 256 + threadIdx.x;
-                const int co = i4 >> 5, q = i4 & 31;
-                float* dst = dyt + co * PP + q * 4;
-                dst[0] = dv[it].x; dst[1] = dv[it].y; dst[2] = dv[it].z; dst[3] = dv[it].w;
+                    float* dst = dyt + co * PP + 8 * t8;
+#pragma unroll
+                    for (int k = 0; k < 8; ++k) { dst[k] = ot[k]; dst[TCW + k] = ob[k]; }
+                }
+#pragma unroll
+                for (int it = 0; it < NIT; ++it) {
+                    const int e = it * 256 + threadIdx.x;
+                    if (e < CI * IR * ICP) patch[e] = sv[it];
+                }
+            } else {
+                float4 dv[8];
+                const float* dn = a.dy + (size_t)n * 64 * HoWo;
+                const bool vec = (a.Wo & 3) == 0;
+#pragma unroll
+                for (int it = 0; it < 8; ++it) {
+                    const int i4 = it * 256 + threadIdx.x;
+                    const int co = i4 >> 5, q = i4 & 31, r = q >> 4, c4 = (q & 15) * 4;
+                    const int oh = oh0 + r, ow = ow0 + c4;
+                    const float* src = dn + (size_t)co * HoWo + (size_t)min(oh, a.Ho - 1) * a.Wo;
+                    float4 v = make_float4(0.f, 0.f, 0.f, 0.f);
+                    if (oh < a.Ho) {
+                        if (vec && ow + 3 < a.Wo) v = *reinterpret_cast<const float4*>(src + ow);
+                        else {
+                            if (ow < a.Wo) v.x = src[ow];
+                            if (ow + 1 < a.Wo) v.y = src[ow + 1];
+                            if (ow + 2 < a.Wo) v.z = src[ow + 2];
+                            if (ow + 3 < a.Wo) v.w = src[ow + 3];
+                        }
+                    }
+                    dv[it] = v;
+                }
+#pragma unroll
+                for (int it = 0; it < NIT; ++it) {
+                    const int e = it * 256 + threadIdx.x;
+                    if (e < CI * IR * ICP) patch[e] = sv[it];
+                }
+#pragma unroll
+                for (int it = 0; it < 8; ++it) {
+                    const int i4 = it * 256 + threadIdx.x;
+                    const int co = i4 >> 5, q = i4 & 31;
+                    float* dst = dyt + co * PP + q * 4;
+                    dst[0] = dv[it].x; dst[1] = dv[it].y; dst[2] = dv[it].z; dst[3] = dv[it].w;
+                }
             }
         }
         __syncthreads();
@@ -668,6 +735,30 @@
     return DYNMM_OK;
 }
 
+bool stem_conv_wgrad_bn_eligible(int Ci, int Co, int KH, int KW, int SH, int SW, int PH, int PW, bool has_x2, int Ho, int Wo) {
+    return stem_conv_wgrad_eligible(Ci, Co, KH, KW, SH, SW, PH, PW, has_x2, false) && Ho > 0 && Wo > 0 && Ho % 2 == 0 &&
+           Wo % 8 == 0;
+}
+
+int launch_stem_conv_wgrad_bn(const float* x, const StemBnArgs& bn, const double* sums, float* dgamma, float* dbeta, float* dw,
+                              float* workspace, int N, int Ci, int H, int W, int Ho, int Wo, hipStream_t st) {
+    if (bn.N != N || bn.C != 64 || bn.H != Ho || bn.W != Wo || Ho % 2 != 0 || Wo % 8 != 0) return DYNMM_EINVAL;
+    const long tiles = (long)N * ceil_div(Ho, 2) * ceil_div(Wo, 64);
+    if (tiles > 0x7fffffffL) return DYNMM_EUNSUPPORTED;
+    const int grid = stem_wgrad_grid(tiles, Ci);
+    const int kpad = ((Ci * 56 + 31) / 32) * 32;
+    StemWgradBnArgs a{{x, nullptr, workspace, N, H, W, Ho, Wo}, bn, sums, dgamma, dbeta};
+    if (Ci == 3)
+        hipLaunchKernelGGL((conv_stem_wgrad_kernel<3, true>), dim3(grid), dim3(256), 0, st, a);
+    else
+        hipLaunchKernelGGL((conv_stem_wgrad_kernel<1, true>), dim3(grid), dim3(256), 0, st, a);
+    DYNMM_LAUNCH_CHECK();
+    hipLaunchKernelGGL(stem_wgrad_finish_kernel, dim3(ceil_div(64 * Ci * 49, 256)), dim3(256), 0, st, workspace, grid, kpad,
+                       Ci, dw);
+    DYNMM_LAUNCH_CHECK();
+    return DYNMM_OK;
+}
+
 bool stem_conv_fwd_eligible(const SmallConvArgs& a, const float* residual) {
     if (residual || a.x2) return false;
     if (a.KH != 7 || a.KW != 7 || a.SH != 2 || a.SW != 2 || a.PH != 3 || a.PW != 3) return false;
diff --git a/dynmm_amd/csrc/pointwise.hip b/dynmm_amd/csrc/pointwise.hip
--- a/dynmm_amd/csrc/pointwise.hip
+++ b/dynmm_amd/csrc/pointwise.hip
@@ -1048,28 +1048,6 @@
 
 namespace dynmm {
 
-struct StemBnArgs {
-    const float* go; const signed char* io;
-    const float* gd; const signed char* id;
-    const float* coef; const float* off; float cscale;
-    const float* x; const float* mean; const float* invstd; const float* gamma; const float* beta;
-    int N, C, H, W, Ho, Wo;
-};
-
-__device__ __forceinline__ void stem_gy_block(const StemBnArgs& a, size_t plane, int ar, int t, float fc, float fo,
-                                              float (&top)[8], float (&bot)[8]) {
-    const size_t po = plane * (size_t)a.Ho * a.Wo;
-    pool_bwd_block(a.go + po, a.io + po, ar, t, a.Ho, a.Wo, top, bot);
-#pragma unroll
-    for (int k = 0; k < 8; ++k) { top[k] = fmaf(fc, top[k], fo); bot[k] = fmaf(fc, bot[k], fo); }
-    if (a.gd) {
-        float dt[8], db[8];
-        pool_bwd_block(a.gd + po, a.id + po, ar, t, a.Ho, a.Wo, dt, db);
-#pragma unroll
-        for (int k = 0; k < 8; ++k) { top[k] += dt[k]; bot[k] += db[k]; }
-    }
-}
-
 __global__ void __launch_bounds__(256) stem_bn_bwd_reduce_kernel(const StemBnArgs a, double* __restrict__ sums) {
     __shared__ float red[4];
     const int c = blockIdx.x, S = gridDim.y;
@@ -1126,7 +1104,7 @@
         if (dbeta) dbeta[c] = sg;
     }
     const float invM = 1.f / ((float)a.N * (float)(a.H * a.W));
-    const float k0 = sc, m1 = sg * invM, m2 = sgx * invM;
+    const float m1 = sg * invM, m2 = sgx * invM;
     const float fc = a.coef[plane], fo = a.off ? a.off[plane] * a.cscale : 0.f;
     const float* xp = a.x + plane * (size_t)a.H * a.W;
     float* dp = dx + plane * (size_t)a.H * a.W;
@@ -1146,8 +1124,7 @@
 #pragma unroll
             for (int k = 0; k < 8; ++k) {
                 const float gy = k < 4 ? top[4 * h + k] : bot[4 * h + k - 4];
-                const float ge = fmaf(xv[k], sc, sh) > 0.f ? gy : 0.f;
-                ov[k] = k0 * (ge - m1 - (xv[k] - mu) * is * m2);
+                ov[k] = stem_bn_dx(xv[k], gy, sc, sh, mu, is, m1, m2);
             }
             *reinterpret_cast<float4*>(dp + o + 4 * h) = make_float4(ov[0], ov[1], ov[2], ov[3]);
             *reinterpret_cast<float4*>(dp + o + a.W + 4 * h) = make_float4(ov[4], ov[5], ov[6], ov[7]);
@@ -1198,18 +1175,6 @@
     hipLaunchKernelGGL(axpby_pool_bwd_apply_kernel, dim3(NC, plane_chunks(Ho * Wo, kChunk)), dim3(256), 0, ST, g_out,
                        idx_out, g_depth, idx_depth, a, b, ca, cb, cscale, dxr, dxd, H, W, Ho, Wo);
     DYNMM_LAUNCH_CHECK();
-    return DYNMM_OK;
-}
-
-static int stem_bn_args(StemBnArgs& a, const float* g_out, const signed char* idx_out, const float* g_depth,
-                        const signed char* idx_depth, const float* coef, const float* off, float cscale, const float* x,
-                        const float* mean, const float* invstd, const float* gamma, const float* beta, int N, int C, int H,
-                        int W) {
-    if (!g_out || !idx_out || !coef || !x || !mean || !invstd || !gamma || !beta || N <= 0 || C <= 0) return DYNMM_EINVAL;
-    if ((g_depth != nullptr) != (idx_depth != nullptr)) return DYNMM_EINVAL;
-    const int Ho = H / 2, Wo = W / 2;
-    if (!pool_fusable(H, W, Ho, Wo, {g_out, g_depth, x}, {idx_out, idx_depth})) return DYNMM_EUNSUPPORTED;
-    a = StemBnArgs{g_out, idx_out, g_depth, idx_depth, coef, off, cscale, x, mean, invstd, gamma, beta, N, C, H, W, Ho, Wo};
     return DYNMM_OK;
 }
 
diff --git a/dynmm_amd/csrc/pool.h b/dynmm_amd/csrc/pool.h
--- a/dynmm_amd/csrc/pool.h
+++ b/dynmm_amd/csrc/pool.h
@@ -48,4 +48,43 @@
     return true;
 }
 
+struct StemBnArgs {
+    const float* go; const signed char* io;
+    const float* gd; const signed char* id;
+    const float* coef; const float* off; float cscale;
+    const float* x; const float* mean; const float* invstd; const float* gamma; const float* beta;
+    int N, C, H, W, Ho, Wo;
+};
+
+__device__ __forceinline__ void stem_gy_block(const StemBnArgs& a, size_t plane, int ar, int t, float fc, float fo,
+                                              float (&top)[8], float (&bot)[8]) {
+    const size_t po = plane * (size_t)a.Ho * a.Wo;
+    pool_bwd_block(a.go + po, a.io + po, ar, t, a.Ho, a.Wo, top, bot);
+#pragma unroll
+    for (int k = 0; k < 8; ++k) { top[k] = fmaf(fc, top[k], fo); bot[k] = fmaf(fc, bot[k], fo); }
+    if (a.gd) {
+        float dt[8], db[8];
+        pool_bwd_block(a.gd + po, a.id + po, ar, t, a.Ho, a.Wo, dt, db);
+#pragma unroll
+        for (int k = 0; k < 8; ++k) { top[k] += dt[k]; bot[k] += db[k]; }
+    }
 }
+
+__device__ __forceinline__ float stem_bn_dx(float x, float gy, float sc, float sh, float mu, float is, float m1, float m2) {
+    const float ge = fmaf(x, sc, sh) > 0.f ? gy : 0.f;
+    return sc * (ge - m1 - (x - mu) * is * m2);
+}
+
+static inline int stem_bn_args(StemBnArgs& a, const float* g_out, const signed char* idx_out, const float* g_depth,
+                               const signed char* idx_depth, const float* coef, const float* off, float cscale,
+                               const float* x, const float* mean, const float* invstd, const float* gamma, const float* beta,
+                               int N, int C, int H, int W) {
+    if (!g_out || !idx_out || !coef || !x || !mean || !invstd || !gamma || !beta || N <= 0 || C <= 0) return DYNMM_EINVAL;
+    if ((g_depth != nullptr) != (idx_depth != nullptr)) return DYNMM_EINVAL;
+    const int Ho = H / 2, Wo = W / 2;
+    if (!pool_fusable(H, W, Ho, Wo, {g_out, g_depth, x}, {idx_out, idx_depth})) return DYNMM_EUNSUPPORTED;
+    a = StemBnArgs{g_out, idx_out, g_depth, idx_depth, coef, off, cscale, x, mean, invstd, gamma, beta, N, C, H, W, Ho, Wo};
+    return DYNMM_OK;
+}
+
+}
diff --git a/dynmm_amd/lib.py b/dynmm_amd/lib.py
--- a/dynmm_amd/lib.py
+++ b/dynmm_amd/lib.py
@@ -121,6 +121,8 @@
     'dynmm_axpby_pool_bwd_reduce': (c_i, [c_f] * 7 + [c_i] * 4 + [c_f]),
     'dynmm_stem_bn_bwd_reduce': (c_i, [c_f] * 6 + [c_fl] + [c_f] * 6 + [c_i] * 5 + [c_f]),
     'dynmm_stem_bn_bwd_apply': (c_i, [c_f] * 6 + [c_fl] + [c_f] * 9 + [c_i] * 4 + [c_f]),
+    'dynmm_conv2d_stem_wgrad_bn_supported': (c_i, [_GP]),
+    'dynmm_conv2d_stem_wgrad_bn': (c_i, [c_f] * 6 + [c_fl] + [c_f] * 11 + [c_sz, _GP, c_f]),
     'dynmm_gap2_bnrelu_fwd': (c_i, [c_f] * 3 + [c_i] + [c_f] * 2 + [c_i] * 2 + [c_f]),
     'dynmm_bn_finalize': (c_i, [c_f] * 10 + [c_i] * 3 + [c_fl, c_fl, c_f]),
     'dynmm_axpby_pool_bwd_apply': (c_i, [c_f] * 8 + [C.c_float] + [c_f] * 2 + [c_i] * 3 + [c_f]),
diff --git a/dynmm_amd/ops.py b/dynmm_amd/ops.py
--- a/dynmm_amd/ops.py
+++ b/dynmm_amd/ops.py
@@ -52,6 +52,7 @@
 WINO = 'all'
 WINO_DGRAD = '43h'
 CONV_BN_STATS = True
+STEM_WGRAD_FOLD = True
 _WINO_OK = {}
 _WINO43_OK = {}
 
@@ -821,6 +822,8 @@
         ctx.defer_mask = defer_mask
         ctx.link = link
         ctx.bn_link = bn_link
+        ctx.stem_fold = {} if (STEM_WGRAD_FOLD and not need_dx and x2 is None and bias is None and act == L.ACT_NONE and
+                               ctx.needs_input_grad[2] and lib.dynmm_conv2d_stem_wgrad_bn_supported(C.byref(g))) else None
         ctx.save_for_backward(x, x2, packed[kinds[1]] if need_dx else None, y if (act != L.ACT_NONE and not defer_mask) else None)
         ctx.wshape = tuple(weight.shape)
         ctx.w_param, ctx.b_param = (w_owner if w_owner is not None else weight), bias
@@ -832,7 +835,12 @@
         st = _stream()
         x, x2, wpd, y = ctx.saved_tensors
         g = ctx.geom
-        gy = _chk(gy, 'grad')
+        fold = ctx.stem_fold.pop('ops', None) if ctx.stem_fold is not None else None
+        if fold is None:
+            gy = _chk(gy, 'grad')
+        elif gy.data_ptr() != fold['ph'].data_ptr():
+            raise L.DynmmHipError('conv2d: the stem BatchNorm backward was left to this weight gradient, but the gradient that '
+                                  'arrived is not its placeholder (the convolution output has another consumer)')
         dbias = None
         act = L.ACT_NONE if ctx.defer_mask else ctx.act
         dbias_ret = None
@@ -897,20 +905,30 @@
         elif ctx.needs_input_grad[2]:
             dw, dw_ret = _grad_dst(ctx.w_param)
             nbytes = lib.dynmm_conv2d_wgrad_workspace_bytes(C.byref(g))
+            if fold is not None:
+                dgamma, dbeta = _grad_dst(fold['gp'])[0], _grad_dst(fold['bp'])[0]
+                what = 'conv2d_stem_wgrad_bn'
+
+                def launch(ws, stream):
+                    return lib.dynmm_conv2d_stem_wgrad_bn(*fold['head'], _p(fold['sums']), _p(dgamma), _p(dbeta), _p(x), _p(dw),
+                                                          _p(ws), nbytes, C.byref(g), stream)
+            else:
+                what = 'conv2d_wgrad'
+
+                def launch(ws, stream):
+                    return lib.dynmm_conv2d_wgrad(_p(x), _p(x2), _p(gy), _p(dw), _p(dbias) if bias_in_wgrad else None,
+                                                  _p(ws), nbytes, C.byref(g), stream)
             if dw_ret is None and _STEP.async_wgrad and PROFILE is None:
                 ws_stream = _wgrad_stream()
                 _CENSUS.add(ws_stream.cuda_stream)
                 ws_stream.wait_stream(torch.cuda.current_stream())
                 with torch.cuda.stream(ws_stream):
-                    ws = torch.empty(max(nbytes // 4, 1), device=gy.device, dtype=torch.float32)
-                    L.check(lib.dynmm_conv2d_wgrad(_p(x), _p(x2), _p(gy), _p(dw), _p(dbias) if bias_in_wgrad else None,
-                                                   _p(ws), nbytes, C.byref(g), ws_stream.cuda_stream), 'conv2d_wgrad')
-                _STEP.inflight.append((x, x2, gy))
+                    ws = torch.empty(max(nbytes // 4, 1), device=x.device, dtype=torch.float32)
+                    L.check(launch(ws, ws_stream.cuda_stream), what)
+                _STEP.inflight.append((x, x2, gy) if fold is None else (x, fold['keep']))
             else:
-                ws = torch.empty(max(nbytes // 4, 1), device=gy.device, dtype=torch.float32)
-                L.check(_timed('wgrad', g, lambda: lib.dynmm_conv2d_wgrad(_p(x), _p(x2), _p(gy), _p(dw),
-                                                                          _p(dbias) if bias_in_wgrad else None, _p(ws), nbytes,
-                                                                          C.byref(g), st)), 'conv2d_wgrad')
+                ws = torch.empty(max(nbytes // 4, 1), device=x.device, dtype=torch.float32)
+                L.check(_timed('wgrad', g, lambda: launch(ws, st)), what)
         _grads_enqueued(torch.cuda.current_stream(), ws_stream)
         if dw_ret is not None and tuple(dw_ret.shape) != ctx.wshape:
             dw_ret = dw_ret.reshape(ctx.wshape)
@@ -1600,7 +1618,7 @@
                                                 N * Cc, H, W, st), 'axpby_pool_bwd_reduce')
         dsr, dsd, dparams_ret = _se2_excite_bwd(lib, st, ctx, da, db, saved, params)
         _grads_enqueued()
-        def bn_chain(k):
+        def bn_chain(k, fold=None):
             x, coef, off, gdp, idp, gam, bet, gp, bp = (
                 (xr, a, dsr, None, None, gam_r, bet_r, ctx.bn_params[0], ctx.bn_params[1]),
                 (xd, b, dsd, g_d, idd, gam_d, bet_d, ctx.bn_params[2], ctx.bn_params[3]))[k]
@@ -1610,6 +1628,11 @@
             head = (_p(g_o), io.data_ptr(), _p(gdp), None if idp is None else idp.data_ptr(), _p(coef), _p(off), 1.0 / HW,
                     _p(x), _p(mean), _p(invstd), _p(gam), _p(bet))
             L.check(lib.dynmm_stem_bn_bwd_reduce(*head, _p(sums), N, Cc, H, W, zeroed, stq), 'stem_bn_bwd_reduce')
+            if fold is not None and STEM_WGRAD_FOLD and _direct_ok(gp) and _direct_ok(bp):
+                ph = torch.empty(1, **f32)
+                fold['ops'] = dict(head=head, sums=sums, gp=gp, bp=bp, ph=ph,
+                                   keep=(g_o, io, gdp, idp, coef, off, x, stats, gam, bet, sums))
+                return ph.expand(x.shape), None, None
             dgamma, dgamma_ret = _grad_dst(gp)
             dbeta, dbeta_ret = _grad_dst(bp)
             dx = torch.empty_like(x)
@@ -1619,7 +1642,7 @@
             return dx, dgamma_ret, dbeta_ret
         if ctx.slots is not None:
             for k in (0, 1):
-                ctx.slots[k]['bwd'] = (lambda k=k: bn_chain(k))
+                ctx.slots[k]['bwd'] = (lambda fold=None, k=k: bn_chain(k, fold))
             ph = torch.empty(1, **f32)
             return (ph.expand(xr.shape), ph.expand(xd.shape), *([None] * 18), *dparams_ret)
         (dxr, dgr, dbr), (dxd, dgd, dbd) = bn_chain(0), bn_chain(1)
@@ -1639,7 +1662,7 @@
         fn = ctx.slot.pop('bwd', None)
         if fn is None:
             return g, None, None, None
-        dx, dgam, dbet = fn()
+        dx, dgam, dbet = fn(ctx.slot.get('fold'))
         return dx, dgam, dbet, None
 
 
@@ -1647,6 +1670,9 @@
     if not (torch.is_grad_enabled() and (x.requires_grad or bn.weight.requires_grad)):
         return x
     slot = {}
+    fold = getattr(x.grad_fn, 'stem_fold', None)
+    if fold is not None:
+        slot['fold'] = fold
     y = _StemBNDeferred.apply(x, bn.weight, bn.bias, slot)
     y._stem_slot = slot
     for attr in ('_bn_sums',):
diff --git a/include/dynmm_hip.h b/include/dynmm_hip.h
--- a/include/dynmm_hip.h
+++ b/include/dynmm_hip.h
@@ -213,6 +213,12 @@
                             const float* x, const float* mean, const float* invstd, const float* gamma,
                             const float* beta, const double* sums, float* dx, float* dgamma, float* dbeta,
                             int N, int C, int H, int W, void* stream);
+int dynmm_conv2d_stem_wgrad_bn_supported(const dynmm_conv_geom* g);
+int dynmm_conv2d_stem_wgrad_bn(const float* g_out, const signed char* idx_out, const float* g_depth,
+                               const signed char* idx_depth, const float* coef, const float* off, float cscale,
+                               const float* y, const float* mean, const float* invstd, const float* gamma,
+                               const float* beta, const double* sums, float* dgamma, float* dbeta, const float* x,
+                               float* dw, void* workspace, size_t workspace_bytes, const dynmm_conv_geom* g, void* stream);
 int dynmm_axpby_pool_bwd_apply(const float* g_out, const signed char* idx_out, const float* g_depth,
                                const signed char* idx_depth, const float* a, const float* b, const float* ca,
                                const float* cb, float cscale, float* dxr, float* dxd, int NC, int H, int W, void* stream);
```

Measured after the change: 520.7 images/s (median of 6 runs). No clear change (+0.3%).
